# qq456cvb/SLAM-MaskRCNN

Hardware: AMD Instinct MI355X
Metric: Mvoxel-updates/s + frames/s, 512^3 semantic TSDF @ 640x480 (higher is better)
Workload: dtype f32; 1 GPU; C3: 512^3 semantic TSDF integrate (sdf f32, weight i32, colour u8x3, 32-bin u32 instance histogram), synthetic 640x480 depth+RGB+mask stream (seed 1, noise on), frames resident in HBM; frames_cycled=16

## Files before the change

### __graft_entry__.py

```python
from __future__ import annotations

import os
import subprocess
import sys

ROOT = os.path.dirname(os.path.abspath(__file__))
PKG = os.path.join(ROOT, "slam-maskrcnn_amd")
CSRC = os.path.join(PKG, "csrc")
LIB = os.path.join(PKG, "semtsdf", "libsemtsdf.so")

HIPCC_FLAGS = ["--offload-arch=gfx950", "-O3", "-ffp-contract=off", "-fPIC", "-shared", "-std=c++17", "-Wall",
               "-Wno-unused-result", "-Wno-bitwise-instead-of-logical"]


def _path():
    for p in (PKG, ROOT):
        if p not in sys.path:
            sys.path.insert(0, p)


def _lib_sources():
    srcs = [os.path.join(CSRC, f) for f in ("semtsdf_kernels.hip", "semtsdf_api.cpp")]
    hdrs = [os.path.join(CSRC, f) for f in ("semtsdf_internal.h", "semtsdf_libm.h", "semtsdf_steps.h")]
    return srcs, srcs + hdrs + [os.path.join(ROOT, "include", "semtsdf.h")]


def build_key(hipcc: str | None = None, extra_flags=()) -> str:
    import hashlib

    hipcc = hipcc or os.environ.get("HIPCC", "/opt/rocm/bin/hipcc")
    h = hashlib.sha256()
    for d in _lib_sources()[1]:
        with open(d, "rb") as f:
            h.update(os.path.basename(d).encode() + b"\0" + f.read() + b"\0")
    h.update(" ".join([*HIPCC_FLAGS, *extra_flags]).encode())
    try:
        ver = subprocess.run([hipcc, "--version"], capture_output=True, text=True, timeout=60).stdout
        h.update(next((ln for ln in ver.splitlines() if "clang version" in ln), ver).encode())
    except Exception:
        pass
    return h.hexdigest()


def build_lib(force: bool = False, extra_flags=(), out: str | None = None) -> str:
    srcs, deps = _lib_sources()
    out = out or LIB
    if not force and os.path.exists(out) and all(os.path.getmtime(out) >= os.path.getmtime(d) for d in deps):
        return out
    hipcc = os.environ.get("HIPCC", "/opt/rocm/bin/hipcc")
    key = build_key(hipcc, extra_flags)
    cmd = [hipcc, *HIPCC_FLAGS, *extra_flags, f'-DSEMTSDF_BUILD_KEY="{key}"', *srcs, "-o", out]
    subprocess.check_call(cmd)
    return out


DET_LIB = os.path.join(PKG, "semtsdf", "libsemtsdf_det.so")


def build_det_lib(force: bool = False) -> str:
    src = os.path.join(CSRC, "semtsdf_det.hip")
    deps = [src, os.path.join(ROOT, "include", "semtsdf_det.h")]
    if not force and os.path.exists(DET_LIB) and all(os.path.getmtime(DET_LIB) >= os.path.getmtime(d) for d in deps):
        return DET_LIB
    hipcc = os.environ.get("HIPCC", "/opt/rocm/bin/hipcc")
    subprocess.check_call([hipcc, *HIPCC_FLAGS, src, "-o", DET_LIB])
    return DET_LIB


def build() -> None:
    build_lib(force=True)
    build_det_lib(force=True)
    _path()
    sys.path.insert(0, os.path.join(ROOT, "oracle"))
    import oracle as O

    O.build(force=True)
    import semtsdf

    semtsdf.load()


def smoke() -> None:
    import numpy as np

    _path()
    sys.path.insert(0, os.path.join(ROOT, "oracle"))
    import oracle as O
    import semtsdf
    from semtsdf import _lib as L
    from semtsdf.synth import SyntheticStream

    semtsdf.load()
    st = SyntheticStream(seed=0)
    f0, f1, f2 = st.frame(0), st.frame(1), st.frame(2)
    D = 64
    p = semtsdf.default_params(D, (520.9, 521.0, 325.1, 249.7), 640, 480)
    semtsdf.place_from_frame(p, f0.depth, float(np.mean(f0.depth[f0.depth > 0])) / 5000.0, L.PLACE_SFM)
    vol = semtsdf.Volume(p, 0)
    g = O.OGeom.from_params(p)
    ost = O.OState(list(p.dim), p.mu, semantic=True)
    num_objs = 0
    for k, fr in enumerate((f1, f2)):
        E = (fr.w2c @ f0.c2w).astype(np.float32)
        m_gpu = fr.mask.copy()
        vol.parse_frame(fr.depth, fr.rgb, m_gpu, E)
        m_ref = fr.mask.copy()
# ... 30 lines not shown
```

### slam-maskrcnn_amd/csrc/semtsdf_api.cpp

```cpp
#include <hip/hip_runtime.h>

#include <algorithm>
#include <cmath>
#include <cstdarg>
#include <cstdio>
#include <cstdlib>
#include <cstring>
#include <mutex>
#include <string>
#include <vector>

#include "../../include/semtsdf.h"
#include "semtsdf_internal.h"

using namespace semtsdf;

namespace {

thread_local std::string g_err;

int fail(int code, const char* fmt, ...) {
    char buf[1024];
    va_list ap;
    va_start(ap, fmt);
    vsnprintf(buf, sizeof(buf), fmt, ap);
    va_end(ap);
    g_err = buf;
    return code;
}

#define HIPC(expr)                                                                                  \
    do {                                                                                            \
        hipError_t e_ = (expr);                                                                     \
        if (e_ != hipSuccess)                                                                       \
            return fail(e_ == hipErrorOutOfMemory ? SEMTSDF_ERR_OOM : SEMTSDF_ERR_HIP, "%s: %s (%s:%d)", \
                        #expr, hipGetErrorString(e_), __FILE__, __LINE__);                          \
    } while (0)

const uint8_t kPalette[kMaxObjects * 3] = {
    230, 25,  75,  60,  180, 75,  255, 225, 25,  0,   130, 200, 245, 130, 48,  145, 30,  180,
    70,  240, 240, 240, 50,  230, 210, 245, 60,  250, 190, 190, 0,   128, 128, 230, 190, 255,
    170, 110, 40,  255, 250, 200, 128, 0,   0,   170, 255, 195, 230, 25,  75,  60,  180, 75,
    255, 225, 25,  0,   130, 200, 245, 130, 48,  145, 30,  180, 70,  240, 240, 240, 50,  230,
    210, 245, 60,  250, 190, 190, 0,   128, 128, 230, 190, 255, 170, 110, 40,  255, 250, 200,
    128, 0,   0,   170, 255, 195};

constexpr int kCounters = 8;
#ifndef SEMTSDF_FRAME_SETS
#define SEMTSDF_FRAME_SETS 2
#endif
constexpr int kFrameSets = SEMTSDF_FRAME_SETS;

struct EventPair {
    hipEvent_t a, b;
};

}

struct semtsdf_vol {
    semtsdf_params p{};
    VolGeom g{};
    VolBufs b{};
    int device = 0;
    hipStream_t stream = nullptr;
    size_t device_bytes = 0;
    uint16_t* depth_d = nullptr;
    uint8_t* rgb_d = nullptr;
    uint8_t* mask_d = nullptr;
    int32_t* cls_d = nullptr;
    struct FrameSet {
        DepthPyramid pyr{};
        unsigned* unit_list = nullptr;
        unsigned* list_count = nullptr;
        unsigned* units = nullptr;
        unsigned* first_tab = nullptr;
        hipEvent_t prep_done = nullptr;
        hipEvent_t set_free = nullptr;
        bool free_recorded = false;
        hipStream_t reader = nullptr;
    } fs[kFrameSets];
    int next_set = 0;
    hipStream_t prep_stream = nullptr;
    hipEvent_t in_ev = nullptr;
    bool async_used = false;
    AssocTables* tables_d = nullptr;
    AssocDecision* decision_d = nullptr;
    AssocExact* exact_d = nullptr;
    AssocPixels px{};
    bool assoc_ray_done = false;
    int* num_objs_d = nullptr;
    float* probs_d = nullptr;
    uint8_t* box_d = nullptr;
    uint8_t* palette_d = nullptr;
    uint8_t* render_d = nullptr;
    float* render_t_d = nullptr;
    uint8_t* maps_d = nullptr;
    uint8_t* track_d = nullptr;
    unsigned long long* counters_d = nullptr;
    IntegrateRare* rare_d = nullptr;
    float* rcp_table_d = nullptr;
    AssocDecision* decision_h = nullptr;
    void* ray_state_d = nullptr;
    MarchCamera ray_cam{};
    int ray_kind = -1;
    int ray_nrec = 1;
    int ray_next = 0;
    uint32_t n_obs = 0;
    bool maps_dirty = false;
    bool maps_stale = true;
    hipEvent_t maps_ev = nullptr;
    bool maps_ev_set = false;
    hipStream_t map_stream = nullptr;
    bool map_set = false;
    bool multi_stream = false;
    bool color_wide = false;
    int64_t wmax_bound = 0;
    const uint8_t* pending_lut = nullptr;
    unsigned long long* wtrace_d = nullptr;
    unsigned* tile_cost_d = nullptr;
    unsigned* tile_perm_d = nullptr;
    int tile_cap = 0, tile_n = 0;
    bool tables_clean = false;
    unsigned long long votes_dropped_seen = 0;
    int instr = 0;
    std::vector<EventPair> ev_integrate, ev_assoc, ev_render, ev_prep;
    double t_integrate = 0, t_assoc = 0, t_render = 0, t_prep = 0;
    uint64_t n_integrate = 0, n_assoc = 0, n_render = 0, n_prep = 0;
};

namespace {

unsigned order_event_flags() { return hipEventDisableTiming | hipEventDisableSystemFence; }

size_t npx(const semtsdf_vol* v) { return (size_t)v->p.width * (size_t)v->p.height; }

hipStream_t pick(const semtsdf_vol* v, void* s) { return s ? (hipStream_t)s : v->stream; }

int dev_alloc(semtsdf_vol* v, void** p, size_t bytes) {
    if (bytes == 0) { *p = nullptr; return SEMTSDF_OK; }
    hipError_t e = hipMalloc(p, bytes);
    if (e != hipSuccess)
        return fail(e == hipErrorOutOfMemory ? SEMTSDF_ERR_OOM : SEMTSDF_ERR_HIP, "hipMalloc(%zu): %s", bytes,
                    hipGetErrorString(e));
    v->device_bytes += bytes;
    return SEMTSDF_OK;
}

void free_all(semtsdf_vol* v) {
    void* ptrs[] = {v->b.sdf, v->b.wt, v->b.bplain, v->b.boct, v->b.botmp, v->b.bdirty, v->b.dlist, v->b.sflag, v->b.color, v->b.hist, v->b.hmask, v->b.cls, v->b.cls_cnt, v->depth_d, v->rgb_d,
                    v->mask_d, v->cls_d, v->tables_d, v->decision_d,
                    v->num_objs_d, v->probs_d, v->box_d, v->palette_d, v->render_d, v->render_t_d, v->maps_d, v->track_d,
                    v->counters_d, v->ray_state_d, v->rcp_table_d, v->wtrace_d, v->exact_d, v->px.bits, v->px.p, v->tile_cost_d, v->tile_perm_d, v->rare_d};
    for (void* q : ptrs)
        if (q) (void)hipFree(q);
    for (auto& f : v->fs)
        for (void* q : {(void*)f.pyr.px, (void*)f.pyr.l0, (void*)f.pyr.l1, (void*)f.unit_list, (void*)f.list_count,
                        (void*)f.units})
            if (q) (void)hipFree(q);
    if (v->decision_h) (void)hipHostFree(v->decision_h);
    for (auto* vec : {&v->ev_integrate, &v->ev_assoc, &v->ev_render, &v->ev_prep})
        for (auto& e : *vec) { (void)hipEventDestroy(e.a); (void)hipEventDestroy(e.b); }
    if (v->maps_ev) (void)hipEventDestroy(v->maps_ev);
    for (auto& f : v->fs) {
        if (f.prep_done) (void)hipEventDestroy(f.prep_done);
        if (f.set_free) (void)hipEventDestroy(f.set_free);
    }
    if (v->prep_stream) (void)hipStreamDestroy(v->prep_stream);
    if (v->in_ev) (void)hipEventDestroy(v->in_ev);
    if (v->stream) (void)hipStreamDestroy(v->stream);
}

int local_planes(const semtsdf_params* p, int* chunk, int* halo);
int after_maps(semtsdf_vol* v, hipStream_t s);

int check_params(const semtsdf_params* p) {
    if (!p) return fail(SEMTSDF_ERR_INVALID, "params is NULL");
    for (int i = 0; i < 3; ++i) {
        if (p->dim[i] < 2 || p->dim[i] > 65535)
            return fail(SEMTSDF_ERR_INVALID, "dim[%d]=%d out of range [2, 65535]", i, p->dim[i]);
        if (!(p->voxel[i] > 0.0f) || !std::isfinite(p->voxel[i]))
            return fail(SEMTSDF_ERR_INVALID, "voxel[%d]=%g must be > 0 (place the volume first)", i, p->voxel[i]);
    }
    {
        const uint64_t ny = ((uint64_t)p->dim[1] + 7) / 8 * 8, nz = ((uint64_t)p->dim[2] + 2 * kZAlign) / kZAlign * kZAlign;
        if ((uint64_t)p->dim[0] * ny * nz >= (1ull << 32) || ny * nz >= (1ull << 32) || nz * 32 >= (1ull << 24))
            return fail(SEMTSDF_ERR_INVALID, "volume %d x %d x %d too large (2^32 stored voxels or more)", p->dim[0],
                        p->dim[1], p->dim[2]);
    }
    if (!(p->mu > 0.0f)) return fail(SEMTSDF_ERR_INVALID, "mu=%g must be > 0", p->mu);
    if (p->width <= 0 || p->height <= 0 || p->width > 65535 || p->height > 65535 || (int64_t)p->width * p->height > (1 << 28))
        return fail(SEMTSDF_ERR_INVALID, "bad frame size %dx%d", p->width, p->height);
    if (!(p->depth_scale > 0.0f)) return fail(SEMTSDF_ERR_INVALID, "depth_scale must be > 0");
    if (!(p->prior_mrcnn_err_rate >= 0x1p-10f && p->prior_mrcnn_err_rate < 1.0f))
        return fail(SEMTSDF_ERR_INVALID, "prior_mrcnn_err_rate=%g outside [2^-10, 1)", (double)p->prior_mrcnn_err_rate);
    if ((p->flags & SEMTSDF_F_VOTE) && (p->flags & SEMTSDF_F_SEMANTIC))
        return fail(SEMTSDF_ERR_INVALID, "SEMANTIC and VOTE are exclusive");
    for (int i = 0; i < 3; ++i)
        if (!(p->voxel[i] >= 0x1p-20f && p->voxel[i] <= 0x1p20f))
            return fail(SEMTSDF_ERR_INVALID, "voxel size %g outside [2^-20, 2^20]", (double)p->voxel[i]);
// ... 10 lines not shown
                        p->dim[1], p->dim[2], lz);
    }
    return SEMTSDF_OK;
}

int local_planes(const semtsdf_params* p, int* chunk, int* halo) {
    if (p->z_nshards == 1) { *chunk = p->dim[2]; *halo = 0; return p->dim[2]; }
    *chunk = p->z_chunk;
    *halo = 1;
    const int nchunks = (p->dim[2] + p->z_chunk - 1) / p->z_chunk;
    int mine = 0;
    const int n = p->z_nshards;
    for (int r = 0; r * n < nchunks; ++r)
        if (r * n + ((r & 1) ? n - 1 - p->z_shard : p->z_shard) < nchunks) ++mine;
    return mine * (p->z_chunk + 1);
}

void fill_E(float dst[12], const float E[16]) {
    for (int i = 0; i < 12; ++i) dst[i] = E[i];
}

void timing_begin(semtsdf_vol* v, std::vector<EventPair>& vec, hipStream_t s, EventPair* ep) {
    ep->a = ep->b = nullptr;
    if (!(v->instr & 1)) return;
    if (hipEventCreate(&ep->a) != hipSuccess || hipEventCreate(&ep->b) != hipSuccess) return;
    (void)hipEventRecord(ep->a, s);
    (void)vec;
}

void timing_end(semtsdf_vol* v, std::vector<EventPair>& vec, hipStream_t s, EventPair* ep) {
    if (!(v->instr & 1) || !ep->a) return;
    (void)hipEventRecord(ep->b, s);
    vec.push_back(*ep);
}

void screen_map(IntegrateArgs& a) {
    for (int i = 0; i < 3; ++i) {
        for (int j = 0; j < 3; ++j) {
            const double acc = (double)a.K[i * 3 + 0] * (double)a.E[0 * 4 + j] +
                               (double)a.K[i * 3 + 1] * (double)a.E[1 * 4 + j] +
                               (double)a.K[i * 3 + 2] * (double)a.E[2 * 4 + j];
            a.M[i * 3 + j] = (float)acc;
        }
        const double acc = (double)a.K[i * 3 + 0] * (double)a.E[3] + (double)a.K[i * 3 + 1] * (double)a.E[7] +
                           (double)a.K[i * 3 + 2] * (double)a.E[11];
        a.m[i] = (float)acc;
    }
    double KE[4][4];
    for (int i = 0; i < 4; ++i)
        for (int j = 0; j < 4; ++j) {
            if (i == 3) {
                KE[i][j] = (double)a.E[2 * 4 + j];
                continue;
            }
            KE[i][j] = (double)a.K[i * 3 + 0] * (double)a.E[0 * 4 + j] + (double)a.K[i * 3 + 1] * (double)a.E[1 * 4 + j] +
                       (double)a.K[i * 3 + 2] * (double)a.E[2 * 4 + j];
        }
    for (int i = 0; i < 4; ++i) {
        double c0 = KE[i][3];
        for (int j = 0; j < 3; ++j) {
            a.cullC[i * 4 + j] = (float)(KE[i][j] * (double)a.g.voxel[j]);
            c0 += KE[i][j] * (double)a.g.start[j];
        }
        a.cullC[i * 4 + 3] = (float)c0;
    }
    int b = 1;
    while (b < (a.width > a.height ? a.width : a.height) + 2) b <<= 1;
    a.ftol = 0.5f - ldexpf((float)b, -21);
}

int widen_color(semtsdf_vol* v, hipStream_t s) {
    if (v->color_wide) return SEMTSDF_OK;
    void* wide = nullptr;
    if (int rc = dev_alloc(v, &wide, v->g.nvox * 16)) return rc;
    HIPC(launch_color_widen(static_cast<const uint8_t*>(v->b.color), static_cast<int32_t*>(wide), v->g.nvox, s));
    HIPC(hipStreamSynchronize(s));
    HIPC(hipFree(v->b.color));
    v->device_bytes -= v->g.nvox * 4;
    v->b.color = wide;
    v->color_wide = true;
    return SEMTSDF_OK;
}


int ensure_prep_stream(semtsdf_vol* v) {
    if (v->prep_stream) return SEMTSDF_OK;
    int lo = 0, hi = 0;
    if (hipDeviceGetStreamPriorityRange(&lo, &hi) != hipSuccess) hi = 0;
    HIPC(hipStreamCreateWithPriority(&v->prep_stream, hipStreamNonBlocking, hi));
    for (auto& f : v->fs) {
        HIPC(hipEventCreateWithFlags(&f.prep_done, order_event_flags()));
        HIPC(hipEventCreateWithFlags(&f.set_free, order_event_flags()));
    }
    return SEMTSDF_OK;
}

int integrate_impl(semtsdf_vol* v, const uint16_t* depth_d, const uint8_t* rgb_d, const uint8_t* mask_d,
                   const int32_t* cls_d, const float E[16], hipStream_t s, bool async = false,
                   hipEvent_t inputs_ready = nullptr, bool inputs_on_s = false) {
    if (!E) return fail(SEMTSDF_ERR_INVALID, "E is NULL");
    if (!depth_d || !rgb_d) return fail(SEMTSDF_ERR_INVALID, "depth/rgb is NULL");
    if ((v->p.flags & SEMTSDF_F_SEMANTIC) && !mask_d) return fail(SEMTSDF_ERR_INVALID, "semantic volume needs a mask");
    if ((v->p.flags & SEMTSDF_F_VOTE) && !cls_d) return fail(SEMTSDF_ERR_INVALID, "vote volume needs cls");
    if ((v->p.flags & SEMTSDF_F_COLOR_I32) && !v->color_wide && v->wmax_bound + 1 >= (1ll << 23)) {
        if (int rc = widen_color(v, s)) return rc;
    }
    IntegrateArgs a{};
    a.g = v->g;
    a.b = v->b;
    fill_E(a.E, E);
    const float* K = v->p.K;
    a.K[0] = K[0]; a.K[1] = K[1]; a.K[2] = K[2];
    a.K[3] = K[4]; a.K[4] = K[5]; a.K[5] = K[6];
    a.K[6] = K[8]; a.K[7] = K[9]; a.K[8] = K[10];
    a.width = v->p.width;
    a.height = v->p.height;
    a.depth_scale = v->p.depth_scale;
    a.gate = v->p.gate;
    a.flags = v->p.flags | ((v->instr & 2) ? 0x80000000u : 0u);
    a.color_wide = v->color_wide ? 1 : 0;
    a.cull = (v->p.flags & SEMTSDF_F_NO_CULL) ? 0 : 1;
    {
        static const char* dbg = getenv("SEMTSDF_DEBUG_INTEGRATE");
        a.debug = dbg ? atoi(dbg) : 0;
    }
    a.depth = depth_d;
    a.rgb = rgb_d;
    a.mask = mask_d;
    a.cls = cls_d;
    const int fset = v->next_set;
    semtsdf_vol::FrameSet& F = v->fs[fset];
    a.pyr = F.pyr;
    a.counters = v->counters_d;
    a.rare = v->rare_d;
    a.unit_list = F.unit_list;
    a.list_count = F.list_count;
    a.units = F.units;
    a.first_tab = F.first_tab;
    a.first_nwaves = integrate_pre_waves();
    a.rcp_table = v->rcp_table_d;
    screen_map(a);
    a.pinhole = (a.K[1] == 0.0f && a.K[3] == 0.0f && a.K[6] == 0.0f && a.K[7] == 0.0f && a.K[8] == 1.0f) ? 1 : 0;
    a.rmu = 1.0f / v->g.mu;
    a.skip_thr = v->g.voxel[0] / 2.0f * (1.0f + 0x1p-16f);
    a.fastdiv = (v->g.mu >= 0x1p-20f && v->g.mu <= 0x1p20f && a.debug != 8) ? 1 : 0;
    a.free_ok = ((v->p.flags & SEMTSDF_F_GATE_COLOR) && !(v->p.flags & SEMTSDF_F_VOTE) && !(a.gate > 1.0f) &&
                 a.fastdiv && a.debug != 9)
                    ? 1
                    : 0;
    if (a.debug == 2) return SEMTSDF_OK;
    const uint8_t* lut = mask_d ? v->pending_lut : nullptr;
    const bool relabel_after = async && lut;
    if (async)
        if (int rc = ensure_prep_stream(v)) return rc;
    hipStream_t ps = s;
    const bool own_order = inputs_ready && inputs_on_s && s == v->stream && (!F.reader || F.reader == v->stream);
    if (async) {
        ps = v->prep_stream;
        v->async_used = true;
        if (inputs_ready) HIPC(hipStreamWaitEvent(ps, inputs_ready, 0));
        if (!own_order) {
            if (!F.free_recorded) {
                HIPC(hipEventRecord(F.set_free, F.reader == v->stream ? v->stream : s));
                F.free_recorded = true;
            }
            HIPC(hipStreamWaitEvent(ps, F.set_free, 0));
        }
    }
    v->next_set = (v->next_set + 1) % kFrameSets;
    EventPair epp;
    timing_begin(v, v->ev_prep, ps, &epp);
    HIPC(launch_depth_pyramid(depth_d, rgb_d, const_cast<uint8_t*>(mask_d), v->p.width, v->p.height,
                              v->p.depth_scale, F.pyr, F.list_count, ps, relabel_after ? nullptr : lut));
    if (lut && !relabel_after) v->pending_lut = nullptr;
    HIPC(launch_cull(a, ps));
    HIPC(launch_compact_lists(a, ps));
    timing_end(v, v->ev_prep, ps, &epp);
    v->n_prep++;
    if (async) {
        HIPC(hipEventRecord(F.prep_done, ps));
        HIPC(hipStreamWaitEvent(s, F.prep_done, 0));
    }
    if (relabel_after) {
        a.lut = &v->decision_d->lut[0];
        a.relabel_mask = const_cast<uint8_t*>(mask_d);
    }
    if (int rc = after_maps(v, s)) return rc;
    v->wmax_bound += 1;
// ... 364 lines not shown
    if (mode == SEMTSDF_PLACE_PYTHON) {
        const double md = mean_depth / 5000.0;
        double tl[3], br[3];
        const double tv[3] = {(double)rx, (double)ry, 1.0}, bv[3] = {(double)(rx + rw), (double)(ry + rh), 1.0};
        for (int i = 0; i < 3; ++i) {
            tl[i] = ((double)Ki[i * 4 + 0] * tv[0] + (double)Ki[i * 4 + 1] * tv[1]) + (double)Ki[i * 4 + 2] * tv[2];
            br[i] = ((double)Ki[i * 4 + 0] * bv[0] + (double)Ki[i * 4 + 1] * bv[1]) + (double)Ki[i * 4 + 2] * bv[2];
            tl[i] *= md;
            br[i] *= md;
        }
        const double dx = tl[0] - br[0], dy = tl[1] - br[1];
        const double half = std::sqrt(dx * dx + dy * dy) / 2.0;
        double vox[3];
        for (int i = 0; i < 3; ++i) {
            const double c = (tl[i] + br[i]) / 2.0;
            const double s = c - half, e = c + half;
            p->vol_start[i] = (float)s;
            p->vol_end[i] = (float)e;
            vox[i] = (e - s) / (double)(p->dim[i] - 1);
            p->voxel[i] = (float)vox[i];
        }
        p->mu = (float)(5.0 * vox[0]);
    } else {
        const float md = (float)mean_depth;
        float tl[4], br[4];
        const float tv[4] = {(float)rx, (float)ry, 1.0f, 1.0f};
        const float bv[4] = {(float)(rx + rw), (float)(ry + rh), 1.0f, 1.0f};
        for (int i = 0; i < 4; ++i) {
            double at = 0, ab = 0;
            for (int k = 0; k < 4; ++k) {
                at += (double)Ki[i * 4 + k] * (double)tv[k];
                ab += (double)Ki[i * 4 + k] * (double)bv[k];
            }
            tl[i] = (float)((double)(float)at * (double)md);
            br[i] = (float)((double)(float)ab * (double)md);
        }
        const float dx = tl[0] - br[0], dy = tl[1] - br[1];
        const float half = (float)(std::sqrt(std::pow((double)dx, 2) + std::pow((double)dy, 2)) / 2.0);
        for (int i = 0; i < 3; ++i) {
            const float c = (tl[i] + br[i]) * 0.5f;
            p->vol_start[i] = c - half;
            p->vol_end[i] = c + half;
            p->voxel[i] = (p->vol_end[i] - p->vol_start[i]) / (float)(p->dim[i] - 1);
        }
        p->mu = 5.0f * p->voxel[0];
    }
    return SEMTSDF_OK;
}

int semtsdf_create(const semtsdf_params* p, int device, semtsdf_vol** out) {
    if (!out) return fail(SEMTSDF_ERR_INVALID, "out is NULL");
    *out = nullptr;
    int rc = check_params(p);
    if (rc) return rc;
    HIPC(hipSetDevice(device));
    semtsdf_vol* v = new semtsdf_vol();
    v->p = *p;
    v->device = device;
    int chunk, halo;
    const int lz = local_planes(p, &chunk, &halo);
    VolGeom& g = v->g;
    g.dimx = p->dim[0]; g.dimy = p->dim[1]; g.dimz = p->dim[2];
    g.lz = lz;
    g.zs = (lz + kZAlign - 1) & ~(kZAlign - 1);
    g.shard = p->z_shard; g.nshards = p->z_nshards; g.chunk = chunk; g.halo = halo;
    for (int i = 0; i < 3; ++i) { g.start[i] = p->vol_start[i]; g.end[i] = p->vol_end[i]; g.voxel[i] = p->voxel[i]; }
    g.mu = p->mu;
    g.nuy = (uint32_t)(g.dimy + 7) / 8;
    g.nuz = (uint32_t)g.zs / 32;
    g.nvox = (uint64_t)g.dimx * g.nuy * g.nuz * 256u;
    g.ty = g.nuz * 256u;
    g.tx = g.nuy * g.ty;
    g.nbx = (g.dimx + 7) / 8; g.nby = (g.dimy + 7) / 8; g.nbz = (g.lz + 7) / 8;
    for (int i = 0; i < 3; ++i) g.rvox[i] = 1.0f / g.voxel[i];
    const size_t n = g.nvox;
    const size_t px = (size_t)p->width * p->height;
    auto bail = [&](int code) { free_all(v); delete v; return code; };
    int prio_least = 0, prio_greatest = 0;
    if (hipDeviceGetStreamPriorityRange(&prio_least, &prio_greatest) != hipSuccess) prio_greatest = 0;
    if (hipStreamCreateWithPriority(&v->stream, hipStreamNonBlocking, prio_greatest) != hipSuccess)
        return bail(fail(SEMTSDF_ERR_HIP, "hipStreamCreate failed"));
    const bool ci32 = p->flags & SEMTSDF_F_COLOR_I32;
    if ((rc = dev_alloc(v, (void**)&v->b.sdf, n * 4))) return bail(rc);
    if ((rc = dev_alloc(v, (void**)&v->b.wt, n * 4))) return bail(rc);
    if ((rc = dev_alloc(v, (void**)&v->b.sflag, n / 32 + 1))) return bail(rc);
    const size_t nbricks = (size_t)g.nbx * g.nby * g.nbz;
    if ((rc = dev_alloc(v, (void**)&v->b.bplain, nbricks * 4))) return bail(rc);
    if ((rc = dev_alloc(v, (void**)&v->b.boct, nbricks * 8))) return bail(rc);
    if ((rc = dev_alloc(v, (void**)&v->b.botmp, nbricks * 8))) return bail(rc);
    const size_t nquads = (size_t)g.nbx * g.nby * (size_t)((g.nbz + 3) / 4);
    if ((rc = dev_alloc(v, (void**)&v->b.bdirty, nquads * 4))) return bail(rc);
    if ((rc = dev_alloc(v, (void**)&v->b.dlist, (nquads + 1) * 4))) return bail(rc);
    if (nquads && (hipMemset(v->b.bdirty, 0, nquads * 4) != hipSuccess || hipMemset(v->b.dlist, 0, 4) != hipSuccess))
        return bail(fail(SEMTSDF_ERR_HIP, "memset failed"));
    (void)ci32;
    if ((rc = dev_alloc(v, &v->b.color, g.nvox * 4))) return bail(rc);
    if (p->flags & SEMTSDF_F_SEMANTIC)
    {
        if ((rc = dev_alloc(v, (void**)&v->b.hist, g.nvox * kMaxObjects * 4))) return bail(rc);
        if ((rc = dev_alloc(v, (void**)&v->b.hmask, n * 4))) return bail(rc);
    }
    if (p->flags & SEMTSDF_F_VOTE) {
        if ((rc = dev_alloc(v, (void**)&v->b.cls, n * 4))) return bail(rc);
        if ((rc = dev_alloc(v, (void**)&v->b.cls_cnt, n * 4))) return bail(rc);
        if ((rc = dev_alloc(v, (void**)&v->cls_d, px * 4))) return bail(rc);
    }
    if ((rc = dev_alloc(v, (void**)&v->depth_d, px * 2))) return bail(rc);
    if ((rc = dev_alloc(v, (void**)&v->rgb_d, px * 3))) return bail(rc);
    if ((rc = dev_alloc(v, (void**)&v->mask_d, px))) return bail(rc);
    for (auto& f : v->fs) {
        DepthPyramid& pyr = f.pyr;
        pyr.w0 = (p->width + 7) / 8; pyr.h0 = (p->height + 7) / 8;
        pyr.w1 = (p->width + 31) / 32; pyr.h1 = (p->height + 31) / 32;
        pyr.rs = 4u * (unsigned)((p->width + 1 + 3) / 4 * 4);
        const size_t nrec = (size_t)pyr.rs * (size_t)((p->height + 1 + 3) / 4);
        if ((rc = dev_alloc(v, (void**)&pyr.px, nrec * 8))) return bail(rc);
        if (hipMemset(pyr.px, 0, nrec * 8) != hipSuccess) return bail(fail(SEMTSDF_ERR_HIP, "memset failed"));
        if ((rc = dev_alloc(v, (void**)&pyr.l0, (size_t)pyr.w1 * 4 * pyr.h1 * 4 * sizeof(uint2)))) return bail(rc);
        if ((rc = dev_alloc(v, (void**)&pyr.l1, (size_t)pyr.w1 * pyr.h1 * sizeof(uint2)))) return bail(rc);
        if ((rc = dev_alloc(v, (void**)&f.unit_list, unit_list_capacity(g) * sizeof(unsigned)))) return bail(rc);
        if ((rc = dev_alloc(v, (void**)&f.list_count, kListCountWords * sizeof(unsigned)))) return bail(rc);
        const uint64_t nunits = std::max<uint64_t>(unit_count(g) + 2 * kLists + 2, 2u * (uint64_t)kPreWaves + 6u);
        if ((rc = dev_alloc(v, (void**)&f.units, (nunits + 2u * (uint64_t)kPreWaves) * sizeof(unsigned)))) return bail(rc);
        f.first_tab = f.units + nunits;
    }
    if ((rc = dev_alloc(v, (void**)&v->rcp_table_d, kRcpTable * sizeof(float)))) return bail(rc);
    {
        float t[kRcpTable];
        for (int i = 0; i < kRcpTable; ++i) t[i] = 1.0f / (float)(i + 1);
        if (hipMemcpy(v->rcp_table_d, t, sizeof(t), hipMemcpyHostToDevice) != hipSuccess)
            return bail(fail(SEMTSDF_ERR_HIP, "rcp table upload failed"));
    }
    if ((rc = dev_alloc(v, (void**)&v->tables_d, sizeof(AssocTables)))) return bail(rc);
    if ((rc = dev_alloc(v, (void**)&v->decision_d, sizeof(AssocDecision)))) return bail(rc);
    if ((rc = dev_alloc(v, (void**)&v->exact_d, sizeof(AssocExact)))) return bail(rc);
    if (hipMemset(v->exact_d, 0, sizeof(AssocExact)) != hipSuccess) return bail(fail(SEMTSDF_ERR_HIP, "memset failed"));
    if ((p->flags & SEMTSDF_F_SEMANTIC) && p->z_nshards == 1) {
        if ((rc = dev_alloc(v, (void**)&v->px.bits, npx(v) * sizeof(uint2)))) return bail(rc);
        if ((rc = dev_alloc(v, (void**)&v->px.p, npx(v) * kMaxObjects * sizeof(float)))) return bail(rc);
    }
    if ((rc = dev_alloc(v, (void**)&v->num_objs_d, 16))) return bail(rc);
    if ((rc = dev_alloc(v, (void**)&v->counters_d, kCounters * sizeof(unsigned long long)))) return bail(rc);
    if ((rc = dev_alloc(v, (void**)&v->rare_d, sizeof(IntegrateRare)))) return bail(rc);
    {
        const IntegrateRare r{v->b.bdirty, v->b.dlist, g.nby, g.nbz, v->counters_d};
        if (hipMemcpy(v->rare_d, &r, sizeof(r), hipMemcpyHostToDevice) != hipSuccess)
            return bail(fail(SEMTSDF_ERR_HIP, "upload of the integrate's rare-path fields failed"));
    }
    if ((rc = dev_alloc(v, (void**)&v->palette_d, sizeof(kPalette)))) return bail(rc);
    if (hipHostMalloc((void**)&v->decision_h, sizeof(AssocDecision), 0) != hipSuccess)
        return bail(fail(SEMTSDF_ERR_HIP, "hipHostMalloc failed"));
    if (hipMemcpy(v->palette_d, kPalette, sizeof(kPalette), hipMemcpyHostToDevice) != hipSuccess)
        return bail(fail(SEMTSDF_ERR_HIP, "palette upload failed"));
    if ((rc = semtsdf_reset(v, nullptr))) return bail(rc);
    if (hipStreamSynchronize(v->stream) != hipSuccess) return bail(fail(SEMTSDF_ERR_HIP, "sync failed"));
    *out = v;
    return SEMTSDF_OK;
}

int semtsdf_destroy(semtsdf_vol* v) {
    if (!v) return SEMTSDF_OK;
    (void)hipSetDevice(v->device);
    (void)hipStreamSynchronize(v->stream);
    free_all(v);
    delete v;
    return SEMTSDF_OK;
}

int semtsdf_get_params(const semtsdf_vol* v, semtsdf_params* out) {
    if (!v || !out) return fail(SEMTSDF_ERR_INVALID, "NULL argument");
    *out = v->p;
    return SEMTSDF_OK;
}

int semtsdf_get_state(const semtsdf_vol* v, semtsdf_state* out) {
    if (!v || !out) return fail(SEMTSDF_ERR_INVALID, "NULL argument");
    int n = 0;
    unsigned long long dropped = 0;
    HIPC(hipMemcpyAsync(&n, v->num_objs_d, sizeof(int), hipMemcpyDeviceToHost, v->stream));
    HIPC(hipMemcpyAsync(&dropped, v->counters_d + 2, sizeof(dropped), hipMemcpyDeviceToHost, v->stream));
    HIPC(hipStreamSynchronize(v->stream));
    out->n_obs = v->n_obs;
    out->num_objs = n;
    out->local_dim[0] = v->g.dimx;
    out->local_dim[1] = v->g.dimy;
    out->local_dim[2] = v->g.lz;
    out->local_voxels = (uint64_t)v->g.dimx * v->g.dimy * v->g.lz;
    out->device_bytes = v->device_bytes;
    out->label_votes_dropped = dropped;
    return SEMTSDF_OK;
}

int semtsdf_set_state(semtsdf_vol* v, uint32_t n_obs, int32_t num_objs) {
    if (!v) return fail(SEMTSDF_ERR_INVALID, "NULL handle");
    v->n_obs = n_obs;
    HIPC(hipMemcpyAsync(v->num_objs_d, &num_objs, sizeof(int), hipMemcpyHostToDevice, v->stream));
    HIPC(hipStreamSynchronize(v->stream));
    return SEMTSDF_OK;
}

void* semtsdf_get_stream(const semtsdf_vol* v) { return v ? (void*)v->stream : nullptr; }

int semtsdf_reset(semtsdf_vol* v, void* stream) {
    if (!v) return fail(SEMTSDF_ERR_INVALID, "NULL handle");
    HIPC(hipSetDevice(v->device));
    hipStream_t s = pick(v, stream);
    const size_t n = v->g.nvox;
    if (int rc = after_maps(v, s)) return rc;
    HIPC(launch_fill_volume(v->g, v->b, v->p.flags, s));
    HIPC(hipMemsetAsync(v->b.wt, 0, n * 4, s));
    HIPC(hipMemsetAsync(v->b.sflag, 0, n / 32 + 1, s));
    HIPC(hipMemsetAsync(v->b.color, 0, v->g.nvox * 4 * (v->color_wide ? 4 : 1), s));
    if (v->b.hist) HIPC(hipMemsetAsync(v->b.hist, 0, v->g.nvox * kMaxObjects * 4, s));
    if (v->b.hmask) HIPC(hipMemsetAsync(v->b.hmask, 0, n * 4, s));
    if (v->b.cls) HIPC(hipMemsetAsync(v->b.cls, 0, n * 4, s));
    if (v->b.cls_cnt) HIPC(hipMemsetAsync(v->b.cls_cnt, 0, n * 4, s));
    HIPC(hipMemsetAsync(v->num_objs_d, 0, 16, s));
    HIPC(hipMemsetAsync(v->counters_d, 0, kCounters * sizeof(unsigned long long), s));
    v->votes_dropped_seen = 0;
    v->n_obs = 0;
    v->wmax_bound = 0;
    v->maps_stale = true;
    return SEMTSDF_OK;
}

static int observe_before(semtsdf_vol* v, const uint8_t* mask_d, hipStream_t s) {
    if (!(v->p.flags & SEMTSDF_F_SEMANTIC) || v->n_obs > 0) return SEMTSDF_OK;
    if (!mask_d) return fail(SEMTSDF_ERR_INVALID, "semantic volume needs a mask");
    if (int rc = tables_ready(v, s)) return rc;
    HIPC(launch_mask_stats(mask_d, (int)npx(v), v->tables_d, s));
    HIPC(launch_first_frame_objs(v->tables_d, v->num_objs_d, s));
    return SEMTSDF_OK;
}
static void observe_after(semtsdf_vol* v) {
    if (v->p.flags & SEMTSDF_F_SEMANTIC) v->n_obs++;
}

int semtsdf_integrate(semtsdf_vol* v, const uint16_t* depth, const uint8_t* rgb, const uint8_t* mask,
                      const float E[16], void* stream) {
    if (!v || !depth || !rgb) return fail(SEMTSDF_ERR_INVALID, "NULL argument");
    HIPC(hipSetDevice(v->device));
    hipStream_t s = pick(v, stream);
    const size_t n = npx(v);
    const bool sem = v->p.flags & SEMTSDF_F_SEMANTIC;
    bool past_bins = false;
    if (sem) {
        if (!mask) return fail(SEMTSDF_ERR_INVALID, "semantic volume needs a mask");
        if (v->p.flags & SEMTSDF_F_ID_SATURATE) {
            if (int rc = validate_mask_host(v, mask)) return rc;
        } else {
            past_bins = validate_mask_host(v, mask) != SEMTSDF_OK;
        }
    }
    HIPC(hipMemcpyAsync(v->depth_d, depth, n * 2, hipMemcpyHostToDevice, s));
    HIPC(hipMemcpyAsync(v->rgb_d, rgb, n * 3, hipMemcpyHostToDevice, s));
    if (sem) HIPC(hipMemcpyAsync(v->mask_d, mask, n, hipMemcpyHostToDevice, s));
    if (int rc = observe_before(v, sem ? v->mask_d : nullptr, s)) return rc;
    int rc = integrate_impl(v, v->depth_d, v->rgb_d, sem ? v->mask_d : nullptr, nullptr, E, s);
    if (rc) return rc;
    observe_after(v);
    HIPC(hipStreamSynchronize(s));
    if (!sem) return SEMTSDF_OK;
    const int rc_votes = check_bad_label(v, s);
    if (past_bins)
        return fail(SEMTSDF_ERR_LABEL, "mask labels >= %d have no histogram bin: their votes were dropped, the "
                    "frame was applied (SEMTSDF_F_ID_SATURATE keeps ids below %d)", kMaxObjects, kMaxObjects);
    return rc_votes;
}

int semtsdf_integrate_dev(semtsdf_vol* v, const uint16_t* depth_d, const uint8_t* rgb_d, const uint8_t* mask_d,
                          const float E[16], void* stream) {
    if (!v) return fail(SEMTSDF_ERR_INVALID, "NULL handle");
    HIPC(hipSetDevice(v->device));
    hipStream_t s = pick(v, stream);
    if (int rc = observe_before(v, mask_d, s)) return rc;
    if (int rc = integrate_impl(v, depth_d, rgb_d, mask_d, nullptr, E, s)) return rc;
    observe_after(v);
    return SEMTSDF_OK;
}

int semtsdf_integrate_dev_async(semtsdf_vol* v, const uint16_t* depth_d, const uint8_t* rgb_d, const uint8_t* mask_d,
                                const float E[16], void* inputs_ready, void* stream) {
    if (!v) return fail(SEMTSDF_ERR_INVALID, "NULL handle");
    HIPC(hipSetDevice(v->device));
    hipStream_t s = pick(v, stream);
    if (int rc = observe_before(v, mask_d, s)) return rc;
    if (int rc = integrate_impl(v, depth_d, rgb_d, mask_d, nullptr, E, s, true, (hipEvent_t)inputs_ready)) return rc;
    observe_after(v);
    return SEMTSDF_OK;
}

int semtsdf_integrate_vote_dev(semtsdf_vol* v, const uint16_t* depth_d, const uint8_t* rgb_d, const int32_t* cls_d,
                               const float E[16], void* stream) {
// ... 758 lines not shown
    if (flags) HIPC(hipMemcpyAsync(flags, flags_d, n, hipMemcpyDeviceToHost, s));
    HIPC(hipStreamSynchronize(s));
    return SEMTSDF_OK;
}

static int icp_check(semtsdf_vol* v, const semtsdf_icp_in* in, const float* E_ref, const float* E_cur, float dist_max,
                     float cos_min, int32_t stride, const int64_t* words) {
    if (!v || !in || !E_ref || !E_cur || !words) return fail(SEMTSDF_ERR_INVALID, "NULL argument");
    if (!in->vertex || !in->normal || !in->flags || !in->m_point || !in->m_normal || !in->m_flags)
        return fail(SEMTSDF_ERR_INVALID, "NULL input map");
    if (npx(v) > ((size_t)1 << 19))
        return fail(SEMTSDF_ERR_INVALID, "image %d x %d has more than 2^19 pixels (the bound of the integer sums)",
                    v->p.width, v->p.height);
    if (stride < 1) return fail(SEMTSDF_ERR_INVALID, "stride=%d must be >= 1", (int)stride);
    if (!(dist_max > 0.0f && dist_max <= 1.0f))
        return fail(SEMTSDF_ERR_INVALID, "dist_max=%g outside (0, 1]", (double)dist_max);
    if (!(cos_min >= -1.0f && cos_min <= 1.0f))
        return fail(SEMTSDF_ERR_INVALID, "cos_min=%g outside [-1, 1]", (double)cos_min);
    if (v->p.z_nshards != 1)
        return fail(SEMTSDF_ERR_UNSUPPORTED, "the ICP system on a Z-sharded handle is not supported");
    return SEMTSDF_OK;
}

static int icp_impl(semtsdf_vol* v, const semtsdf_icp_in& in_d, const float E_ref[16], const float E_cur[16],
                    float dist_max, float cos_min, int32_t stride, int64_t* words_d, hipStream_t s) {
    IcpArgs a{};
    a.vertex = in_d.vertex; a.normal = in_d.normal; a.flags = in_d.flags;
    a.m_point = in_d.m_point; a.m_normal = in_d.m_normal; a.m_flags = in_d.m_flags;
    for (int i = 0; i < 3; ++i) {
        double acc = 0;
        for (int k = 0; k < 3; ++k) acc += (double)E_cur[k * 4 + i] * (double)E_cur[k * 4 + 3];
        a.o[i] = (float)(-acc);
        for (int j = 0; j < 3; ++j) {
            a.Rt[i * 3 + j] = E_cur[j * 4 + i];
            a.K[i * 3 + j] = v->p.K[i * 4 + j];
        }
    }
    fill_E(a.Eref, E_ref);
    a.dmax2 = dist_max * dist_max;
    a.cos_min = cos_min;
    a.stride = stride;
    a.width = v->p.width;
    a.height = v->p.height;
    a.words = reinterpret_cast<long long*>(words_d);
    HIPC(hipMemsetAsync(words_d, 0, kIcpWords * 8, s));
    HIPC(launch_icp_system(a, s));
    return SEMTSDF_OK;
}

int semtsdf_icp_system_dev(semtsdf_vol* v, const semtsdf_icp_in* in_dev, const float E_ref[16],
                           const float E_cur[16], float dist_max, float cos_min, int32_t stride, int64_t* words_dev,
                           void* stream) {
    if (int rc = icp_check(v, in_dev, E_ref, E_cur, dist_max, cos_min, stride, words_dev)) return rc;
    HIPC(hipSetDevice(v->device));
    return icp_impl(v, *in_dev, E_ref, E_cur, dist_max, cos_min, stride, words_dev, pick(v, stream));
}

int semtsdf_icp_system(semtsdf_vol* v, const semtsdf_icp_in* in_host, const float E_ref[16], const float E_cur[16],
                       float dist_max, float cos_min, int32_t stride, int64_t* words_host, void* stream) {
    if (int rc = icp_check(v, in_host, E_ref, E_cur, dist_max, cos_min, stride, words_host)) return rc;
    HIPC(hipSetDevice(v->device));
    hipStream_t s = pick(v, stream);
    const size_t n = npx(v);
    if (int rc = track_scratch(v)) return rc;
    float* f = reinterpret_cast<float*>(v->track_d);
    uint8_t* b = v->track_d + n * 48 + kIcpWords * 8;
    int64_t* words_d = reinterpret_cast<int64_t*>(v->track_d + n * 48);
    HIPC(hipMemcpyAsync(f, in_host->vertex, n * 12, hipMemcpyHostToDevice, s));
    HIPC(hipMemcpyAsync(f + n * 3, in_host->normal, n * 12, hipMemcpyHostToDevice, s));
    HIPC(hipMemcpyAsync(f + n * 6, in_host->m_point, n * 12, hipMemcpyHostToDevice, s));
    HIPC(hipMemcpyAsync(f + n * 9, in_host->m_normal, n * 12, hipMemcpyHostToDevice, s));
    HIPC(hipMemcpyAsync(b, in_host->flags, n, hipMemcpyHostToDevice, s));
    HIPC(hipMemcpyAsync(b + n, in_host->m_flags, n, hipMemcpyHostToDevice, s));
    semtsdf_icp_in d{f, f + n * 3, b, f + n * 6, f + n * 9, b + n};
    if (int rc = icp_impl(v, d, E_ref, E_cur, dist_max, cos_min, stride, words_d, s)) return rc;
    HIPC(hipMemcpyAsync(words_host, words_d, kIcpWords * 8, hipMemcpyDeviceToHost, s));
    HIPC(hipStreamSynchronize(s));
    return SEMTSDF_OK;
}

static uint64_t nref(const semtsdf_vol* v) { return (uint64_t)v->g.dimx * v->g.dimy * v->g.lz; }

static int vox_xfer(semtsdf_vol* v, void* host, void* dev, bool to_host, const char* what, hipStream_t s, uint64_t vb,
                    uint64_t ve) {
    if (ve <= vb) return SEMTSDF_OK;
    const uint64_t chunk = std::min<uint64_t>(ve - vb, 1ull << 26);
    void* stage = nullptr;
    HIPC(hipMalloc(&stage, chunk * 4));
    for (uint64_t v0 = vb; v0 < ve; v0 += chunk) {
        const uint64_t nv = std::min<uint64_t>(chunk, ve - v0);
        char* h = static_cast<char*>(host) + (v0 - vb) * 4;
        hipError_t e;
        if (to_host) {
            e = launch_vox_chunk(dev, stage, true, v->g, v0, nv, s);
            if (e == hipSuccess) e = hipMemcpyAsync(h, stage, nv * 4, hipMemcpyDeviceToHost, s);
        } else {
            e = hipMemcpyAsync(stage, h, nv * 4, hipMemcpyHostToDevice, s);
            if (e == hipSuccess) e = launch_vox_chunk(stage, dev, false, v->g, v0, nv, s);
        }
        if (e == hipSuccess) e = hipStreamSynchronize(s);
        if (e != hipSuccess) {
            (void)hipFree(stage);
            return fail(SEMTSDF_ERR_HIP, "%s transfer: %s", what, hipGetErrorString(e));
        }
    }
    HIPC(hipFree(stage));
    return SEMTSDF_OK;
}

static int color_xfer(semtsdf_vol* v, void* host, bool to_host, hipStream_t s, uint64_t vb, uint64_t ve) {
    const bool i32 = v->p.flags & SEMTSDF_F_COLOR_I32;
    const size_t es = i32 ? 4 : 1;
    if (ve <= vb) return SEMTSDF_OK;
    const uint64_t chunk = std::min<uint64_t>(ve - vb, 1ull << 24);
    void* stage = nullptr;
    HIPC(hipMalloc(&stage, chunk * 3 * es));
    for (uint64_t v0 = vb; v0 < ve; v0 += chunk) {
        const uint64_t nv = std::min<uint64_t>(chunk, ve - v0);
        char* h = static_cast<char*>(host) + (v0 - vb) * 3 * es;
        hipError_t e;
        if (to_host) {
            e = launch_color_chunk(v->b.color, stage, true, i32, v->color_wide, v->g, v0, nv, s);
            if (e == hipSuccess) e = hipMemcpyAsync(h, stage, nv * 3 * es, hipMemcpyDeviceToHost, s);
        } else {
            e = hipMemcpyAsync(stage, h, nv * 3 * es, hipMemcpyHostToDevice, s);
            if (e == hipSuccess) e = launch_color_chunk(stage, v->b.color, false, i32, v->color_wide, v->g, v0, nv, s);
        }
        if (e == hipSuccess) e = hipStreamSynchronize(s);
        if (e != hipSuccess) {
            (void)hipFree(stage);
            return fail(SEMTSDF_ERR_HIP, "colour transfer: %s", hipGetErrorString(e));
        }
    }
    HIPC(hipFree(stage));
    return SEMTSDF_OK;
}

int semtsdf_download_slab(semtsdf_vol* v, int x0, int x1, float* sdf, int32_t* wt, void* color, uint32_t* hist,
                          int32_t* cls, int32_t* cls_cnt) {
    if (!v) return fail(SEMTSDF_ERR_INVALID, "NULL handle");
    if (x0 < 0 || x1 > v->g.dimx || x0 > x1) return fail(SEMTSDF_ERR_INVALID, "bad x range [%d, %d)", x0, x1);
    HIPC(hipSetDevice(v->device));
    hipStream_t s = v->stream;
    const uint64_t plane = (uint64_t)v->g.dimy * v->g.lz;
    const uint64_t vb = (uint64_t)x0 * plane, ve = (uint64_t)x1 * plane;
    int rc;
    if (sdf && (rc = vox_xfer(v, sdf, v->b.sdf, true, "sdf", s, vb, ve))) return rc;
    if (wt && (rc = vox_xfer(v, wt, v->b.wt, true, "weight", s, vb, ve))) return rc;
    if (color) {
        rc = color_xfer(v, color, true, s, vb, ve);
        if (rc) return rc;
    }
    if (cls) {
        if (!(v->p.flags & SEMTSDF_F_VOTE)) return fail(SEMTSDF_ERR_STATE, "not a VOTE volume");
        if ((rc = vox_xfer(v, cls, v->b.cls, true, "cls", s, vb, ve))) return rc;
    }
    if (cls_cnt) {
        if (!(v->p.flags & SEMTSDF_F_VOTE)) return fail(SEMTSDF_ERR_STATE, "not a VOTE volume");
        if ((rc = vox_xfer(v, cls_cnt, v->b.cls_cnt, true, "cls_cnt", s, vb, ve))) return rc;
    }
    if (hist) {
        if (!(v->p.flags & SEMTSDF_F_SEMANTIC)) return fail(SEMTSDF_ERR_STATE, "not a SEMANTIC volume");
        const uint64_t chunk = std::max<uint64_t>(1, std::min<uint64_t>(ve - vb, 1ull << 22));
        uint32_t* stage = nullptr;
        HIPC(hipMalloc(&stage, chunk * kMaxObjects * 4));
        for (uint64_t v0 = vb; v0 < ve; v0 += chunk) {
            const uint64_t nv = std::min<uint64_t>(chunk, ve - v0);
            hipError_t e = launch_hist_chunk_to_vm(v->b.hist, stage, v->g, v0, nv, s);
            if (e == hipSuccess)
                e = hipMemcpyAsync(hist + (v0 - vb) * kMaxObjects, stage, nv * kMaxObjects * 4, hipMemcpyDeviceToHost, s);
            if (e == hipSuccess) e = hipStreamSynchronize(s);
            if (e != hipSuccess) {
                (void)hipFree(stage);
                return fail(SEMTSDF_ERR_HIP, "histogram download: %s", hipGetErrorString(e));
            }
        }
        HIPC(hipFree(stage));
    }
    HIPC(hipStreamSynchronize(s));
    return SEMTSDF_OK;
}

int semtsdf_download(semtsdf_vol* v, float* sdf, int32_t* wt, void* color, uint32_t* hist, int32_t* cls,
                     int32_t* cls_cnt) {
    if (!v) return fail(SEMTSDF_ERR_INVALID, "NULL handle");
    return semtsdf_download_slab(v, 0, v->g.dimx, sdf, wt, color, hist, cls, cls_cnt);
}

int semtsdf_upload(semtsdf_vol* v, const float* sdf, const int32_t* wt, const void* color, const uint32_t* hist,
                   const int32_t* cls, const int32_t* cls_cnt) {
    if (!v) return fail(SEMTSDF_ERR_INVALID, "NULL handle");
    HIPC(hipSetDevice(v->device));
    hipStream_t s = v->stream;
    int rc;
    if ((rc = after_maps(v, s))) return rc;
    v->maps_stale = true;
    if (sdf || wt) HIPC(hipMemsetAsync(v->b.sflag, 0, v->g.nvox / 32 + 1, s));
    if (sdf && (rc = vox_xfer(v, const_cast<float*>(sdf), v->b.sdf, false, "sdf", s, 0, nref(v)))) return rc;
    if (wt && (rc = vox_xfer(v, const_cast<int32_t*>(wt), v->b.wt, false, "weight", s, 0, nref(v)))) return rc;
    if (wt) {
        int64_t m = 0;
        for (uint64_t i = 0, n = nref(v); i < n; ++i) m = std::max<int64_t>(m, wt[i]);
        v->wmax_bound = m;
    }
    if (color) {
        if ((v->p.flags & SEMTSDF_F_COLOR_I32) && !v->color_wide) {
            const int32_t* c = static_cast<const int32_t*>(color);
            const uint64_t nc = nref(v) * 3;
            bool fits = true;
            for (uint64_t i = 0; i < nc && fits; ++i) fits = (uint32_t)c[i] <= 255u;
            if (!fits && (rc = widen_color(v, s))) return rc;
        }
        rc = color_xfer(v, const_cast<void*>(color), false, s, 0, nref(v));
        if (rc) return rc;
    }
    if (cls) {
        if (!(v->p.flags & SEMTSDF_F_VOTE)) return fail(SEMTSDF_ERR_STATE, "not a VOTE volume");
        if ((rc = vox_xfer(v, const_cast<int32_t*>(cls), v->b.cls, false, "cls", s, 0, nref(v)))) return rc;
    }
    if (cls_cnt) {
        if (!(v->p.flags & SEMTSDF_F_VOTE)) return fail(SEMTSDF_ERR_STATE, "not a VOTE volume");
        if ((rc = vox_xfer(v, const_cast<int32_t*>(cls_cnt), v->b.cls_cnt, false, "cls_cnt", s, 0, nref(v)))) return rc;
    }
    if (hist) {
        if (!(v->p.flags & SEMTSDF_F_SEMANTIC)) return fail(SEMTSDF_ERR_STATE, "not a SEMANTIC volume");
        HIPC(hipMemsetAsync(v->b.hmask, 0xFF, v->g.nvox * 4, s));
        const uint64_t n = (uint64_t)v->g.dimx * v->g.dimy * v->g.lz;
        const uint64_t chunk = std::max<uint64_t>(1, std::min<uint64_t>(n, 1ull << 22));
        uint32_t* stage = nullptr;
        HIPC(hipMalloc(&stage, chunk * kMaxObjects * 4));
        for (uint64_t v0 = 0; v0 < n; v0 += chunk) {
            const uint64_t nv = std::min<uint64_t>(chunk, n - v0);
            hipError_t e =
                hipMemcpyAsync(stage, hist + v0 * kMaxObjects, nv * kMaxObjects * 4, hipMemcpyHostToDevice, s);
            if (e == hipSuccess) e = launch_hist_chunk_to_bm(stage, v->b.hist, v->g, v0, nv, s);
            if (e == hipSuccess) e = hipStreamSynchronize(s);
            if (e != hipSuccess) {
                (void)hipFree(stage);
                return fail(SEMTSDF_ERR_HIP, "histogram upload: %s", hipGetErrorString(e));
            }
        }
        HIPC(hipFree(stage));
        HIPC(launch_hist_mask(v->g, v->b, s));
    }
    v->maps_stale = true;
    HIPC(hipStreamSynchronize(s));
    return SEMTSDF_OK;
}

int semtsdf_map_words(semtsdf_vol* v, uint64_t* out, uint64_t capacity, uint64_t* count) {
    if (!v || !count) return fail(SEMTSDF_ERR_INVALID, "NULL argument");
    HIPC(hipSetDevice(v->device));
    hipStream_t s = v->stream;
    *count = (uint64_t)v->g.nbx * v->g.nby * v->g.nbz;
    if (int rc = ensure_maps(v, s)) return rc;
    const uint64_t n = std::min<uint64_t>(capacity, *count);
    if (out && n) HIPC(hipMemcpyAsync(out, v->b.boct, n * sizeof(uint64_t), hipMemcpyDeviceToHost, s));
    HIPC(hipStreamSynchronize(s));
    return SEMTSDF_OK;
}

int semtsdf_export_surface(semtsdf_vol* v, float sdf_max, int32_t min_weight, semtsdf_surface_point* out,
                           uint64_t capacity, uint64_t* count) {
    static_assert(sizeof(semtsdf_surface_point) == sizeof(SurfacePoint), "surface point layout");
    if (!v || !count) return fail(SEMTSDF_ERR_INVALID, "NULL argument");
    if (!(sdf_max > 0.0f)) return fail(SEMTSDF_ERR_INVALID, "sdf_max must be > 0");
    HIPC(hipSetDevice(v->device));
    hipStream_t s = v->stream;
    if (int rc = after_maps(v, s)) return rc;
    unsigned long long* cnt_d = nullptr;
    HIPC(hipMalloc((void**)&cnt_d, sizeof(unsigned long long)));
    SurfacePoint* pts_d = nullptr;
    auto cleanup = [&]() {
        if (cnt_d) (void)hipFree(cnt_d);
        if (pts_d) (void)hipFree(pts_d);
    };
    auto run = [&](SurfacePoint* o, uint64_t cap, unsigned long long* n) -> hipError_t {
        hipError_t e = hipMemsetAsync(cnt_d, 0, sizeof(unsigned long long), s);
        if (e == hipSuccess) e = launch_export_surface(v->g, v->b, sdf_max, min_weight, v->color_wide ? 1 : 0,
                                                       (v->p.flags & SEMTSDF_F_SEMANTIC) ? 1 : 0, o, cap, cnt_d, s);
        if (e == hipSuccess) e = hipMemcpyAsync(n, cnt_d, sizeof(*n), hipMemcpyDeviceToHost, s);
        if (e == hipSuccess) e = hipStreamSynchronize(s);
        return e;
    };
    unsigned long long n = 0;
    hipError_t e = run(nullptr, 0, &n);
// ... 286 lines not shown
```

### slam-maskrcnn_amd/csrc/semtsdf_internal.h

```cpp
#pragma once
#include <hip/hip_runtime_api.h>
#include <stdint.h>

namespace semtsdf {

constexpr int kMaxObjects = 32;
constexpr int kMaxDetections = 256;
constexpr int kRcpTable = 1024;
constexpr int kZAlign = 32;
#ifndef SEMTSDF_BRICK_DIST_CAP
#define SEMTSDF_BRICK_DIST_CAP 16
#endif
constexpr int kBrickDistCap = SEMTSDF_BRICK_DIST_CAP;
constexpr int kListSegs = 64;
constexpr unsigned kPreWaves = 65534;
constexpr unsigned kFirstTabSlots = kListSegs * 256;
constexpr int kListCountStride = 64;
constexpr int kLists = 3;
constexpr int kListTotalsWord = kLists * kListSegs * kListCountStride;
constexpr int kListCountWords = kListTotalsWord + 8;

struct VolGeom {
    int dimx, dimy, dimz;
    int lz;
    int zs;
    int shard, nshards, chunk, halo;
    float start[3];
    float end[3];
    float voxel[3];
    float mu;
    uint64_t nvox;
    uint32_t nuy, nuz;
    uint32_t tx, ty;
    int nbx, nby, nbz;
    float rvox[3];
};

__device__ inline uint32_t tile_xterm(const VolGeom& g, int x) { return (uint32_t)x * g.tx; }
__device__ inline uint32_t tile_yterm(const VolGeom& g, int y) {
    return __umul24((uint32_t)(y >> 3), g.ty) + (uint32_t)(y & 7) * 4u;
}
__device__ inline uint32_t tile_zterm(int zl) { return (uint32_t)(zl >> 5) * 256u + (uint32_t)((zl >> 2) & 7) * 32u + (uint32_t)(zl & 3); }
__device__ inline uint32_t tile_index(const VolGeom& g, int x, int y, int zl) {
    return tile_xterm(g, x) + tile_yterm(g, y) + tile_zterm(zl);
}

struct VolBufs {
    float* sdf;
    int32_t* wt;
    void* color;
    uint32_t* hist;
    uint32_t* hmask;
    int32_t* cls;
    int32_t* cls_cnt;
    float* bplain;
    uint64_t* boct;
    uint64_t* botmp;
    uint32_t* bdirty;
    uint32_t* dlist;
    uint8_t* sflag;
};

struct DepthPyramid {
    uint2* px;
    uint2* l0;
    uint2* l1;
    int w0, h0, w1, h1;
    unsigned rs;
};

__device__ inline unsigned rec_index(const DepthPyramid& p, unsigned u, unsigned v) {
    return __umul24(v >> 2, p.rs) + ((u << 2) | (v & 3u));
}

struct IntegrateRare {
    uint32_t* bdirty;
    uint32_t* dlist;
    int nby, nbz;
    unsigned long long* counters;
};

struct IntegrateArgs {
    VolGeom g;
    VolBufs b;
    float E[12];
    float K[9];
    float M[9];
    float m[3];
    float cullC[16];
    float ftol;
    float skip_thr;
    const float* rcp_table;
    int width, height;
    float depth_scale;
    float gate;
    uint32_t flags;
    int cull;
    int debug;
    const uint16_t* depth;
    const uint8_t* rgb;
    const uint8_t* mask;
    const int32_t* cls;
    DepthPyramid pyr;
    unsigned long long* counters;
    int pinhole;
    float rmu;
    int fastdiv;
    unsigned* unit_list;
    unsigned* list_count;
    unsigned* units;
    int free_ok;
    int color_wide;
    unsigned long long* wtrace;
    unsigned wtrace_slots;
    const uint8_t* lut;
    uint8_t* relabel_mask;
    const IntegrateRare* rare;
    unsigned* first_tab;
    unsigned first_nwaves;
};
constexpr int kWaveTraceWords = 8;

constexpr double kFixScale = 268435456.0;
struct AssocTables {
    long long t1[kMaxObjects][kMaxObjects];
    long long t3[kMaxObjects][kMaxObjects];
    long long t2[kMaxObjects];
    unsigned int c1[kMaxObjects];
    unsigned int c2[kMaxObjects];
    unsigned int c3[kMaxObjects][kMaxObjects];
    unsigned int first_px[256];
    unsigned int max_label;
    unsigned int pos_max;
};
static_assert(sizeof(AssocTables) % 8 == 0, "AssocTables is cleared as 8-B words");

struct AssocDecision {
    int max_obj_now;
    int num_objs_before;
    int num_objs_after;
    int bad_label;
    int assigned_prev[kMaxObjects];
    float assigned_prob[kMaxObjects];
    unsigned char lut[256];
// ... 86 lines not shown
    uint8_t* flags;
};

struct FrameMapsArgs {
    const uint16_t* depth;
    float Kinv[9];
    float depth_scale;
    int width, height;
    float* vertex;
    float* normal;
    uint8_t* flags;
};

constexpr int kIcpWords = 32;

struct IcpArgs {
    const float* vertex;
    const float* normal;
    const uint8_t* flags;
    const float* m_point;
    const float* m_normal;
    const uint8_t* m_flags;
    float Rt[9], o[3];
    float Eref[12];
    float K[9];
    float dmax2, cos_min;
    int stride;
    int width, height;
    long long* words;
};

struct ShardRayState {
    int* k;
    float* fk;
    int* j;
    float* fj;
    float* fp;
    float* t;
};

constexpr int kAssocPartialLen = 3 * kMaxObjects * kMaxObjects + 3 * kMaxObjects;

struct ShardRayArgs {
    VolGeom g;
    VolBufs b;
    MarchCamera cam;
    int width, height;
    int kind;
    int step;
    const int2* gathered;
    int nrec;
    int2* send;
    ShardRayState st;
    int color_i32;
    const uint8_t* palette;
    uint8_t* out_bgr;
    float* out_t;
    const uint8_t* mask;
    float n_obs, eps, box_thresh;
    long long* partial;
};

hipError_t launch_shard_ray_step(const ShardRayArgs& a, hipStream_t s);
hipError_t launch_shard_render_final(const ShardRayArgs& a, hipStream_t s);
hipError_t launch_shard_render_finish(const ShardRayArgs& a, hipStream_t s);
hipError_t launch_shard_assoc_partial(const ShardRayArgs& a, hipStream_t s);
hipError_t launch_shard_assoc_pixels(const ShardRayArgs& a, int32_t* out, hipStream_t s);
hipError_t launch_tables_from_partial(const long long* reduced, AssocTables* t, hipStream_t s);
hipError_t launch_copy_f4(const void* src, void* dst, size_t n16, hipStream_t s);
hipError_t launch_min_i64(long long* dst, const long long* src, size_t n, hipStream_t s);
hipError_t launch_masks_to_labels(const uint8_t* masks, int npx, int n, int min_area, void* scratch, uint8_t* out,
                                  hipStream_t s);
size_t mask_scratch_bytes();
size_t mask_scratch_kept_offset();
hipError_t launch_detections_to_labels(const int32_t* boxes, const void* mini, int dtype, int mh, int mw, int n,
                                       int width, int height, int min_area, void* scratch, uint8_t* out,
                                       uint32_t* areas, hipStream_t s);
hipError_t launch_brick_min(const VolGeom& g, const VolBufs& b, bool all, hipStream_t s);
hipError_t launch_fill_volume(const VolGeom& g, const VolBufs& b, uint32_t flags, hipStream_t s);
hipError_t launch_depth_pyramid(const uint16_t* depth, const uint8_t* rgb, uint8_t* mask, int w, int h,
                                float scale, const DepthPyramid& p, unsigned* list_count, hipStream_t s,
                                const uint8_t* lut = nullptr);
hipError_t launch_vox_chunk(const void* src, void* dst, bool to_ref, const VolGeom& g, uint64_t v0, uint64_t nv,
                            hipStream_t s);
hipError_t launch_color_widen(const uint8_t* narrow, int32_t* wide, uint64_t nvox, hipStream_t s);
hipError_t launch_color_chunk(const void* src, void* dst, bool to_ref, bool ref_i32, bool dev_i32, const VolGeom& g,
                              uint64_t v0, uint64_t nv, hipStream_t s);
hipError_t launch_integrate(const IntegrateArgs& a, hipStream_t s, hipEvent_t e0 = nullptr,
                            hipEvent_t e1 = nullptr);
uint64_t unit_count(const VolGeom& g);
uint64_t unit_list_capacity(const VolGeom& g);
int unit_grid_fits(int dimx, int dimy, int local_z);
hipError_t launch_cull(const IntegrateArgs& a, hipStream_t s);
hipError_t launch_compact_lists(const IntegrateArgs& a, hipStream_t s);
unsigned integrate_pre_waves();
hipError_t launch_tables_init(AssocTables* t, hipStream_t s);
hipError_t launch_mask_stats(const uint8_t* mask, int npx, AssocTables* t, hipStream_t s);
hipError_t launch_assoc_march(const AssocArgs& a, hipStream_t s);
hipError_t launch_assoc_decide(const DecideArgs& a, hipStream_t s);
hipError_t launch_assoc_from_probs(const float* probs, const uint8_t* box, const uint8_t* mask, int npx, float n_obs,
                                   float eps, AssocTables* t, AssocPixels px, hipStream_t s);
hipError_t launch_libm_eval(int fn, const float* x, float* y, size_t n, hipStream_t s);
hipError_t launch_first_frame_objs(const AssocTables* t, int* num_objs_dev, hipStream_t s);
hipError_t launch_relabel(uint8_t* mask, int npx, const AssocDecision* d, hipStream_t s);
hipError_t launch_render(const RenderArgs& a, hipStream_t s);
hipError_t launch_model_maps(const MapsArgs& a, hipStream_t s);
hipError_t launch_frame_maps(const FrameMapsArgs& a, hipStream_t s);
hipError_t launch_icp_system(const IcpArgs& a, hipStream_t s);
hipError_t launch_march_fused(const AssocArgs& aa, const RenderArgs& ra, hipStream_t s);
hipError_t launch_copy_host(const void* src, void* dst, size_t n16, hipStream_t s);
hipError_t launch_hist_chunk_to_vm(const uint32_t* bm, uint32_t* vm, const VolGeom& g, uint64_t v0, uint64_t nv,
                                   hipStream_t s);
hipError_t launch_hist_chunk_to_bm(const uint32_t* vm, uint32_t* bm, const VolGeom& g, uint64_t v0, uint64_t nv,
                                   hipStream_t s);
hipError_t launch_hist_mask(const VolGeom& g, const VolBufs& b, hipStream_t s);
struct SurfacePoint {
    uint32_t x, y, z;
    float sdf;
    uint32_t rgbl;
};
hipError_t launch_export_surface(const VolGeom& g, const VolBufs& b, float sdf_max, int min_w, int color_wide,
                                 int semantic, SurfacePoint* out, uint64_t cap, unsigned long long* count, hipStream_t s);

struct MeshVertexRec {
    uint4 a;
    uint4 b;
};
constexpr int kMeshXB = 4;
constexpr unsigned kMeshGroup = 4096;
__host__ __device__ inline uint64_t mesh_blocks(const VolGeom& g) { return g.nvox / 256u; }
inline uint64_t mesh_groups(const VolGeom& g) { return (mesh_blocks(g) + kMeshGroup - 1) / kMeshGroup; }
__host__ __device__ inline uint32_t mesh_classify_blocks(const VolGeom& g) {
    return (uint32_t)((g.dimx + kMeshXB - 1) / kMeshXB) * g.nuy * g.nuz;
}
inline uint64_t mesh_list_words(const VolGeom& g) { return 2u + mesh_classify_blocks(g) + mesh_blocks(g); }
template <typename T>
__host__ __device__ inline T* mesh_list_blocks(const VolGeom&, T* alist) { return alist + 2; }
template <typename T>
__host__ __device__ inline T* mesh_list_tiles(const VolGeom& g, T* alist) { return alist + 2 + mesh_classify_blocks(g); }
hipError_t launch_mesh_count(const VolGeom& g, const VolBufs& b, int min_w, uint2* cnt, unsigned long long* gsum,
                             uint32_t* alist, ulonglong2* base, unsigned long long* tot, hipStream_t s);
hipError_t launch_mesh_emit(const VolGeom& g, const VolBufs& b, int min_w, int color_wide, int semantic,
                            const uint2* cnt, const uint32_t* alist, unsigned nblocks, unsigned ntiles,
                            const ulonglong2* base, uint32_t* vtab, MeshVertexRec* verts, uint32_t* tris, hipStream_t s);

struct InstanceRec {
    unsigned long long voxels, votes, support, sum[3], rgb_sum[3];
    uint32_t min[3], max[3];
};
hipError_t launch_instance_stats(const VolGeom& g, const VolBufs& b, float sdf_max, int min_w, int color_wide,
                                 InstanceRec* rec, unsigned long long* overlap, hipStream_t s);
struct RemapLut {
    unsigned long long w[4];
};
hipError_t launch_remap_instances(const VolGeom& g, const VolBufs& b, RemapLut lut, uint32_t moved, hipStream_t s);

}
```

### slam-maskrcnn_amd/csrc/semtsdf_kernels.hip

```cpp
#include <hip/hip_runtime.h>
#include <hip/hip_ext.h>
#include <stdint.h>
#include <limits.h>
#include <stddef.h>
#include <stdlib.h>
#include "semtsdf_internal.h"
#include "semtsdf_libm.h"
#include "semtsdf_steps.h"

namespace semtsdf {

__device__ __forceinline__ int f2i_rd(float x) {
    const float f = floorf(x);
    if (!(f == f)) return 0;
    if (f >= 2147483648.0f) return INT_MAX;
    if (f <= -2147483648.0f) return INT_MIN;
    return (int)f;
}

__device__ __forceinline__ float dot3(float a0, float a1, float a2, float b0, float b1, float b2) {
    return fmaf(a2, b2, fmaf(a1, b1, a0 * b0));
}

typedef float f32x2 __attribute__((ext_vector_type(2)));
// ... 927 lines not shown
    unsigned tmask = 0;
    float dm[4];
    float dmin = 1.0f;
#pragma unroll
    for (int k = 0; k < 4; ++k) {
        const float d = __uint_as_float(P.rec[k].x);
        dm[k] = d;
        const float diff = d - P.qz[k];
        const bool t = (d != 0.0f) & (diff > -g.mu);
        const float dc = fminf(diff, g.mu);
        C.fv[k] = div_by_rcp(dc, g.mu, a.rmu);
        dmin = __builtin_elementwise_minimum(dmin, fabsf(dc));
        tmask |= (t ? 1u : 0u) << k;
        C.pix[k] = P.rec[k].y;
        if (VOTE) C.img[k] = P.lin[k];
    }
    tmask &= P.vmask;
    if (SEM && a.lut) {
#pragma unroll
        for (int k = 0; k < 4; ++k) C.pix[k] = relabel_rec(C.pix[k], lutv);
    }
    C.sflag = P.sflag;
    C.ub = P.ub;
    if (!(dmin >= 0x1p-60f) || !a.fastdiv) {
#pragma unroll
        for (int k = 0; k < 4; ++k) {
            const float dc = fminf(dm[k] - P.qz[k], g.mu);
            if (!a.fastdiv || !(fabsf(dc) >= 0x1p-60f)) C.fv[k] = dc == 0.0f ? dc : dc / g.mu;
        }
    }
    unsigned gbits = 0xFu;
    if (GATE) {
        gbits = 0u;
#pragma unroll
        for (int k = 0; k < 4; ++k) gbits |= (C.fv[k] < a.gate ? 1u : 0u) << k;
    }
    unsigned gmask = tmask & gbits;
    if (COUNT && count) {
        n_touch += __popc(tmask);
        n_gate += __popc(gmask);
        n_lines += count_lines(tmask);
    }
    if (kProbes && (a.debug == 3 || a.debug == 21)) tmask = gmask = 0;
    if (kProbes && a.debug == 4) gmask = 0;
    C.tmask = tmask;
    C.gmask = gmask;
    C.hlab = 0xFFu;
    C.hmode = 0u;
    if (SEM && gmask && !(kProbes && a.debug == 6)) {
        unsigned lab = 0xFFu, same = 1u;
#pragma unroll
        for (int k = 3; k >= 0; --k) lab = ((gmask >> k) & 1u) ? (C.pix[k] >> 24) : lab;
#pragma unroll
        for (int k = 0; k < 4; ++k) same &= (((gmask >> k) & 1u) == 0u) | ((C.pix[k] >> 24) == lab);
        C.hlab = lab;
        C.hmode = (same && lab < (unsigned)kMaxObjects) ? 1u : 2u;
    }
}

constexpr uint64_t line_lanes() {
    uint64_t m = 0;
    for (int y = 0; y < UY; ++y) m |= 1ull << (LZQ * y);
    return m;
}
constexpr uint64_t kLineLanes = line_lanes();

__device__ __forceinline__ bool tile_line_all(bool p) {
    static_assert(UY == 8 && UX == 1, "lane = zq + LZQ y + kUnitLanes slot");
    const uint64_t b = __ballot(!p);
    const int lane = (int)__lane_id();
    return ((b >> (lane % LZQ + lane_slot(lane) * kUnitLanes)) & kLineLanes) == 0ull;
}

template <class T>
__device__ __forceinline__ T ld_state(const void* p) {
    static_assert(sizeof(T) == 16, "16-byte vectors");
    return *reinterpret_cast<const T*>(p);
}
template <class T>
__device__ __forceinline__ void st_state(void* p, const T& v) {
    static_assert(sizeof(T) == 16, "16-byte vectors");
    *reinterpret_cast<T*>(p) = v;
}

template <bool SEM, bool CI32, bool VOTE, bool FREE>
__device__ __forceinline__ void stage_load(const IntegrateArgs& a, const UnitPos& up, unsigned coff, const Cls& C,
                                           Ld& L) {
    const VolGeom& g = a.g;
    (void)up;
    const uint32_t ub = C.ub;
    const uint32_t v = ub + coff;
    const uint4* dummy = reinterpret_cast<const uint4*>(a.b.sdf);
    const bool t = C.tmask != 0u, gt = C.gmask != 0u;
    const unsigned lg = gt ? coff : 0u;
    bool fone = true;
#pragma unroll
    for (int k = 0; k < 4; ++k) fone &= (((C.tmask >> k) & 1u) == 0u) | (C.fv[k] == 1.0f);
    const bool skip = (C.sflag != 0u) & fone;
    L.skip = skip;
    L.s4 = ld_state<float4>(a.b.sdf + ((skip | !t) ? 0u : v));
    L.w4 = ld_state<int4>(a.b.wt + (t ? v : 0u));
    if (FREE) return;
    if (CI32) {
#pragma unroll
        for (int k = 0; k < 4; ++k) L.c32[k] = reinterpret_cast<const int4*>(a.b.color)[(uint64_t)ub + lg + (gt ? k : 0)];
    } else {
        L.c8 = ld_state<uint4>(reinterpret_cast<const uint32_t*>(a.b.color) + (gt ? v : 0u));
    }
    if (SEM)
        L.h4 = ld_state<uint4>(a.b.hist + (C.hmode == 1u ? (uint64_t)C.hlab * g.nvox + v : 0ull));
    if (VOTE) {
        L.vc4 = *(t ? reinterpret_cast<const int4*>(a.b.cls + v) : reinterpret_cast<const int4*>(dummy));
        L.vn4 = *(t ? reinterpret_cast<const int4*>(a.b.cls_cnt + v) : reinterpret_cast<const int4*>(dummy));
#pragma unroll
        for (int k = 0; k < 4; ++k) L.vin[k] = a.cls[C.img[k] < a.width * a.height ? C.img[k] : 0];
    }
}

template <bool SEM, bool GATE, bool CI32, bool VOTE, bool FREE>
__device__ __forceinline__ void stage_compute(const IntegrateArgs& a, const float* __restrict__ s_rcp, const Cls& C,
                                              const Ld& L, Out& O) {
    const unsigned tmask = C.tmask, gmask = C.gmask;
    const float so[4] = {L.skip ? 1.0f : L.s4.x, L.skip ? 1.0f : L.s4.y, L.skip ? 1.0f : L.s4.z,
                         L.skip ? 1.0f : L.s4.w};
    O.skip = L.skip;
    O.oflag = C.sflag;
    O.ub = C.ub;
    const int wo[4] = {L.w4.x, L.w4.y, L.w4.z, L.w4.w};
    float sn[4];
    int wn[4];
    unsigned wmax = 0u;
    float nmin = 1.0f;
#pragma unroll
    for (int k = 0; k < 4; ++k) {
        const int tk = (int)(tmask << (31 - k)) >> 31;
        const float num = fmaf(so[k], (float)wo[k], C.fv[k]);
        const float rw = s_rcp[min((unsigned)wo[k], (unsigned)kRcpTable - 1u)];
        const float upd = div_by_rcp(num, (float)wo[k] + 1.0f, rw);
        wmax = max(wmax, (unsigned)wo[k]);
        nmin = __builtin_elementwise_minimum(nmin, fabsf(num));
        sn[k] = __uint_as_float((__float_as_uint(upd) & (unsigned)tk) | (__float_as_uint(so[k]) & ~(unsigned)tk));
        wn[k] = wo[k] - tk;
    }
    if (!((wmax < (unsigned)kRcpTable) & (nmin >= 0x1p-60f)) || !a.fastdiv) {
#pragma unroll
        for (int k = 0; k < 4; ++k) {
            const float num = fmaf(so[k], (float)wo[k], C.fv[k]);
            const bool slow = !(((unsigned)wo[k] < (unsigned)kRcpTable) & (fabsf(num) >= 0x1p-60f)) || !a.fastdiv;
            if (!((tmask >> k) & 1u) || !slow) continue;
            sn[k] = num / (float)(wo[k] + 1);
        }
    }
    O.s4 = make_float4(sn[0], sn[1], sn[2], sn[3]);
    O.w4 = make_int4(wn[0], wn[1], wn[2], wn[3]);
    unsigned xs = 0u;
#pragma unroll
    for (int k = 0; k < 4; ++k) xs |= __float_as_uint(so[k] - a.skip_thr) ^ __float_as_uint(sn[k] - a.skip_thr);
    O.cross = (int)xs < 0;
    if (FREE) return;
    if (CI32) {
#pragma unroll
        for (int k = 0; k < 4; ++k) {
            const int4 o = L.c32[k];
            const bool gk = (gmask >> k) & 1u;
            const int wi = wo[k], dw = wo[k] + 1;
            const int r0 = C.pix[k] & 0xFF, r1 = (C.pix[k] >> 8) & 0xFF, r2 = (C.pix[k] >> 16) & 0xFF;
            int4 n;
            n.x = gk ? avg_div(o.x * wi + r0, dw) : o.x;
            n.y = gk ? avg_div(o.y * wi + r1, dw) : o.y;
            n.z = gk ? avg_div(o.z * wi + r2, dw) : o.z;
            n.w = o.w;
            O.c32[k] = n;
        }
    } else {
        O.c8 = L.c8;
    }
    if (gmask) {
        if (CI32) {
        } else {
            const unsigned co[4] = {L.c8.x, L.c8.y, L.c8.z, L.c8.w};
            unsigned cw[4];
            unsigned cslow = 0;
#pragma unroll
            for (int k = 0; k < 4; ++k) {
                const bool gk = (gmask >> k) & 1u;
                const unsigned wi = (unsigned)wo[k], o = co[k], px = C.pix[k];
                const float rw = s_rcp[min(wi, (unsigned)kRcpTable - 1u)];
                const unsigned n0 = avg_u8(o & 0xFFu, px & 0xFFu, wi, rw);
                const unsigned n1 = avg_u8((o >> 8) & 0xFFu, (px >> 8) & 0xFFu, wi, rw);
                const unsigned n2 = avg_u8((o >> 16) & 0xFFu, (px >> 16) & 0xFFu, wi, rw);
                cw[k] = gk ? (n0 | (n1 << 8) | (n2 << 16)) : o;
                cslow |= ((gk & (wi >= (unsigned)kRcpTable)) ? 1u : 0u) << k;
            }
            if (cslow) {
#pragma unroll
                for (int k = 0; k < 4; ++k) {
                    if (!(cslow & (1u << k))) continue;
                    const unsigned wi = (unsigned)wo[k], o = co[k], px = C.pix[k];
                    const int dw = (int)(wi + 1u);
                    const unsigned n0 = (unsigned)((int)((o & 0xFFu) * wi + (px & 0xFFu)) / dw);
                    const unsigned n1 = (unsigned)((int)(((o >> 8) & 0xFFu) * wi + ((px >> 8) & 0xFFu)) / dw);
                    const unsigned n2 = (unsigned)((int)(((o >> 16) & 0xFFu) * wi + ((px >> 16) & 0xFFu)) / dw);
                    cw[k] = (n0 & 0xFFu) | ((n1 & 0xFFu) << 8) | ((n2 & 0xFFu) << 16);
                }
            }
            O.c8 = make_uint4(cw[0], cw[1], cw[2], cw[3]);
        }
        if (SEM) {
            O.h4 = make_uint4(L.h4.x + (gmask & 1u), L.h4.y + ((gmask >> 1) & 1u), L.h4.z + ((gmask >> 2) & 1u),
                              L.h4.w + ((gmask >> 3) & 1u));
        }
    }
    if (VOTE) {
        int vc[4] = {L.vc4.x, L.vc4.y, L.vc4.z, L.vc4.w}, vn[4] = {L.vn4.x, L.vn4.y, L.vn4.z, L.vn4.w};
#pragma unroll
        for (int k = 0; k < 4; ++k) {
            if (!((tmask >> k) & 1u)) continue;
            if (vn[k] == 0) {
                vc[k] = L.vin[k];
                vn[k] = 1;
            } else if (vc[k] == L.vin[k]) {
                vn[k] += 1;
            } else {
                vn[k] -= 1;
            }
        }
        O.vc4 = make_int4(vc[0], vc[1], vc[2], vc[3]);
        O.vn4 = make_int4(vn[0], vn[1], vn[2], vn[3]);
    }
}

__device__ __forceinline__ void voxel_or(uint32_t* p, uint32_t v) {
    (void)__hip_atomic_fetch_or(p, v, __ATOMIC_RELAXED, __HIP_MEMORY_SCOPE_WORKGROUP);
}
__device__ __forceinline__ void voxel_add(uint32_t* p, uint32_t v) {
    (void)__hip_atomic_fetch_add(p, v, __ATOMIC_RELAXED, __HIP_MEMORY_SCOPE_WORKGROUP);
}

template <bool SEM, bool CI32, bool VOTE, bool FREE>
__device__ __forceinline__ void stage_store(const IntegrateArgs& a, const UnitPos& up, unsigned coff,
                                            const StoreMeta& M, const Out& O) {
    const VolGeom& g = a.g;
    const unsigned tmask = M.meta & 15u, gmask = (M.meta >> 4) & 15u, hmode = (M.meta >> 8) & 3u,
                   hlab = M.meta >> 16;
    {
        const uint64_t cb = __ballot(O.cross);
        const __attribute__((address_space(4))) IntegrateRare* R =
            (const __attribute__((address_space(4))) IntegrateRare*)a.rare;
        if (cb && R->bdirty) {
            const int lane = (int)__lane_id(), j = lane % kUnitLanes;
            const int bz = (up.uz * UZ >> 3) + j;
            const uint64_t pj = ((kLineLanes << (2 * (j & 3))) | (kLineLanes << (2 * (j & 3) + 1)))
                                << (lane_slot(lane) * kUnitLanes);
            if (j < UZ / 8 && (cb & pj) && bz < R->nbz) {
                const unsigned nbq = (unsigned)(R->nbz + 3) >> 2;
                const unsigned q = __umul24(__umul24((unsigned)(up.x * UX >> 3), (unsigned)R->nby) +
                                                (unsigned)(up.uy * UY >> 3), nbq) + ((unsigned)bz >> 2);
                __attribute__((address_space(1))) uint32_t* bd = (__attribute__((address_space(1))) uint32_t*)R->bdirty;
                __attribute__((address_space(1))) uint32_t* dl = (__attribute__((address_space(1))) uint32_t*)R->dlist;
                if (__hip_atomic_fetch_or(bd + q, 1u << (bz & 3), __ATOMIC_RELAXED, __HIP_MEMORY_SCOPE_AGENT) == 0u)
                    dl[1 + __hip_atomic_fetch_add(dl, 1u, __ATOMIC_RELAXED, __HIP_MEMORY_SCOPE_AGENT)] = q;
            }
        }
    }
    const bool line = ((__ballot(tmask != 0u) >> ((int)__lane_id() % LZQ + lane_slot((int)__lane_id()) * kUnitLanes)) &
                       kLineLanes) != 0ull;
    if (!line) return;
    const uint64_t v = O.ub + coff;
    if (!(kProbes && a.debug == 10) && tmask != 0u) {
        if (!O.skip) st_state(a.b.sdf + v, O.s4);
        st_state(a.b.wt + v, O.w4);
    }
    {
        const unsigned s_and = __float_as_uint(O.s4.x) & __float_as_uint(O.s4.y) & __float_as_uint(O.s4.z) &
                               __float_as_uint(O.s4.w);
        const unsigned s_or = __float_as_uint(O.s4.x) | __float_as_uint(O.s4.y) | __float_as_uint(O.s4.z) |
                              __float_as_uint(O.s4.w);
        const int wmx = max(max(O.w4.x, O.w4.y), max(O.w4.z, O.w4.w));
        const bool vals = (s_and == 0x3f800000u) & (s_or == 0x3f800000u) & (wmx < (1 << 23));
        const bool one = tmask != 0u ? vals : (O.oflag != 0u);
        const unsigned nb = tile_line_all(one) ? 1u : 0u;
        if (lane_y((int)__lane_id()) == 0 && nb != O.oflag) a.b.sflag[v >> 5] = (uint8_t)nb;
    }
    if (!FREE && gmask != 0u) {
        if (CI32) {
#pragma unroll
            for (int k = 0; k < 4; ++k) reinterpret_cast<int4*>(a.b.color)[v + k] = O.c32[k];
        } else {
            st_state(reinterpret_cast<uint32_t*>(a.b.color) + v, O.c8);
        }
        if (SEM && gmask) {
            if (hmode == 1u) {
                st_state(a.b.hist + (uint64_t)hlab * g.nvox + v, O.h4);
                const unsigned hk[4] = {O.h4.x, O.h4.y, O.h4.z, O.h4.w};
                unsigned nb = 0;
#pragma unroll
                for (int k = 0; k < 4; ++k) nb |= (((((gmask >> k) & 1u) != 0u) & (hk[k] == 1u)) ? 1u : 0u) << k;
                if (nb) {
#pragma unroll
                    for (int k = 0; k < 4; ++k)
                        if ((nb >> k) & 1u) voxel_or(a.b.hmask + v + k, 1u << hlab);
                }
            }
            if (hmode == 2u) {
                unsigned bad = 0;
#pragma unroll
                for (int k = 0; k < 4; ++k) {
                    const unsigned lab = (M.labs >> (8 * k)) & 0xFFu;
                    const bool gk = (gmask >> k) & 1u;
                    if (gk && lab < (unsigned)kMaxObjects) {
                        voxel_add(a.b.hist + (uint64_t)lab * g.nvox + v + k, 1u);
                        voxel_or(a.b.hmask + v + k, 1u << lab);
                    }
                    bad += (gk && lab >= (unsigned)kMaxObjects) ? 1u : 0u;
                }
                if (bad) {
                    const __attribute__((address_space(4))) IntegrateRare* R4 =
                        (const __attribute__((address_space(4))) IntegrateRare*)a.rare;
                    __hip_atomic_fetch_add((__attribute__((address_space(1))) unsigned long long*)R4->counters + 2,
                                           (unsigned long long)bad, __ATOMIC_RELAXED, __HIP_MEMORY_SCOPE_AGENT);
                }
            }
        }
    }
    if (!FREE && VOTE && tmask) {
        *reinterpret_cast<int4*>(a.b.cls + v) = O.vc4;
        *reinterpret_cast<int4*>(a.b.cls_cnt + v) = O.vn4;
    }
}

struct ListView {
    const unsigned* list;
    unsigned total, ngroups;
    unsigned cnt;
    unsigned i;
};

__device__ __forceinline__ ListView list_view(const unsigned* units, const unsigned* list_count, int l, unsigned wave,
                                              unsigned nwaves, unsigned rot, unsigned xi = 0u, unsigned nsp = 1u) {
    const __attribute__((address_space(4))) unsigned* tw =
        (const __attribute__((address_space(4))) unsigned*)(list_count + kListTotalsWord);
    ListView v;
    v.list = units + tw[2 * l];
    v.total = tw[2 * l + 1];
    const unsigned ng = (v.total + kSlots - 1) / kSlots;
    const unsigned lo = nsp == 1u ? 0u : ng * xi / nsp;
    v.ngroups = nsp == 1u ? ng : ng * (xi + 1u) / nsp;
    v.cnt = v.ngroups - lo;
    v.i = lo + (wave + nwaves - rot % nwaves) % nwaves;
    return v;
}

static_assert(kSlots == 2, "two entries per group (one 8-byte load, one pad per list)");
__device__ __forceinline__ void group_entries(const ListView& v, unsigned grp, unsigned seg_cap, unsigned* e) {
    (void)seg_cap;
    const __attribute__((address_space(4))) unsigned* l4 = (const __attribute__((address_space(4))) unsigned*)v.list;
    e[0] = l4[2u * grp];
    e[1] = l4[2u * grp + 1u];
}

__device__ __forceinline__ UnitPos lane_pos(const UnitGrid& ug, const unsigned* e) {
    const int slot = lane_slot(threadIdx.x & 63);
    UnitPos p = unit_pos(ug, e[0]);
#pragma unroll
    for (int k = 1; k < kSlots; ++k) {
        const bool have = e[k] != ~0u;
        const UnitPos q = unit_pos(ug, have ? e[k] : e[0]);
        if (slot == k) {
            p = q;
            p.ok = have;
        }
    }
    return p;
}

struct Counts {
    unsigned touch, gate, lines;
};

struct Pipe {
    UnitPos cur;
    Proj P;
    Cls C;
    Ld L;
    Out O;
    bool primed = false;
    unsigned lutv = 0;
    unsigned groups = 0;
};

template <int KIND>
struct KindOf {
    static constexpr bool FREE = KIND != 0, FULL = KIND == 2;
};

template <bool SEM, bool GATE, bool CI32, bool VOTE, bool COUNT, bool SHARD, bool PIN, int KIND>
__device__ __forceinline__ void list_prime(const IntegrateArgs& a, const UnitGrid& ug, unsigned seg_cap,
                                           const ListView& v, Pipe& S, Counts& n, const unsigned* pre = nullptr) {
    constexpr bool FREE = KindOf<KIND>::FREE, FULL = KindOf<KIND>::FULL;
    const int lane = threadIdx.x & 63;
    const unsigned coff = (unsigned)lane_zq(lane) * 32u + (unsigned)lane_y(lane) * 4u;
    unsigned e[kSlots];
    if (pre) {
        e[0] = pre[0];
        e[1] = pre[1];
    } else {
        group_entries(v, v.i, seg_cap, e);
    }
    S.cur = lane_pos(ug, e);
    stage_project<SHARD, PIN, FREE, FULL, VOTE>(a, S.cur, lane, S.P);
    stage_classify<SEM, GATE, VOTE, COUNT, FREE>(a, S.P, S.C, true, n.touch, n.gate, n.lines, S.lutv);
    stage_load<SEM, CI32, VOTE, FREE>(a, S.cur, coff, S.C, S.L);
    S.primed = true;
}

#ifndef SEMTSDF_PRIO_EVERY
#define SEMTSDF_PRIO_EVERY 4
#endif
static_assert((SEMTSDF_PRIO_EVERY & (SEMTSDF_PRIO_EVERY - 1)) == 0, "a power of two");
__device__ __forceinline__ void rotate_prio(unsigned p) {
    switch (p & 3u) {
        case 0: __builtin_amdgcn_s_setprio(0); break;
        case 1: __builtin_amdgcn_s_setprio(1); break;
        case 2: __builtin_amdgcn_s_setprio(2); break;
        default: __builtin_amdgcn_s_setprio(3); break;
    }
}
__device__ __forceinline__ unsigned dispatch_round() {
    return __builtin_amdgcn_readfirstlane((blockIdx.x * 4u) / gridDim.x);
}

template <bool SEM, bool GATE, bool CI32, bool VOTE, bool COUNT, bool SHARD, bool PIN, int KIND, int NKIND>
__device__ __forceinline__ void integrate_list(const IntegrateArgs& a, const UnitGrid& ug, unsigned seg_cap,
                                               const float* __restrict__ s_rcp, ListView& v, const ListView* nx,
                                               unsigned nwaves, Pipe& S, Counts& n) {
    constexpr bool FREE = KindOf<KIND>::FREE, FULL = KindOf<KIND>::FULL;
    constexpr bool NFREE = KindOf<(NKIND < 0 ? 0 : NKIND)>::FREE, NFULL = KindOf<(NKIND < 0 ? 0 : NKIND)>::FULL;
    const int lane = threadIdx.x & 63;
    const unsigned coff = (unsigned)lane_zq(lane) * 32u + (unsigned)lane_y(lane) * 4u;
    if (v.i >= v.ngroups) return;
    if (!S.primed) list_prime<SEM, GATE, CI32, VOTE, COUNT, SHARD, PIN, KIND>(a, ug, seg_cap, v, S, n);
    unsigned en[kSlots];
    if (v.i + nwaves < v.ngroups) group_entries(v, v.i + nwaves, seg_cap, en);
    const bool chain = NKIND >= 0 && nx->i < nx->ngroups;
    unsigned eb[kSlots];
    if (chain) group_entries(*nx, nx->i, seg_cap, eb);
    while (v.i + nwaves < v.ngroups) {
        const UnitPos nxt = lane_pos(ug, en);
        if (v.i + 2u * nwaves < v.ngroups) group_entries(v, v.i + 2u * nwaves, seg_cap, en);
        stage_project<SHARD, PIN, FREE, FULL, VOTE>(a, nxt, lane, S.P);
        stage_compute<SEM, GATE, CI32, VOTE, FREE>(a, s_rcp, S.C, S.L, S.O);
        const StoreMeta Mc = store_meta(S.C);
        stage_classify<SEM, GATE, VOTE, COUNT, FREE>(a, S.P, S.C, true, n.touch, n.gate, n.lines, S.lutv);
        stage_store<SEM, CI32, VOTE, FREE>(a, S.cur, coff, Mc, S.O);
        stage_load<SEM, CI32, VOTE, FREE>(a, nxt, coff, S.C, S.L);
        S.cur = nxt;
        v.i += nwaves;
        ++S.groups;
        if (SEMTSDF_PRIO_EVERY == 1 || (S.groups & (SEMTSDF_PRIO_EVERY - 1u)) == 0u)
            rotate_prio(S.groups / SEMTSDF_PRIO_EVERY);
    }
    if (chain) {
        const UnitPos nxt = lane_pos(ug, eb);
        stage_project<SHARD, PIN, NFREE, NFULL, VOTE>(a, nxt, lane, S.P);
        stage_compute<SEM, GATE, CI32, VOTE, FREE>(a, s_rcp, S.C, S.L, S.O);
        const StoreMeta Mc = store_meta(S.C);
        stage_classify<SEM, GATE, VOTE, COUNT, NFREE>(a, S.P, S.C, true, n.touch, n.gate, n.lines, S.lutv);
        stage_store<SEM, CI32, VOTE, FREE>(a, S.cur, coff, Mc, S.O);
        stage_load<SEM, CI32, VOTE, NFREE>(a, nxt, coff, S.C, S.L);
        S.cur = nxt;
        S.primed = true;
    } else {
        stage_compute<SEM, GATE, CI32, VOTE, FREE>(a, s_rcp, S.C, S.L, S.O);
        stage_store<SEM, CI32, VOTE, FREE>(a, S.cur, coff, store_meta(S.C), S.O);
        S.primed = false;
    }
    v.i += nwaves;
}

#ifndef SEMTSDF_INTEGRATE_WPE
#define SEMTSDF_INTEGRATE_WPE 4
#endif
template <bool SEM, bool GATE, bool CI32, bool VOTE, bool COUNT, bool SHARD, bool PIN>
__global__ __launch_bounds__(256) __attribute__((amdgpu_waves_per_eu(VOTE ? 3 : SEMTSDF_INTEGRATE_WPE))) void k_integrate(
    IntegrateArgs a, UnitGrid ug, unsigned seg_cap) {
    __shared__ float s_rcp[kRcpTable];
    unsigned long long tr[5] = {0, 0, 0, 0, 0};
    unsigned long long trn = 0;
    const unsigned nwaves = gridDim.x * (blockDim.x >> 6);
    const unsigned wave = __builtin_amdgcn_readfirstlane(blockIdx.x * (blockDim.x >> 6) + (threadIdx.x >> 6));
    auto groups_of = [&](unsigned n, unsigned rot_) -> unsigned long long {
        const unsigned ng = (n + kSlots - 1) / kSlots, i0 = (wave + nwaves - rot_ % nwaves) % nwaves;
        return i0 < ng ? (ng - 1u - i0) / nwaves + 1u : 0u;
    };
    if (SEMTSDF_WAVE_TRACE) tr[0] = wall_clock64();
    for (int i = (int)threadIdx.x; i < kRcpTable; i += (int)blockDim.x) s_rcp[i] = a.rcp_table[i];
    const int lane = threadIdx.x & 63;
    Counts n{};
    unsigned nlive = 0;
    Pipe S;
    S.groups = dispatch_round() * SEMTSDF_PRIO_EVERY;
    if (SEM && a.lut) S.lutv = reinterpret_cast<const uint32_t*>(a.lut)[lane];
    const unsigned* cnt = a.list_count;
    const unsigned* lst = a.units;
    unsigned n0;
    unsigned rot0 = 0;
    const bool split = (gridDim.x & 7u) == 0u;
    const unsigned nsp = split ? 8u : 1u, xi = split ? blockIdx.x & 7u : 0u;
    const unsigned wx = split ? __builtin_amdgcn_readfirstlane((blockIdx.x >> 3) * (blockDim.x >> 6) + (threadIdx.x >> 6))
                              : wave;
    const unsigned nwx = nwaves / nsp;
    if (GATE && !VOTE) {
        const __attribute__((address_space(4))) unsigned* u4 = (const __attribute__((address_space(4))) unsigned*)lst;
        const bool tab = split && a.first_nwaves == nwaves;
        const unsigned wq = min(wave, kPreWaves - 1u);
        const __attribute__((address_space(4))) unsigned* t4 =
            tab ? (const __attribute__((address_space(4))) unsigned*)a.first_tab : u4;
        const unsigned pre1[2] = {t4[2u * wq], t4[2u * wq + 1u]};
        ListView vf = list_view(lst, cnt, 2, wx, nwx, 0u, xi, nsp);
        ListView v1 = list_view(lst, cnt, 1, wx, nwx, 0u, xi, nsp);
        rot0 = (vf.cnt + v1.cnt) % nwx;
        ListView v0 = list_view(lst, cnt, 0, wx, nwx, rot0, xi, nsp);
        if (vf.i < vf.ngroups)
            list_prime<SEM, GATE, CI32, VOTE, COUNT, SHARD, PIN, 2>(a, ug, seg_cap, vf, S, n);
        else if (v1.i < v1.ngroups)
            list_prime<SEM, GATE, CI32, VOTE, COUNT, SHARD, PIN, 1>(a, ug, seg_cap, v1, S, n,
                                                                   (!split || tab) && wq == wave ? pre1 : nullptr);
        else if (v0.i < v0.ngroups)
            list_prime<SEM, GATE, CI32, VOTE, COUNT, SHARD, PIN, 0>(a, ug, seg_cap, v0, S, n);
        __syncthreads();
        if (SEMTSDF_WAVE_TRACE) tr[1] = tr[2] = tr[3] = wall_clock64();
        integrate_list<SEM, GATE, CI32, VOTE, COUNT, SHARD, PIN, 2, 1>(a, ug, seg_cap, s_rcp, vf, &v1, nwx, S, n);
        if (SEMTSDF_WAVE_TRACE) tr[2] = wall_clock64();
        integrate_list<SEM, GATE, CI32, VOTE, COUNT, SHARD, PIN, 1, 0>(a, ug, seg_cap, s_rcp, v1, &v0, nwx, S, n);
        if (SEMTSDF_WAVE_TRACE) {
            tr[3] = wall_clock64();
            trn = groups_of(vf.total, 0u) | (groups_of(v1.total, 0u) << 20);
        }
        integrate_list<SEM, GATE, CI32, VOTE, COUNT, SHARD, PIN, 0, -1>(a, ug, seg_cap, s_rcp, v0, nullptr, nwx, S, n);
        n0 = v0.total;
        if (COUNT && blockIdx.x == 0 && threadIdx.x == 0) {
            atomicAdd(a.counters + 4, (unsigned long long)(v1.total + vf.total));
            atomicAdd(a.counters + 5, (unsigned long long)vf.total);
        }
        if (COUNT) nlive += v1.total + vf.total;
    } else {
        const __attribute__((address_space(4))) unsigned* u4 = (const __attribute__((address_space(4))) unsigned*)lst;
        const bool tab = split && a.first_nwaves == nwaves;
        const unsigned wq = min(wave, kPreWaves - 1u);
        const __attribute__((address_space(4))) unsigned* t4 =
            tab ? (const __attribute__((address_space(4))) unsigned*)a.first_tab - 4 : u4;
        const unsigned pre0[2] = {t4[4u + 2u * wq], t4[5u + 2u * wq]};
        ListView v0 = list_view(lst, cnt, 0, wx, nwx, 0u, xi, nsp);
        if (v0.i < v0.ngroups)
            list_prime<SEM, GATE, CI32, VOTE, COUNT, SHARD, PIN, 0>(a, ug, seg_cap, v0, S, n,
                                                                   (tab || (!split && v0.list == lst + 4)) && wq == wave ? pre0
                                                                                                                : nullptr);
        __syncthreads();
        if (SEMTSDF_WAVE_TRACE) tr[1] = tr[2] = tr[3] = wall_clock64();
        integrate_list<SEM, GATE, CI32, VOTE, COUNT, SHARD, PIN, 0, -1>(a, ug, seg_cap, s_rcp, v0, nullptr, nwx, S, n);
        n0 = v0.total;
    }
    if (SEM && a.lut && a.relabel_mask) {
        const unsigned npx = (unsigned)(a.width * a.height);
        const unsigned gid = blockIdx.x * blockDim.x + threadIdx.x, nth = gridDim.x * blockDim.x;
        uint32_t* m4 = reinterpret_cast<uint32_t*>(a.relabel_mask);
        const bool al = ((uintptr_t)a.relabel_mask & 3u) == 0u;
        const unsigned n4 = al ? npx >> 2 : 0u;
        for (unsigned base = 0; base < n4; base += nth) {
            const unsigned i = base + gid;
            const uint32_t v = i < n4 ? m4[i] : 0u;
            uint32_t o = 0;
#pragma unroll
            for (int k = 0; k < 4; ++k) o |= (relabel_rec(v << (24 - 8 * k), S.lutv) >> 24) << (8 * k);
            if (i < n4) m4[i] = o;
        }
        for (unsigned base = n4 * 4; base < npx; base += nth) {
            const unsigned i = base + gid;
            const uint32_t v = i < npx ? (uint32_t)a.relabel_mask[i] : 0u;
            const uint32_t o = relabel_rec(v << 24, S.lutv) >> 24;
            if (i < npx) a.relabel_mask[i] = (uint8_t)o;
        }
    }
    if (SEMTSDF_WAVE_TRACE && a.wtrace && wave < a.wtrace_slots) {
        tr[4] = wall_clock64();
        trn |= groups_of(n0, rot0) << 40;
        if (lane < 8) {
            const unsigned long long hw = (unsigned long long)__smid() | ((unsigned long long)blockIdx.x << 32);
            const unsigned hwid = __builtin_amdgcn_s_getreg((4) | (0 << 6) | (31 << 11));
            const unsigned long long v = lane < 5 ? tr[lane < 5 ? lane : 0] : lane == 5 ? hw : lane == 6 ? trn : (unsigned long long)hwid;
            a.wtrace[(size_t)wave * kWaveTraceWords + lane] = v;
        }
    }
    if (COUNT) {
        nlive += n0;
        unsigned long long t = n.touch, gg = n.gate, tl = n.lines;
        for (int off = 32; off > 0; off >>= 1) {
            t += __shfl_xor(t, off, 64);
            gg += __shfl_xor(gg, off, 64);
            tl += __shfl_xor(tl, off, 64);
        }
        if (lane == 0) {
            if (t) atomicAdd(a.counters + 0, t);
            if (gg) atomicAdd(a.counters + 1, gg);
            if (tl) atomicAdd(a.counters + 7, tl);
        }
        if (blockIdx.x == 0 && threadIdx.x == 0) atomicAdd(a.counters + 3, (unsigned long long)nlive);
    }
}

static unsigned resident_grid_cus() {
    int dev = 0, cus = 0;
    if (hipGetDevice(&dev) != hipSuccess) return 256;
    if (hipDeviceGetAttribute(&cus, hipDeviceAttributeMultiprocessorCount, dev) != hipSuccess) return 256;
    return (unsigned)cus;
}

template <typename K>
static unsigned resident_grid(K kernel, int block = 256) {
    int dev = 0, cus = 0, per = 0;
    if (hipGetDevice(&dev) != hipSuccess) return 1024;
    if (hipDeviceGetAttribute(&cus, hipDeviceAttributeMultiprocessorCount, dev) != hipSuccess) return 1024;
    if (hipOccupancyMaxActiveBlocksPerMultiprocessor(&per, kernel, block, 0) != hipSuccess || per < 1) per = 1;
    return (unsigned)(cus * per);
}

template <bool SEM, bool GATE, bool CI32, bool VOTE, bool COUNT, bool SHARD, bool PIN>
static hipError_t launch_integrate_k(const IntegrateArgs& a, hipStream_t s, hipEvent_t e0, hipEvent_t e1) {
    const UnitGrid ug = unit_grid(a.g);
    if (ug.n == 0) return hipSuccess;
    constexpr int block = 256;
    static const unsigned grid0 = resident_grid(k_integrate<SEM, GATE, CI32, VOTE, COUNT, SHARD, PIN>, block);
    const unsigned ncu = resident_grid_cus();
    unsigned grid = grid0;
    if (kProbes && a.debug >= 100) grid = grid0 * (unsigned)(a.debug - 100) / 8u;
    static const char* gpc = getenv("SEMTSDF_GRID_PER_CU");
    if (gpc && atoi(gpc) > 0) grid = ncu * (unsigned)atoi(gpc);
    if (e0) {
        hipExtLaunchKernelGGL((k_integrate<SEM, GATE, CI32, VOTE, COUNT, SHARD, PIN>), dim3(grid), dim3(block), 0, s, e0,
                              e1, 0, a, ug, list_seg_cap(ug));
    } else {
        hipLaunchKernelGGL((k_integrate<SEM, GATE, CI32, VOTE, COUNT, SHARD, PIN>), dim3(grid), dim3(block), 0, s, a, ug,
                           list_seg_cap(ug));
    }
    return hipGetLastError();
}

template <bool SEM, bool GATE, bool CI32, bool VOTE>
static hipError_t launch_integrate_t(const IntegrateArgs& a, bool count, hipStream_t s, hipEvent_t e0, hipEvent_t e1) {
    const bool shard = a.g.nshards > 1, pin = a.pinhole != 0;
    if (count) {
        if (shard) return launch_integrate_k<SEM, GATE, CI32, VOTE, true, true, false>(a, s, e0, e1);
        return launch_integrate_k<SEM, GATE, CI32, VOTE, true, false, false>(a, s, e0, e1);
    }
    if (shard) {
        if (pin) return launch_integrate_k<SEM, GATE, CI32, VOTE, false, true, true>(a, s, e0, e1);
        return launch_integrate_k<SEM, GATE, CI32, VOTE, false, true, false>(a, s, e0, e1);
    }
    if (pin) return launch_integrate_k<SEM, GATE, CI32, VOTE, false, false, true>(a, s, e0, e1);
    return launch_integrate_k<SEM, GATE, CI32, VOTE, false, false, false>(a, s, e0, e1);
}

unsigned integrate_pre_waves() {
    static const unsigned w = 4u * resident_grid(k_integrate<true, true, false, false, false, false, true>, 256);
    return w <= kFirstTabSlots ? w : 0u;
}

hipError_t launch_integrate(const IntegrateArgs& a, hipStream_t s, hipEvent_t e0, hipEvent_t e1) {
    const bool count = a.counters != nullptr && (a.flags & 0x80000000u);
    const bool sem = a.flags & 0x1u, gate = a.flags & 0x2u, ci32 = a.color_wide != 0, vote = a.flags & 0x8u;
    if (vote) {
        if (ci32) return launch_integrate_t<false, false, true, true>(a, count, s, e0, e1);
        return launch_integrate_t<false, false, false, true>(a, count, s, e0, e1);
    }
    if (sem) {
        if (gate) {
            if (ci32) return launch_integrate_t<true, true, true, false>(a, count, s, e0, e1);
            return launch_integrate_t<true, true, false, false>(a, count, s, e0, e1);
        }
        if (ci32) return launch_integrate_t<true, false, true, false>(a, count, s, e0, e1);
        return launch_integrate_t<true, false, false, false>(a, count, s, e0, e1);
    }
    if (gate) {
        if (ci32) return launch_integrate_t<false, true, true, false>(a, count, s, e0, e1);
        return launch_integrate_t<false, true, false, false>(a, count, s, e0, e1);
    }
    if (ci32) return launch_integrate_t<false, false, true, false>(a, count, s, e0, e1);
    return launch_integrate_t<false, false, false, false>(a, count, s, e0, e1);
}

struct Tri {
    uint32_t i000;
    uint32_t dx, dy;
    uint32_t dz;
    float fx, fy, fz;
};

struct TriCoord {
    int xc, yc, zc, zl;
    int dxv, dyv, dzv;
    float fx, fy, fz;
};

template <bool SH = true>
__device__ __forceinline__ TriCoord tri_coord(const VolGeom& g, float px, float py, float pz) {
    const float ix = vox_coord(px, g.start[0], g.voxel[0], g.rvox[0]);
    const float iy = vox_coord(py, g.start[1], g.voxel[1], g.rvox[1]);
    const float iz = vox_coord(pz, g.start[2], g.voxel[2], g.rvox[2]);
    const float flx = floorf(ix), fly = floorf(iy), flz = floorf(iz);
    const float hx = (float)(g.dimx - 1), hy = (float)(g.dimy - 1), hz = (float)(g.dimz - 1);
    TriCoord c;
    c.fx = ix - flx;
    c.fy = iy - fly;
    c.fz = iz - flz;
    c.xc = (int)fminf(fmaxf(flx, 0.0f), hx);
    c.yc = (int)fminf(fmaxf(fly, 0.0f), hy);
    c.zc = (int)fminf(fmaxf(flz, 0.0f), hz);
    c.dxv = ((flx >= 0.0f) & (flx < hx)) ? 1 : 0;
    c.dyv = ((fly >= 0.0f) & (fly < hy)) ? 1 : 0;
    c.dzv = ((flz >= 0.0f) & (flz < hz)) ? 1 : 0;
    c.zl = (!SH || g.nshards == 1) ? c.zc : global_to_local_z(g, c.zc);
    return c;
}

__device__ __forceinline__ Tri tri_from(const VolGeom& g, const TriCoord& c) {
    Tri t;
    const uint32_t y0 = tile_yterm(g, c.yc), z0 = tile_zterm(c.zl);
    t.i000 = tile_xterm(g, c.xc) + y0 + z0;
    t.dx = c.dxv ? g.tx : 0u;
    t.dy = tile_yterm(g, c.yc + c.dyv) - y0;
    t.dz = tile_zterm(c.zl + c.dzv) - z0;
    t.fx = c.fx; t.fy = c.fy; t.fz = c.fz;
    return t;
}

template <bool SH = true>
__device__ __forceinline__ Tri tri_setup(const VolGeom& g, float px, float py, float pz) {
    return tri_from(g, tri_coord<SH>(g, px, py, pz));
}

__device__ __forceinline__ int brick_of(const VolGeom& g, const TriCoord& c) {
    return (int)__umul24(__umul24((unsigned)(c.xc >> 3), (unsigned)g.nby) + (unsigned)(c.yc >> 3), (unsigned)g.nbz) +
           (c.zl >> 3);
}

template <typename T>
__device__ __forceinline__ float tri_eval(const T* __restrict__ p, const Tri& t) {
    const T* q = p + t.i000;
    const float d0 = (float)q[0], d1 = (float)q[t.dz];
    const float d2 = (float)q[t.dy], d3 = (float)q[t.dy + t.dz];
    const float d4 = (float)q[t.dx], d5 = (float)q[t.dx + t.dz];
    const float d6 = (float)q[t.dx + t.dy], d7 = (float)q[t.dx + t.dy + t.dz];
    const float low = mixf(mixf(d0, d4, t.fx), mixf(d2, d6, t.fx), t.fy);
    const float high = mixf(mixf(d1, d5, t.fx), mixf(d3, d7, t.fx), t.fy);
    return mixf(low, high, t.fz);
}

__device__ __forceinline__ unsigned tri_bins(const uint32_t* __restrict__ hm, const Tri& t) {
    const uint32_t* q = hm + t.i000;
    return q[0] | q[t.dz] | q[t.dy] | q[t.dy + t.dz] | q[t.dx] | q[t.dx + t.dz] | q[t.dx + t.dy] |
           q[t.dx + t.dy + t.dz];
}

__device__ __forceinline__ unsigned tri_hist(const VolGeom& g, const VolBufs& b, const Tri& tr, float* p) {
    const unsigned bins = tri_bins(b.hmask, tr);
#pragma unroll
    for (int k = 0; k < kMaxObjects; ++k) p[k] = ((bins >> k) & 1u) ? tri_eval(b.hist + (uint64_t)k * g.nvox, tr) : 0.0f;
    return bins;
}

template <bool SH = true>
// ... 1081 lines not shown
    ray_render(a.cam, x, y, &ox, &oy, &oz, &dx, &dy, &dz);
    uint8_t b = 0, gch = 0, r = 0;
    float th = -1.0f;
    MarchStats ms;
    const uint64_t t_start = STATS ? __builtin_amdgcn_s_memrealtime() : 0;
    if (march_ray(a.g, a.b, ox, oy, oz, dx, dy, dz, &t, STATS ? &ms : nullptr)) {
        th = t;
        const Tri tr = tri_setup<false>(a.g, fmaf(t, dx, ox), fmaf(t, dy, oy), fmaf(t, dz, oz));
        shade_hit(a.g, a.b, tr, a.mode, a.color_i32, a.palette, &b, &gch, &r);
    }
    a.out_bgr[(size_t)px * 3 + 0] = b;
    a.out_bgr[(size_t)px * 3 + 1] = gch;
    a.out_bgr[(size_t)px * 3 + 2] = r;
    if (a.out_t) a.out_t[px] = th;
    if (STATS) {
        unsigned* q = a.ray_stats + (size_t)px * 4;
        q[0] = ms.iters; q[1] = ms.lookups; q[2] = ms.evals; q[3] = ms.skipped;
        const uint64_t t_end = __builtin_amdgcn_s_memrealtime();
        const size_t npx = (size_t)a.width * a.height;
        const unsigned wave = (unsigned)(by * ((a.width + 15) / 16) + bx) * 4 + (threadIdx.x >> 6);
        if ((threadIdx.x & 63) == 0) {
            unsigned long long* w = reinterpret_cast<unsigned long long*>(a.ray_stats + npx * 4) + wave * 2;
            w[0] = t_start;
            w[1] = t_end;
        }
    }
}

template <bool STATS>
__global__ __launch_bounds__(256) __attribute__((amdgpu_waves_per_eu(SEMTSDF_MARCH_WPE))) void k_render(RenderArgs a) {
    render_tile<STATS>(a, (int)blockIdx.x, (int)blockIdx.y);
}

#ifndef SEMTSDF_FUSED_WPE
#define SEMTSDF_FUSED_WPE 4
#endif
__global__ __launch_bounds__(256) __attribute__((amdgpu_waves_per_eu(SEMTSDF_FUSED_WPE))) void k_march_fused(
    AssocArgs aa, RenderArgs ra, int na, int nr) {
    __shared__ AssocLds s;
    const int b = aa.tile_perm ? (int)__builtin_amdgcn_readfirstlane(aa.tile_perm[blockIdx.x]) : (int)blockIdx.x;
    const int m = min(na, nr);
    const uint64_t t0 = aa.tile_cost ? __builtin_amdgcn_s_memrealtime() : 0;
    bool assoc;
    int t;
    if (b < 2 * m) {
        assoc = (b & 1) == 0;
        t = b >> 1;
    } else {
        assoc = na > nr;
        t = b - m;
    }
    if (assoc) {
        const int tx = (aa.width + 15) / 16;
        assoc_tile(aa, s, t % tx, t / tx);
    } else {
        const int tx = (ra.width + 15) / 16;
        render_tile<false>(ra, t % tx, t / tx);
    }
    if (aa.tile_cost) {
        __syncthreads();
        if (threadIdx.x == 0) aa.tile_cost[b] = (unsigned)min(__builtin_amdgcn_s_memrealtime() - t0, (uint64_t)0xFFFFFFFFu);
    }
}

hipError_t launch_march_fused(const AssocArgs& aa, const RenderArgs& ra, hipStream_t s) {
    const int na = ((aa.width + 15) / 16) * ((aa.height + 15) / 16);
    const int nr = ((ra.width + 15) / 16) * ((ra.height + 15) / 16);
    hipLaunchKernelGGL(k_march_fused, dim3(na + nr), dim3(256), 0, s, aa, ra, na, nr);
    return hipGetLastError();
}

hipError_t launch_render(const RenderArgs& a, hipStream_t s) {
    const dim3 grid((a.width + 15) / 16, (a.height + 15) / 16);
    if (a.ray_stats)
        hipLaunchKernelGGL(k_render<true>, grid, dim3(256), 0, s, a);
    else
        hipLaunchKernelGGL(k_render<false>, grid, dim3(256), 0, s, a);
    return hipGetLastError();
}

__device__ __forceinline__ float maps_sample(const VolGeom& g, const VolBufs& b, float px, float py, float pz,
                                             int* wmin) {
    const Tri tr = tri_setup<false>(g, px, py, pz);
    const int32_t* q = b.wt + tr.i000;
    const int w0 = min(min(q[0], q[tr.dz]), min(q[tr.dy], q[tr.dy + tr.dz]));
    const int w1 = min(min(q[tr.dx], q[tr.dx + tr.dz]), min(q[tr.dx + tr.dy], q[tr.dx + tr.dy + tr.dz]));
    *wmin = min(*wmin, min(w0, w1));
    return tri_eval(b.sdf, tr);
}

template <bool LABEL, bool NORMAL>
__global__ __launch_bounds__(256) __attribute__((amdgpu_waves_per_eu(SEMTSDF_MARCH_WPE))) void k_model_maps(MapsArgs a) {
    const int x = (int)blockIdx.x * 16 + (int)(threadIdx.x & 15);
    const int y = (int)blockIdx.y * 16 + (int)(threadIdx.x >> 4);
    if (x >= a.width || y >= a.height) return;
    const size_t px = (size_t)y * a.width + x;
    float ox, oy, oz, dx, dy, dz, t;
    ray_render(a.cam, x, y, &ox, &oy, &oz, &dx, &dy, &dz);
    float th = -1.0f, P[3] = {0.0f, 0.0f, 0.0f}, n[3] = {0.0f, 0.0f, 0.0f}, votes = 0.0f;
    int obj = 0;
    unsigned fl = 0;
    if (march_ray(a.g, a.b, ox, oy, oz, dx, dy, dz, &t, nullptr)) {
        th = t;
        fl = 1u;
        P[0] = fmaf(t, dx, ox);
        P[1] = fmaf(t, dy, oy);
        P[2] = fmaf(t, dz, oz);
        if (LABEL) {
            const Tri tr = tri_setup<false>(a.g, P[0], P[1], P[2]);
            unsigned bins = tri_bins(a.b.hmask, tr);
            while (bins) {
                const int k = __ffs((int)bins) - 1;
                bins &= bins - 1u;
                const float c = tri_eval(a.b.hist + (uint64_t)k * a.g.nvox, tr);
                if (c > votes) { votes = c; obj = k; }
            }
        }
        if (NORMAL) {
            int wmin = INT_MAX;
            float g0 = 0.0f, g1 = 0.0f, g2 = 0.0f;
#pragma unroll 1
            for (int ax = 0; ax < 3; ++ax) {
                const bool ax0 = ax == 0, ax1 = ax == 1, ax2 = ax == 2;
                const float v = ax0 ? a.g.voxel[0] : ax1 ? a.g.voxel[1] : a.g.voxel[2];
                const float pa = ax0 ? P[0] : ax1 ? P[1] : P[2];
                const float hi = pa + v, lo = pa - v;
                const float sp = maps_sample(a.g, a.b, ax0 ? hi : P[0], ax1 ? hi : P[1], ax2 ? hi : P[2], &wmin);
                const float sm = maps_sample(a.g, a.b, ax0 ? lo : P[0], ax1 ? lo : P[1], ax2 ? lo : P[2], &wmin);
                const float d = (sp - sm) / (v + v);
                g0 = ax0 ? d : g0;
                g1 = ax1 ? d : g1;
                g2 = ax2 ? d : g2;
            }
            const float n2 = dot3(g0, g1, g2, g0, g1, g2);
            if (wmin >= a.min_weight && n2 > 0.0f && n2 < __builtin_inff()) {
                const float inv = 1.0f / sqrtf(n2);
                n[0] = g0 * inv;
                n[1] = g1 * inv;
                n[2] = g2 * inv;
                fl |= 2u;
            }
        }
    }
    if (a.t) a.t[px] = th;
    if (a.point) {
        a.point[px * 3 + 0] = P[0];
        a.point[px * 3 + 1] = P[1];
        a.point[px * 3 + 2] = P[2];
    }
    if (LABEL) {
        if (a.label) a.label[px] = (uint8_t)obj;
        if (a.votes) a.votes[px] = votes;
    }
    if (NORMAL) {
        if (a.normal) {
            a.normal[px * 3 + 0] = n[0];
            a.normal[px * 3 + 1] = n[1];
            a.normal[px * 3 + 2] = n[2];
        }
        if (a.flags) a.flags[px] = (uint8_t)fl;
    }
}

hipError_t launch_model_maps(const MapsArgs& a, hipStream_t s) {
    const dim3 grid((a.width + 15) / 16, (a.height + 15) / 16);
    const bool lab = a.label || a.votes, nor = a.normal || a.flags;
    if (lab && nor)
        hipLaunchKernelGGL((k_model_maps<true, true>), grid, dim3(256), 0, s, a);
    else if (lab)
// ... 516 lines not shown
}

hipError_t launch_shard_render_final(const ShardRayArgs& a, hipStream_t s) {
    hipLaunchKernelGGL(k_shard_render_final, tile_grid(a.width, a.height), dim3(256), 0, s, a);
    return hipGetLastError();
}

hipError_t launch_shard_render_finish(const ShardRayArgs& a, hipStream_t s) {
    const int npx = a.width * a.height;
    int blocks = (npx + 255) / 256;
    if (blocks > 1024) blocks = 1024;
    hipLaunchKernelGGL(k_shard_render_finish, dim3(blocks), dim3(256), 0, s, a);
    return hipGetLastError();
}

hipError_t launch_shard_assoc_partial(const ShardRayArgs& a, hipStream_t s) {
    hipLaunchKernelGGL(k_shard_assoc_partial, tile_grid(a.width, a.height), dim3(256), 0, s, a);
    return hipGetLastError();
}

hipError_t launch_tables_from_partial(const long long* reduced, AssocTables* t, hipStream_t s) {
    hipLaunchKernelGGL(k_tables_from_partial, dim3(1), dim3(256), 0, s, reduced, t);
    return hipGetLastError();
}

__device__ __forceinline__ uint64_t tile_of_ref(const VolGeom& g, uint64_t v) {
    const uint64_t row = v / (uint64_t)g.lz;
    const int z = (int)(v - row * (uint64_t)g.lz);
    const int x = (int)(row / (uint64_t)g.dimy), y = (int)(row - (uint64_t)x * g.dimy);
    return tile_index(g, x, y, z);
}

__global__ __launch_bounds__(256) void k_hist_mask(VolGeom g, const uint32_t* __restrict__ hist,
                                                   uint32_t* __restrict__ hmask) {
    for (uint64_t v = (uint64_t)blockIdx.x * blockDim.x + threadIdx.x; v < g.nvox; v += (uint64_t)gridDim.x * blockDim.x) {
        unsigned m = 0;
        for (int k = 0; k < kMaxObjects; ++k) m |= (hist[(uint64_t)k * g.nvox + v] != 0u ? 1u : 0u) << k;
        hmask[v] = m;
    }
}

hipError_t launch_hist_mask(const VolGeom& g, const VolBufs& b, hipStream_t s) {
    if (!b.hist || !b.hmask || g.nvox == 0) return hipSuccess;
    uint64_t blocks = (g.nvox + 255) / 256;
    if (blocks > 16384) blocks = 16384;
    hipLaunchKernelGGL(k_hist_mask, dim3((unsigned)blocks), dim3(256), 0, s, g, b.hist, b.hmask);
    return hipGetLastError();
}

__global__ __launch_bounds__(256) void k_hist_to_vm(VolGeom g, const uint32_t* __restrict__ bm, uint32_t* __restrict__ vm,
                                                    uint64_t v0, uint64_t nv) {
    for (uint64_t i = (uint64_t)blockIdx.x * blockDim.x + threadIdx.x; i < nv * kMaxObjects;
         i += (uint64_t)gridDim.x * blockDim.x) {
        const uint64_t v = v0 + i / kMaxObjects, k = i % kMaxObjects;
        vm[i] = bm[k * g.nvox + tile_of_ref(g, v)];
    }
}

__global__ __launch_bounds__(256) void k_hist_to_bm(VolGeom g, const uint32_t* __restrict__ vm, uint32_t* __restrict__ bm,
                                                    uint64_t v0, uint64_t nv) {
    for (uint64_t i = (uint64_t)blockIdx.x * blockDim.x + threadIdx.x; i < nv * kMaxObjects;
         i += (uint64_t)gridDim.x * blockDim.x) {
        const uint64_t k = i / nv, v = v0 + i % nv;
        bm[k * g.nvox + tile_of_ref(g, v)] = vm[(v - v0) * kMaxObjects + k];
    }
}

hipError_t launch_hist_chunk_to_vm(const uint32_t* bm, uint32_t* vm, const VolGeom& g, uint64_t v0, uint64_t nv,
                                   hipStream_t s) {
    uint64_t blocks = (nv * kMaxObjects + 255) / 256;
    if (blocks > 16384) blocks = 16384;
    hipLaunchKernelGGL(k_hist_to_vm, dim3((unsigned)blocks), dim3(256), 0, s, g, bm, vm, v0, nv);
    return hipGetLastError();
}

hipError_t launch_hist_chunk_to_bm(const uint32_t* vm, uint32_t* bm, const VolGeom& g, uint64_t v0, uint64_t nv,
                                   hipStream_t s) {
    uint64_t blocks = (nv * kMaxObjects + 255) / 256;
    if (blocks > 16384) blocks = 16384;
    hipLaunchKernelGGL(k_hist_to_bm, dim3((unsigned)blocks), dim3(256), 0, s, g, vm, bm, v0, nv);
    return hipGetLastError();
}

__global__ __launch_bounds__(256) void k_vox_to_ref(VolGeom g, const uint32_t* __restrict__ dev, uint32_t* __restrict__ ref,
                                                    uint64_t v0, uint64_t nv) {
    for (uint64_t i = (uint64_t)blockIdx.x * blockDim.x + threadIdx.x; i < nv; i += (uint64_t)gridDim.x * blockDim.x)
        ref[i] = dev[tile_of_ref(g, v0 + i)];
}

__global__ __launch_bounds__(256) void k_vox_from_ref(VolGeom g, const uint32_t* __restrict__ ref, uint32_t* __restrict__ dev,
                                                      uint64_t v0, uint64_t nv) {
    for (uint64_t i = (uint64_t)blockIdx.x * blockDim.x + threadIdx.x; i < nv; i += (uint64_t)gridDim.x * blockDim.x)
        dev[tile_of_ref(g, v0 + i)] = ref[i];
}

hipError_t launch_vox_chunk(const void* src, void* dst, bool to_ref, const VolGeom& g, uint64_t v0, uint64_t nv,
                            hipStream_t s) {
    uint64_t blocks = (nv + 255) / 256;
    if (blocks > 16384) blocks = 16384;
    if (blocks == 0) return hipSuccess;
    if (to_ref)
        hipLaunchKernelGGL(k_vox_to_ref, dim3((unsigned)blocks), dim3(256), 0, s, g, (const uint32_t*)src, (uint32_t*)dst, v0, nv);
    else
        hipLaunchKernelGGL(k_vox_from_ref, dim3((unsigned)blocks), dim3(256), 0, s, g, (const uint32_t*)src, (uint32_t*)dst, v0, nv);
    return hipGetLastError();
}

template <typename TD, typename TR>
__global__ __launch_bounds__(256) void k_color_to_ref(VolGeom g, const TD* __restrict__ dev, TR* __restrict__ ref,
                                                      uint64_t v0, uint64_t nv) {
    for (uint64_t i = (uint64_t)blockIdx.x * blockDim.x + threadIdx.x; i < nv * 3; i += (uint64_t)gridDim.x * blockDim.x) {
        const uint64_t v = v0 + i / 3, c = i % 3;
        ref[i] = (TR)dev[tile_of_ref(g, v) * 4 + c];
    }
}

template <typename TD, typename TR>
__global__ __launch_bounds__(256) void k_color_from_ref(VolGeom g, const TR* __restrict__ ref, TD* __restrict__ dev,
                                                        uint64_t v0, uint64_t nv) {
    for (uint64_t i = (uint64_t)blockIdx.x * blockDim.x + threadIdx.x; i < nv * 3; i += (uint64_t)gridDim.x * blockDim.x) {
        const uint64_t v = v0 + i / 3, c = i % 3;
        dev[tile_of_ref(g, v) * 4 + c] = (TD)ref[i];
    }
}

__global__ __launch_bounds__(256) void k_color_widen(const uint32_t* __restrict__ narrow, int4* __restrict__ wide,
                                                     uint64_t nvox) {
    for (uint64_t v = (uint64_t)blockIdx.x * blockDim.x + threadIdx.x; v < nvox; v += (uint64_t)gridDim.x * blockDim.x) {
        const uint32_t c = narrow[v];
        wide[v] = make_int4((int)(c & 0xFFu), (int)((c >> 8) & 0xFFu), (int)((c >> 16) & 0xFFu), 0);
    }
}

hipError_t launch_color_widen(const uint8_t* narrow, int32_t* wide, uint64_t nvox, hipStream_t s) {
    if (nvox == 0) return hipSuccess;
    uint64_t blocks = (nvox + 255) / 256;
    if (blocks > 65536) blocks = 65536;
    hipLaunchKernelGGL(k_color_widen, dim3((unsigned)blocks), dim3(256), 0, s, reinterpret_cast<const uint32_t*>(narrow),
                       reinterpret_cast<int4*>(wide), nvox);
    return hipGetLastError();
}

template <typename TD, typename TR>
static void color_chunk_t(const void* src, void* dst, bool to_ref, const VolGeom& g, uint64_t v0, uint64_t nv,
                          dim3 gr, hipStream_t s) {
    if (to_ref)
        hipLaunchKernelGGL((k_color_to_ref<TD, TR>), gr, dim3(256), 0, s, g, (const TD*)src, (TR*)dst, v0, nv);
    else
        hipLaunchKernelGGL((k_color_from_ref<TD, TR>), gr, dim3(256), 0, s, g, (const TR*)src, (TD*)dst, v0, nv);
}

hipError_t launch_color_chunk(const void* src, void* dst, bool to_ref, bool ref_i32, bool dev_i32, const VolGeom& g,
                              uint64_t v0, uint64_t nv, hipStream_t s) {
    uint64_t blocks = (nv * 3 + 255) / 256;
    if (blocks > 16384) blocks = 16384;
    const dim3 gr((unsigned)blocks);
    if (dev_i32)
        color_chunk_t<int32_t, int32_t>(src, dst, to_ref, g, v0, nv, gr, s);
    else if (ref_i32)
        color_chunk_t<uint8_t, int32_t>(src, dst, to_ref, g, v0, nv, gr, s);
    else
        color_chunk_t<uint8_t, uint8_t>(src, dst, to_ref, g, v0, nv, gr, s);
    return hipGetLastError();
}


struct MaskScratch {
    unsigned area[kMaxDetections];
    unsigned short rank[kMaxDetections];
    unsigned char label[kMaxDetections];
    unsigned n_kept;
};

__global__ __launch_bounds__(256) void k_mask_areas(const uint8_t* __restrict__ masks, int npx, int n,
                                                     MaskScratch* __restrict__ sc) {
    __shared__ unsigned s_area[kMaxDetections];
    for (int i = threadIdx.x; i < n; i += blockDim.x) s_area[i] = 0u;
    __syncthreads();
    const int lane = threadIdx.x & 63;
    for (int base = blockIdx.x * blockDim.x; base < npx; base += gridDim.x * blockDim.x) {
        const int p = base + (int)threadIdx.x;
        const uint8_t* row = masks + (size_t)p * n;
        for (int i = 0; i < n; ++i) {
            const bool on = p < npx && row[i] != 0;
            const unsigned c = (unsigned)__popcll(__ballot(on));
            if (lane == 0 && c) atomicAdd(&s_area[i], c);
        }
    }
    __syncthreads();
    for (int i = threadIdx.x; i < n; i += blockDim.x)
        if (s_area[i]) atomicAdd(&sc->area[i], s_area[i]);
}

__global__ __launch_bounds__(256) void k_mask_decide(MaskScratch* __restrict__ sc, int n, int min_area) {
    const int i = threadIdx.x;
    __shared__ unsigned s_area[kMaxDetections];
    __shared__ unsigned char s_keep[kMaxDetections];
    if (i < n) {
        s_area[i] = sc->area[i];
        s_keep[i] = (long long)sc->area[i] > (long long)min_area ? 1 : 0;
    }
    __syncthreads();
    if (i < n) {
        unsigned rank = 0, before = 0;
        for (int j = 0; j < n; ++j) {
            if (!s_keep[j]) continue;
            rank += (s_area[j] < s_area[i] || (s_area[j] == s_area[i] && j < i)) ? 1u : 0u;
            before += j < i ? 1u : 0u;
        }
        sc->rank[i] = s_keep[i] ? (unsigned short)rank : (unsigned short)0xFFFF;
        sc->label[i] = (unsigned char)(before + 1);
    }
    if (i == 0) {
        unsigned k = 0;
// ... 118 lines not shown
        const int p = base + (int)threadIdx.x;
        bool on = false;
        if (p < total) {
            const int ry = p / cw;
            on = paste_on(m, mh, mw, b, sy, sx, cy0 + ry, cx0 + (p - ry * cw));
        }
        count += (unsigned)__popcll(__ballot(on));
    }
    if ((threadIdx.x & 63) == 0 && count) atomicAdd(&s_count, count);
    __syncthreads();
    if (threadIdx.x == 0 && s_count) atomicAdd(&sc->area[i], s_count);
}

__global__ __launch_bounds__(256) void k_paste_labels(const PasteBox* __restrict__ boxes, const void* __restrict__ mini,
                                                      int dtype, int mh, int mw, int n, int width, int height,
                                                      const MaskScratch* __restrict__ sc, uint8_t* __restrict__ out,
                                                      unsigned* __restrict__ areas) {
    __shared__ PasteBox s_box[kMaxDetections];
    __shared__ float s_sy[kMaxDetections], s_sx[kMaxDetections];
    __shared__ unsigned short s_idx[kMaxDetections];
    __shared__ unsigned char s_label[kMaxDetections];
    for (int i = threadIdx.x; i < n; i += 256) {
        const unsigned r = sc->rank[i];
        if (r != 0xFFFFu) {
            const PasteBox b = boxes[i];
            s_box[r] = b;
            s_sy[r] = paste_scale(mh, (long long)b.y2 - b.y1);
            s_sx[r] = paste_scale(mw, (long long)b.x2 - b.x1);
            s_idx[r] = (unsigned short)i;
            s_label[r] = sc->label[i];
        }
        if (areas && blockIdx.x == 0) areas[i] = sc->area[i];
    }
    __syncthreads();
    const int kept = (int)sc->n_kept;
    const int p = blockIdx.x * 256 + (int)threadIdx.x;
    if (p >= width * height) return;
    const int y = p / width, x = p - y * width;
    const int msz = mh * mw;
    unsigned char lab = 0;
    for (int r = 0; r < kept; ++r) {
        const PasteBox b = s_box[r];
        if (y < b.y1 || y >= b.y2 || x < b.x1 || x >= b.x2) continue;
        const MiniGlobal m{(const char*)mini + (size_t)s_idx[r] * msz * (dtype == 2 ? 4 : 2), dtype};
        if (paste_on(m, mh, mw, b, s_sy[r], s_sx[r], y, x)) {
            lab = s_label[r];
            break;
        }
    }
    out[p] = lab;
}

hipError_t launch_detections_to_labels(const int32_t* boxes, const void* mini, int dtype, int mh, int mw, int n,
                                       int width, int height, int min_area, void* scratch, uint8_t* out,
                                       uint32_t* areas, hipStream_t s) {
    static_assert(sizeof(PasteBox) == 4 * sizeof(int32_t), "boxes are [n][4] int32");
    MaskScratch* sc = (MaskScratch*)scratch;
    const PasteBox* b = (const PasteBox*)boxes;
    hipLaunchKernelGGL(k_paste_clear, dim3(1), dim3(kMaxDetections), 0, s, sc);
    if (n > 0)
        hipLaunchKernelGGL(k_paste_areas, dim3(kPasteAreaBlocks, n), dim3(256), 0, s, b, mini, dtype, mh, mw, width,
                           height, sc);
    hipLaunchKernelGGL(k_mask_decide, dim3(1), dim3(kMaxDetections), 0, s, sc, n, min_area);
    const int blocks = (width * height + 255) / 256;
    hipLaunchKernelGGL(k_paste_labels, dim3(blocks), dim3(256), 0, s, b, mini, dtype, mh, mw, n, width, height,
                       (const MaskScratch*)sc, out, areas);
    return hipGetLastError();
}



__global__ __launch_bounds__(256) void k_export_surface(VolGeom g, VolBufs b, float sdf_max, int min_w, int color_wide,
                                                        int semantic, SurfacePoint* __restrict__ out, uint64_t cap,
                                                        unsigned long long* __restrict__ count) {
    const uint64_t n = (uint64_t)g.dimx * (uint64_t)g.dimy * (uint64_t)g.lz;
    for (uint64_t v = blockIdx.x * (uint64_t)blockDim.x + threadIdx.x; v < n; v += (uint64_t)gridDim.x * blockDim.x) {
        const uint64_t row = v / (uint64_t)g.lz;
        const int l = (int)(v - row * (uint64_t)g.lz);
        const int x = (int)(row / (uint64_t)g.dimy), y = (int)(row - (uint64_t)x * g.dimy);
        if (g.nshards > 1 && (l % (g.chunk + g.halo)) >= g.chunk) continue;
        const int gz = local_to_global_z(g, l);
        if (gz >= g.dimz) continue;
        const uint32_t t = tile_index(g, x, y, l);
        const int w = b.wt[t];
        const float s = b.sdf[t];
        if (w < min_w || !(fabsf(s) < sdf_max)) continue;
        unsigned r, gg, bb;
        if (color_wide) {
            const int4 c = reinterpret_cast<const int4*>(b.color)[t];
            r = (unsigned)min(max(c.x, 0), 255); gg = (unsigned)min(max(c.y, 0), 255); bb = (unsigned)min(max(c.z, 0), 255);
        } else {
            const unsigned c = reinterpret_cast<const uint32_t*>(b.color)[t];
            r = c & 0xFFu; gg = (c >> 8) & 0xFFu; bb = (c >> 16) & 0xFFu;
        }
        unsigned lab = 0, best = 0;
        if (semantic) {
            unsigned bins = b.hmask[t];
            while (bins) {
                const int k = __ffs((int)bins) - 1;
                bins &= bins - 1u;
                const unsigned c = b.hist[(uint64_t)k * g.nvox + t];
                if (c > best) { best = c; lab = (unsigned)k; }
            }
        }
        const unsigned long long i = atomicAdd(count, 1ull);
        if (out && i < cap) {
            SurfacePoint p;
            p.x = (uint32_t)x; p.y = (uint32_t)y; p.z = (uint32_t)gz;
            p.sdf = s;
            p.rgbl = r | (gg << 8) | (bb << 16) | (lab << 24);
            out[i] = p;
        }
    }
}

hipError_t launch_export_surface(const VolGeom& g, const VolBufs& b, float sdf_max, int min_w, int color_wide,
                                 int semantic, SurfacePoint* out, uint64_t cap, unsigned long long* count, hipStream_t s) {
    const uint64_t n = (uint64_t)g.dimx * g.dimy * g.lz;
    if (n == 0) return hipSuccess;
    const uint64_t blocks = (n + 255) / 256;
    hipLaunchKernelGGL(k_export_surface, dim3((unsigned)(blocks < 65536 ? blocks : 65536)), dim3(256), 0, s, g, b, sdf_max,
                       min_w, color_wide, semantic, out, cap, count);
    return hipGetLastError();
}

struct MeshTable {
    uint8_t v[6][4];
    uint8_t n[6][16];
    uint8_t e[6][16][6];
    int bad;
};

constexpr MeshTable make_mesh_table() {
    MeshTable T{};
    const int perms[6][3] = {{0, 1, 2}, {0, 2, 1}, {1, 0, 2}, {1, 2, 0}, {2, 0, 1}, {2, 1, 0}};
    for (int t = 0; t < 6; ++t) {
        int V[4][3] = {};
        for (int i = 0; i < 3; ++i) {
            for (int a = 0; a < 3; ++a) V[i + 1][a] = V[i][a];
            V[i + 1][perms[t][i]] += 1;
        }
        for (int i = 0; i < 4; ++i) T.v[t][i] = (uint8_t)(V[i][0] | V[i][1] << 1 | V[i][2] << 2);
        for (int s = 0; s < 16; ++s) {
            int neg[4] = {}, pos[4] = {}, nn = 0, np = 0;
            for (int i = 0; i < 4; ++i) {
                if (s >> i & 1) neg[nn++] = i;
                else pos[np++] = i;
            }
            int tri[2][3][2] = {};
            int nt = 0;
            if (nn == 1) {
                for (int k = 0; k < 3; ++k) { tri[0][k][0] = neg[0]; tri[0][k][1] = pos[k]; }
                nt = 1;
            } else if (nn == 3) {
                for (int k = 0; k < 3; ++k) { tri[0][k][0] = pos[0]; tri[0][k][1] = neg[k]; }
                nt = 1;
            } else if (nn == 2) {
                const int A = neg[0], B = neg[1], C = pos[0], D = pos[1];
                const int q[2][3][2] = {{{A, C}, {A, D}, {B, D}}, {{A, C}, {B, D}, {B, C}}};
                for (int j = 0; j < 2; ++j)
                    for (int k = 0; k < 3; ++k) { tri[j][k][0] = q[j][k][0]; tri[j][k][1] = q[j][k][1]; }
                nt = 2;
            }
            T.n[t][s] = (uint8_t)nt;
            int want[3] = {};
            for (int a = 0; a < 3; ++a) {
                for (int i = 0; i < np; ++i) want[a] += V[pos[i]][a] * nn;
// ... 23 lines not shown
__constant__ MeshTable kMesh = make_mesh_table();

constexpr int kMeshHY = 10;
constexpr int kMeshHZ = 40;

__device__ __forceinline__ unsigned mesh_block_scan(unsigned val, unsigned* s_w, unsigned* tot) {
    const int lane = threadIdx.x & 63, w = threadIdx.x >> 6;
    unsigned incl = val;
    for (int off = 1; off < 64; off <<= 1) {
        const unsigned n = __shfl_up(incl, off);
        if (lane >= off) incl += n;
    }
    if (lane == 63) s_w[w] = incl;
    __syncthreads();
    unsigned pre = 0, t = 0;
    for (int i = 0; i < 4; ++i) {
        const unsigned c = s_w[i];
        pre += i < w ? c : 0u;
        t += c;
    }
    __syncthreads();
    *tot = t;
    return pre + incl - val;
}

__device__ __forceinline__ unsigned mesh_tet_case(unsigned signs, int t) {
    unsigned s = 0;
    for (int i = 0; i < 4; ++i) s |= ((signs >> kMesh.v[t][i]) & 1u) << i;
    return s;
}

__device__ __forceinline__ unsigned mesh_voxel_rgbl(const VolGeom& g, const VolBufs& b, uint32_t t, int color_wide,
                                                    int semantic) {
    unsigned r, gg, bb;
    if (color_wide) {
        const int4 c = reinterpret_cast<const int4*>(b.color)[t];
        r = (unsigned)min(max(c.x, 0), 255); gg = (unsigned)min(max(c.y, 0), 255); bb = (unsigned)min(max(c.z, 0), 255);
    } else {
        const unsigned c = reinterpret_cast<const uint32_t*>(b.color)[t];
        r = c & 0xFFu; gg = (c >> 8) & 0xFFu; bb = (c >> 16) & 0xFFu;
    }
    unsigned lab = 0, best = 0;
    if (semantic) {
        unsigned bins = b.hmask[t];
        while (bins) {
            const int k = __ffs((int)bins) - 1;
            bins &= bins - 1u;
            const unsigned c = b.hist[(uint64_t)k * g.nvox + t];
            if (c > best) { best = c; lab = (unsigned)k; }
        }
    }
    return r | (gg << 8) | (bb << 16) | (lab << 24);
}

template <int EMIT>
__global__ __launch_bounds__(256) void k_mesh_classify(VolGeom g, VolBufs b, int min_w, int color_wide, int semantic,
                                                       uint2* __restrict__ cnt, unsigned long long* __restrict__ gsum,
                                                       uint32_t* __restrict__ alist, const ulonglong2* __restrict__ base,
                                                       uint32_t* __restrict__ vtab, MeshVertexRec* __restrict__ verts) {
    constexpr int NL = kMeshXB + 2;
    __shared__ uint8_t s_f[NL][kMeshHY][kMeshHZ];
    __shared__ float s_s[EMIT ? NL : 1][EMIT ? kMeshHY : 1][EMIT ? kMeshHZ : 1];
    __shared__ uint8_t s_cv[kMeshXB + 1][9][36];
    __shared__ unsigned s_w[4];
    const unsigned tid = threadIdx.x;
    const unsigned tiles_x = g.nuz * g.nuy;
    const unsigned bid = EMIT ? mesh_list_blocks(g, alist)[blockIdx.x] : blockIdx.x;
    const unsigned tyz = bid % tiles_x;
    const int zt = (int)(tyz % g.nuz), yt = (int)(tyz / g.nuz), x0 = (int)(bid / tiles_x) * kMeshXB;
    const int nx = min(kMeshXB, g.dimx - x0);
    const int y0 = yt * 8, z0 = zt * 32;
    int has_neg = 0, has_pos = 0;
    for (int i = (int)tid; i < NL * kMeshHY * kMeshHZ; i += 256) {
        const int dx = i / (kMeshHY * kMeshHZ), r = i - dx * (kMeshHY * kMeshHZ);
        const int zg = r / (kMeshHY * 4), r2 = r - zg * (kMeshHY * 4);
        const int hy = r2 >> 2, hz = zg * 4 + (r2 & 3);
        const int X = x0 + dx - 1, Y = y0 - 1 + hy, L = z0 - 4 + hz;
        unsigned f = 0;
        float s = 0.0f;
        if (hz >= 3 && hz <= 36 && X >= 0 && X < g.dimx && Y >= 0 && Y < g.dimy && L >= 0 && L < g.lz &&
            local_to_global_z(g, L) < g.dimz) {
            const uint32_t t = tile_index(g, X, Y, L);
            s = b.sdf[t];
            const unsigned ok = b.wt[t] >= min_w ? 1u : 0u, ng = s < 0.0f ? 1u : 0u;
            f = ok | (ng << 1);
            has_neg |= (int)(ok & ng);
            has_pos |= (int)(ok & (ng ^ 1u));
        }
        s_f[dx][hy][hz] = (uint8_t)f;
        if constexpr (EMIT != 0) s_s[dx][hy][hz] = s;
    }
    const int any_neg = __syncthreads_or(has_neg);
    const int any_pos = __syncthreads_or(has_pos);
    if (!any_neg || !any_pos) {
        if (!EMIT && (int)tid < nx) cnt[(unsigned)(x0 + (int)tid) * tiles_x + tyz] = make_uint2(0u, 0u);
        return;
    }
    const int per = g.chunk + g.halo;
    for (int i = (int)tid; i < (kMeshXB + 1) * 9 * 33; i += 256) {
        const int cx = i / (9 * 33), r = i - cx * (9 * 33);
        const int cy = r / 33, cz = r - cy * 33;
        const int L = z0 - 1 + cz;
        unsigned v = (L >= 0 && (g.nshards == 1 || (L % per) < g.chunk)) ? 1u : 0u;
        for (int p = 0; p < 8; ++p) v &= s_f[cx + (p & 1)][cy + ((p >> 1) & 1)][3 + cz + (p >> 2)];
        s_cv[cx][cy][cz] = (uint8_t)v;
    }
    __syncthreads();
    const int zi = (int)((tid >> 5) * 4 + (tid & 3)), yi = (int)((tid >> 2) & 7);
    const int hy = yi + 1, hz = zi + 4;
    bool listed = false;
    for (int j = 0; j < nx; ++j) {
        const int x = x0 + j;
        const unsigned blk = (unsigned)x * tiles_x + tyz;
        if (EMIT) {
            const uint2 c = cnt[blk];
            if ((c.x | c.y) == 0u) continue;
        }
        unsigned signs = 0;
        for (int p = 0; p < 8; ++p)
            signs |= ((unsigned)(s_f[j + 1 + (p & 1)][hy + ((p >> 1) & 1)][hz + (p >> 2)] >> 1) & 1u) << p;
        const unsigned valid = s_cv[j + 1][yi + 1][zi + 1];
        unsigned mask = 0;
        for (int c = 1; c < 8; ++c) {
            if ((((signs >> c) ^ signs) & 1u) == 0u) continue;
            const int ex = c & 1, ey = (c >> 1) & 1, ez = c >> 2;
            unsigned any = 0;
            for (int mx = ex; mx < 2; ++mx)
                for (int my = ey; my < 2; ++my)
                    for (int mz = ez; mz < 2; ++mz) any |= s_cv[j + mx][yi + my][zi + mz];
            mask |= any << c;
        }
        unsigned ntri = 0;
        if (valid)
            for (int t = 0; t < 6; ++t) ntri += kMesh.n[t][mesh_tet_case(signs, t)];
        const unsigned nv = (unsigned)__popc(mask);
        unsigned tot;
        const unsigned pre = mesh_block_scan(nv | (ntri << 16), s_w, &tot);
        if constexpr (!EMIT) {
            if (tid == 0) {
                cnt[blk] = make_uint2(tot & 0xFFFFu, tot >> 16);
                if (tot) {
                    atomicAdd(&gsum[2u * (blk / kMeshGroup)], (unsigned long long)(tot & 0xFFFFu));
                    atomicAdd(&gsum[2u * (blk / kMeshGroup) + 1u], (unsigned long long)(tot >> 16));
                }
                if (tot >> 16) mesh_list_tiles(g, alist)[atomicAdd(&alist[1], 1u)] = blk;
                if (tot && !listed) {
                    listed = true;
                    mesh_list_blocks(g, alist)[atomicAdd(&alist[0], 1u)] = bid;
                }
            }
        } else {
            const uint32_t t0 = blk * 256u + tid;
            vtab[t0] = valid | mask | ((pre & 0xFFFFu) << 8) | (signs << 19);
            const int y = y0 + yi, l = z0 + zi;
            const int gz = local_to_global_z(g, l);
            uint64_t vi = base[blk].x + (pre & 0xFFFFu);
            const float s0 = s_s[j + 1][hy][hz];
            for (int c = 1; c < 8; ++c) {
                if (!((mask >> c) & 1u)) continue;
                const int ex = c & 1, ey = (c >> 1) & 1, ez = c >> 2;
                const float s1 = s_s[j + 1 + ex][hy + ey][hz + ez];
                const float t = __fdiv_rn(s0, __fsub_rn(s0, s1));
                const float px = __fadd_rn(__fmul_rn(__fadd_rn((float)x, ex ? t : 0.0f), g.voxel[0]), g.start[0]);
                const float py = __fadd_rn(__fmul_rn(__fadd_rn((float)y, ey ? t : 0.0f), g.voxel[1]), g.start[1]);
                const float pz = __fadd_rn(__fmul_rn(__fadd_rn((float)gz, ez ? t : 0.0f), g.voxel[2]), g.start[2]);
                const bool own = fabsf(s0) <= fabsf(s1);
                const uint32_t ta = own ? t0 : tile_index(g, x + ex, y + ey, l + ez);
// ... 56 lines not shown
    unsigned tot;
    const unsigned pre = mesh_block_scan(ntri, s_w, &tot);
    if (!ntri) return;
    const int zt = (int)(blk % g.nuz), yt = (int)((blk / g.nuz) % g.nuy), x = (int)(blk / (g.nuz * g.nuy));
    const int y = yt * 8 + (int)((tid >> 2) & 7), l = zt * 32 + (int)((tid >> 5) * 4 + (tid & 3));
    for (int p = 0; p < 7; ++p) {
        const uint32_t t = tile_index(g, x + (p & 1), y + ((p >> 1) & 1), l + (p >> 2));
        const uint32_t wp = vtab[t];
        s_first[p][tid] = (uint32_t)(base[t >> 8].x + ((wp >> 8) & 0x7FFu));
        s_mask[p][tid] = (uint8_t)(wp & 0xFEu);
    }
    uint64_t ti = (base[blk].y + pre) * 3u;
    for (int t = 0; t < 6; ++t) {
        const unsigned s = mesh_tet_case(signs, t);
        const unsigned n = kMesh.n[t][s];
        for (unsigned j = 0; j < n * 3u; ++j) {
            const unsigned e = kMesh.e[t][s][j];
            const unsigned p = e & 7u, c = e >> 3;
            tris[ti++] = s_first[p][tid] + (unsigned)__popc(s_mask[p][tid] & ((1u << c) - 1u));
        }
    }
}

hipError_t launch_mesh_count(const VolGeom& g, const VolBufs& b, int min_w, uint2* cnt, unsigned long long* gsum,
                             uint32_t* alist, ulonglong2* base, unsigned long long* tot, hipStream_t s) {
    const unsigned nb = (unsigned)mesh_blocks(g), ng = (unsigned)mesh_groups(g);
    hipError_t e = hipMemsetAsync(gsum, 0, (size_t)ng * 2 * sizeof(unsigned long long), s);
    if (e == hipSuccess) e = hipMemsetAsync(alist, 0, 2 * sizeof(uint32_t), s);
    if (e != hipSuccess) return e;
    hipLaunchKernelGGL(k_mesh_classify<0>, dim3(mesh_classify_blocks(g)), dim3(256), 0, s, g, b, min_w, 0, 0, cnt, gsum,
                       alist, (const ulonglong2*)nullptr, (uint32_t*)nullptr, (MeshVertexRec*)nullptr);
    hipLaunchKernelGGL(k_mesh_scan, dim3(ng), dim3(256), 0, s, (const uint2*)cnt, (const unsigned long long*)gsum, base,
                       nb, tot);
    return hipGetLastError();
}

hipError_t launch_mesh_emit(const VolGeom& g, const VolBufs& b, int min_w, int color_wide, int semantic,
                            const uint2* cnt, const uint32_t* alist, unsigned nblocks, unsigned ntiles,
                            const ulonglong2* base, uint32_t* vtab, MeshVertexRec* verts, uint32_t* tris, hipStream_t s) {
    if (nblocks > mesh_classify_blocks(g) || ntiles > mesh_blocks(g)) return hipErrorInvalidValue;
    if (nblocks)
        hipLaunchKernelGGL(k_mesh_classify<1>, dim3(nblocks), dim3(256), 0, s, g, b, min_w, color_wide, semantic,
                           const_cast<uint2*>(cnt), (unsigned long long*)nullptr, const_cast<uint32_t*>(alist), base, vtab,
                           verts);
    if (ntiles) hipLaunchKernelGGL(k_mesh_triangles, dim3(ntiles), dim3(256), 0, s, g, alist, base, vtab, tris);
    return hipGetLastError();
}

constexpr int kInstSums = 9;
static_assert(offsetof(InstanceRec, min) == kInstSums * 8 && sizeof(InstanceRec) == 96, "InstanceRec layout");
constexpr unsigned kInstBlocks = 2048;

__global__ __launch_bounds__(256) void k_instance_clear(InstanceRec* __restrict__ rec,
                                                        unsigned long long* __restrict__ overlap) {
    const unsigned tid = threadIdx.x;
    if (tid < kMaxObjects) {
        InstanceRec r{};
        r.min[0] = r.min[1] = r.min[2] = 0xFFFFFFFFu;
        rec[tid] = r;
    }
    if (overlap)
        for (unsigned i = tid; i < kMaxObjects * kMaxObjects; i += 256u) overlap[i] = 0ull;
}

__global__ __launch_bounds__(256) void k_instance_stats(VolGeom g, VolBufs b, float sdf_max, int min_w, int color_wide,
                                                        InstanceRec* __restrict__ rec,
                                                        unsigned long long* __restrict__ overlap) {
    __shared__ unsigned long long s_sum[kMaxObjects][kInstSums];
    __shared__ unsigned s_min[kMaxObjects][3], s_max[kMaxObjects][3];
    __shared__ unsigned s_ov[kMaxObjects * kMaxObjects];
    const unsigned tid = threadIdx.x;
    for (unsigned i = tid; i < kMaxObjects * kInstSums; i += 256u) (&s_sum[0][0])[i] = 0ull;
    for (unsigned i = tid; i < kMaxObjects * 3; i += 256u) { (&s_min[0][0])[i] = 0xFFFFFFFFu; (&s_max[0][0])[i] = 0u; }
    for (unsigned i = tid; i < kMaxObjects * kMaxObjects; i += 256u) s_ov[i] = 0u;
    __syncthreads();
    const unsigned ntiles = (unsigned)(g.nvox >> 8), tiles_x = g.nuy * g.nuz;
    const unsigned lane = tid & 63u;
    const int yi = (int)(lane & 7u), zq = (int)(lane >> 3);
    const int per = g.chunk + g.halo;
    for (unsigned tile = __builtin_amdgcn_readfirstlane(blockIdx.x * 4u + (tid >> 6)); tile < ntiles;
         tile += gridDim.x * 4u) {
        const uint32_t t0 = tile * 256u + lane * 4u;
        const float4 s4 = reinterpret_cast<const float4*>(b.sdf)[t0 >> 2];
        const int4 w4 = reinterpret_cast<const int4*>(b.wt)[t0 >> 2];
        const float sv[4] = {s4.x, s4.y, s4.z, s4.w};
        const int wv[4] = {w4.x, w4.y, w4.z, w4.w};
        unsigned sel = 0;
#pragma unroll
        for (int j = 0; j < 4; ++j) sel |= (wv[j] >= min_w && fabsf(sv[j]) < sdf_max ? 1u : 0u) << j;
        if (!sel) continue;
        const unsigned x = tile / tiles_x, r = tile - x * tiles_x;
        const unsigned yt = r / g.nuz, zt = r - yt * g.nuz;
        const int y = (int)yt * 8 + yi;
        if (y >= g.dimy) continue;
#pragma unroll
        for (int j = 0; j < 4; ++j) {
            if (!((sel >> j) & 1u)) continue;
            const int l = (int)zt * 32 + zq * 4 + j;
            if (l >= g.lz) continue;
            if (g.nshards > 1 && (l % per) >= g.chunk) continue;
            const int gz = local_to_global_z(g, l);
            if (gz >= g.dimz) continue;
            const uint32_t t = t0 + (uint32_t)j;
            const unsigned bins = b.hmask[t];
            unsigned lab = 0, best = 0;
            for (unsigned m = bins; m; m &= m - 1u) {
                const int k = __ffs((int)m) - 1;
                const unsigned c = b.hist[(uint64_t)k * g.nvox + t];
                if (c > best) { best = c; lab = (unsigned)k; }
                atomicAdd(&s_sum[k][2], 1ull);
                if (overlap)
                    for (unsigned m2 = bins; m2; m2 &= m2 - 1u) atomicAdd(&s_ov[k * kMaxObjects + (__ffs((int)m2) - 1)], 1u);
            }
            unsigned cr, cg, cb;
            if (color_wide) {
                const int4 c = reinterpret_cast<const int4*>(b.color)[t];
                cr = (unsigned)min(max(c.x, 0), 255); cg = (unsigned)min(max(c.y, 0), 255); cb = (unsigned)min(max(c.z, 0), 255);
            } else {
                const unsigned c = reinterpret_cast<const uint32_t*>(b.color)[t];
                cr = c & 0xFFu; cg = (c >> 8) & 0xFFu; cb = (c >> 16) & 0xFFu;
            }
            unsigned long long* a = s_sum[lab];
            atomicAdd(&a[0], 1ull);
            atomicAdd(&a[1], (unsigned long long)best);
            atomicAdd(&a[3], (unsigned long long)x);
            atomicAdd(&a[4], (unsigned long long)y);
            atomicAdd(&a[5], (unsigned long long)gz);
            atomicAdd(&a[6], (unsigned long long)cr);
            atomicAdd(&a[7], (unsigned long long)cg);
            atomicAdd(&a[8], (unsigned long long)cb);
            atomicMin(&s_min[lab][0], x); atomicMin(&s_min[lab][1], (unsigned)y); atomicMin(&s_min[lab][2], (unsigned)gz);
            atomicMax(&s_max[lab][0], x); atomicMax(&s_max[lab][1], (unsigned)y); atomicMax(&s_max[lab][2], (unsigned)gz);
        }
    }
    __syncthreads();
    for (unsigned i = tid; i < kMaxObjects * kInstSums; i += 256u) {
        const unsigned long long v = (&s_sum[0][0])[i];
        if (v) atomicAdd(reinterpret_cast<unsigned long long*>(&rec[i / kInstSums]) + i % kInstSums, v);
    }
    if (tid < kMaxObjects * 3) {
        const unsigned k = tid / 3u, a = tid - k * 3u;
        if (s_min[k][a] != 0xFFFFFFFFu) {
            atomicMin(&rec[k].min[a], s_min[k][a]);
            atomicMax(&rec[k].max[a], s_max[k][a]);
        }
    }
    if (overlap)
        for (unsigned i = tid; i < kMaxObjects * kMaxObjects; i += 256u)
            if (s_ov[i]) atomicAdd(&overlap[i], (unsigned long long)s_ov[i]);
}

hipError_t launch_instance_stats(const VolGeom& g, const VolBufs& b, float sdf_max, int min_w, int color_wide,
                                 InstanceRec* rec, unsigned long long* overlap, hipStream_t s) {
    hipLaunchKernelGGL(k_instance_clear, dim3(1), dim3(256), 0, s, rec, overlap);
    const uint64_t blocks = ((g.nvox >> 8) + 3u) / 4u;
    if (blocks)
        hipLaunchKernelGGL(k_instance_stats, dim3((unsigned)(blocks < kInstBlocks ? blocks : kInstBlocks)), dim3(256), 0, s,
                           g, b, sdf_max, min_w, color_wide, rec, overlap);
    return hipGetLastError();
}

__device__ __forceinline__ unsigned remap_lut(const RemapLut& L, int k) {
    const unsigned long long w = k < 16 ? (k < 8 ? L.w[0] : L.w[1]) : (k < 24 ? L.w[2] : L.w[3]);
    return (unsigned)(w >> ((k & 7) * 8)) & 0xFFu;
}

__global__ __launch_bounds__(256) void k_remap_instances(VolGeom g, uint32_t* hist, uint32_t* __restrict__ hmask,
// ... 44 lines not shown
```

Baseline: 1.610 million Mvoxel-updates/s.

## Store TSDF weights as uint16 with on-demand widening to int32

The per-voxel weight array is now stored as 16-bit unsigned by default, and every kernel reading it (integrate, maps sampling, meshing, instance stats, transfers) is templated or branched on a wide flag. If the running weight bound could exceed 65535, or uploaded weights do not fit, the volume is widened to int32 once. This halves weight read and write traffic in the memory-bound integrate kernel. The cost is an extra template dimension, a runtime branch in the non-templated readers, and the code needed to widen and narrow the buffer.

```diff
diff --git a/__graft_entry__.py b/__graft_entry__.py
--- a/__graft_entry__.py
+++ b/__graft_entry__.py
@@ -21,7 +21,7 @@
 
 def _lib_sources():
     srcs = [os.path.join(CSRC, f) for f in ("semtsdf_kernels.hip", "semtsdf_api.cpp")]
-    hdrs = [os.path.join(CSRC, f) for f in ("semtsdf_internal.h", "semtsdf_libm.h", "semtsdf_steps.h")]
+    hdrs = [os.path.join(CSRC, f) for f in ("semtsdf_internal.h", "semtsdf_libm.h", "semtsdf_steps.h", "semtsdf_wscan.h")]
     return srcs, srcs + hdrs + [os.path.join(ROOT, "include", "semtsdf.h")]
 
 
diff --git a/slam-maskrcnn_amd/csrc/semtsdf_api.cpp b/slam-maskrcnn_amd/csrc/semtsdf_api.cpp
--- a/slam-maskrcnn_amd/csrc/semtsdf_api.cpp
+++ b/slam-maskrcnn_amd/csrc/semtsdf_api.cpp
@@ -12,6 +12,7 @@
 
 #include "../../include/semtsdf.h"
 #include "semtsdf_internal.h"
+#include "semtsdf_wscan.h"
 
 using namespace semtsdf;
 
@@ -115,6 +116,7 @@
     bool multi_stream = false;
     bool color_wide = false;
     int64_t wmax_bound = 0;
+    bool wt_wide = false;
     const uint8_t* pending_lut = nullptr;
     unsigned long long* wtrace_d = nullptr;
     unsigned* tile_cost_d = nullptr;
@@ -291,6 +293,19 @@
     return SEMTSDF_OK;
 }
 
+int widen_weights(semtsdf_vol* v, hipStream_t s) {
+    if (v->wt_wide) return SEMTSDF_OK;
+    void* wide = nullptr;
+    if (int rc = dev_alloc(v, &wide, v->g.nvox * 4)) return rc;
+    HIPC(launch_weight_widen(static_cast<const uint16_t*>(v->b.wt), static_cast<int32_t*>(wide), v->g.nvox, s));
+    HIPC(hipStreamSynchronize(s));
+    HIPC(hipFree(v->b.wt));
+    v->device_bytes -= v->g.nvox * 2;
+    v->b.wt = wide;
+    v->wt_wide = true;
+    v->b.wt_wide = 1;
+    return SEMTSDF_OK;
+}
 
 int ensure_prep_stream(semtsdf_vol* v) {
     if (v->prep_stream) return SEMTSDF_OK;
@@ -313,6 +328,9 @@
     if ((v->p.flags & SEMTSDF_F_VOTE) && !cls_d) return fail(SEMTSDF_ERR_INVALID, "vote volume needs cls");
     if ((v->p.flags & SEMTSDF_F_COLOR_I32) && !v->color_wide && v->wmax_bound + 1 >= (1ll << 23)) {
         if (int rc = widen_color(v, s)) return rc;
+    }
+    if (!v->wt_wide && v->wmax_bound + 1 > kNarrowWeightMax) {
+        if (int rc = widen_weights(v, s)) return rc;
     }
     IntegrateArgs a{};
     a.g = v->g;
@@ -843,7 +861,7 @@
         return bail(fail(SEMTSDF_ERR_HIP, "hipStreamCreate failed"));
     const bool ci32 = p->flags & SEMTSDF_F_COLOR_I32;
     if ((rc = dev_alloc(v, (void**)&v->b.sdf, n * 4))) return bail(rc);
-    if ((rc = dev_alloc(v, (void**)&v->b.wt, n * 4))) return bail(rc);
+    if ((rc = dev_alloc(v, &v->b.wt, n * 2))) return bail(rc);
     if ((rc = dev_alloc(v, (void**)&v->b.sflag, n / 32 + 1))) return bail(rc);
     const size_t nbricks = (size_t)g.nbx * g.nby * g.nbz;
     if ((rc = dev_alloc(v, (void**)&v->b.bplain, nbricks * 4))) return bail(rc);
@@ -969,7 +987,17 @@
     const size_t n = v->g.nvox;
     if (int rc = after_maps(v, s)) return rc;
     HIPC(launch_fill_volume(v->g, v->b, v->p.flags, s));
-    HIPC(hipMemsetAsync(v->b.wt, 0, n * 4, s));
+    if (v->wt_wide) {
+        void* narrow = nullptr;
+        if (int rc = dev_alloc(v, &narrow, n * 2)) return rc;
+        HIPC(hipStreamSynchronize(s));
+        HIPC(hipFree(v->b.wt));
+        v->device_bytes -= n * 4;
+        v->b.wt = narrow;
+        v->wt_wide = false;
+        v->b.wt_wide = 0;
+    }
+    HIPC(hipMemsetAsync(v->b.wt, 0, n * 2, s));
     HIPC(hipMemsetAsync(v->b.sflag, 0, n / 32 + 1, s));
     HIPC(hipMemsetAsync(v->b.color, 0, v->g.nvox * 4 * (v->color_wide ? 4 : 1), s));
     if (v->b.hist) HIPC(hipMemsetAsync(v->b.hist, 0, v->g.nvox * kMaxObjects * 4, s));
@@ -1894,7 +1922,7 @@
 static uint64_t nref(const semtsdf_vol* v) { return (uint64_t)v->g.dimx * v->g.dimy * v->g.lz; }
 
 static int vox_xfer(semtsdf_vol* v, void* host, void* dev, bool to_host, const char* what, hipStream_t s, uint64_t vb,
-                    uint64_t ve) {
+                    uint64_t ve, bool dev_u16 = false) {
     if (ve <= vb) return SEMTSDF_OK;
     const uint64_t chunk = std::min<uint64_t>(ve - vb, 1ull << 26);
     void* stage = nullptr;
@@ -1904,11 +1932,11 @@
         char* h = static_cast<char*>(host) + (v0 - vb) * 4;
         hipError_t e;
         if (to_host) {
-            e = launch_vox_chunk(dev, stage, true, v->g, v0, nv, s);
+            e = launch_vox_chunk(dev, stage, true, v->g, v0, nv, s, dev_u16);
             if (e == hipSuccess) e = hipMemcpyAsync(h, stage, nv * 4, hipMemcpyDeviceToHost, s);
         } else {
             e = hipMemcpyAsync(stage, h, nv * 4, hipMemcpyHostToDevice, s);
-            if (e == hipSuccess) e = launch_vox_chunk(stage, dev, false, v->g, v0, nv, s);
+            if (e == hipSuccess) e = launch_vox_chunk(stage, dev, false, v->g, v0, nv, s, dev_u16);
         }
         if (e == hipSuccess) e = hipStreamSynchronize(s);
         if (e != hipSuccess) {
@@ -1958,7 +1986,7 @@
     const uint64_t vb = (uint64_t)x0 * plane, ve = (uint64_t)x1 * plane;
     int rc;
     if (sdf && (rc = vox_xfer(v, sdf, v->b.sdf, true, "sdf", s, vb, ve))) return rc;
-    if (wt && (rc = vox_xfer(v, wt, v->b.wt, true, "weight", s, vb, ve))) return rc;
+    if (wt && (rc = vox_xfer(v, wt, v->b.wt, true, "weight", s, vb, ve, !v->wt_wide))) return rc;
     if (color) {
         rc = color_xfer(v, color, true, s, vb, ve);
         if (rc) return rc;
@@ -2009,11 +2037,12 @@
     v->maps_stale = true;
     if (sdf || wt) HIPC(hipMemsetAsync(v->b.sflag, 0, v->g.nvox / 32 + 1, s));
     if (sdf && (rc = vox_xfer(v, const_cast<float*>(sdf), v->b.sdf, false, "sdf", s, 0, nref(v)))) return rc;
-    if (wt && (rc = vox_xfer(v, const_cast<int32_t*>(wt), v->b.wt, false, "weight", s, 0, nref(v)))) return rc;
     if (wt) {
-        int64_t m = 0;
-        for (uint64_t i = 0, n = nref(v); i < n; ++i) m = std::max<int64_t>(m, wt[i]);
-        v->wmax_bound = m;
+        const WeightScan ws = scan_weights(wt, nref(v));
+        if (!ws.fits_u16 && (rc = widen_weights(v, s))) return rc;
+        rc = vox_xfer(v, const_cast<int32_t*>(wt), v->b.wt, false, "weight", s, 0, nref(v), !v->wt_wide);
+        if (rc) return rc;
+        v->wmax_bound = ws.wmax;
     }
     if (color) {
         if ((v->p.flags & SEMTSDF_F_COLOR_I32) && !v->color_wide) {
diff --git a/slam-maskrcnn_amd/csrc/semtsdf_internal.h b/slam-maskrcnn_amd/csrc/semtsdf_internal.h
--- a/slam-maskrcnn_amd/csrc/semtsdf_internal.h
+++ b/slam-maskrcnn_amd/csrc/semtsdf_internal.h
@@ -47,7 +47,7 @@
 
 struct VolBufs {
     float* sdf;
-    int32_t* wt;
+    void* wt;
     void* color;
     uint32_t* hist;
     uint32_t* hmask;
@@ -59,7 +59,12 @@
     uint32_t* bdirty;
     uint32_t* dlist;
     uint8_t* sflag;
-};
+    int wt_wide;
+};
+
+__device__ inline int wt_at(const VolBufs& b, uint32_t t) {
+    return b.wt_wide ? static_cast<const int32_t*>(b.wt)[t] : (int)static_cast<const uint16_t*>(b.wt)[t];
+}
 
 struct DepthPyramid {
     uint2* px;
@@ -312,7 +317,8 @@
                                 float scale, const DepthPyramid& p, unsigned* list_count, hipStream_t s,
                                 const uint8_t* lut = nullptr);
 hipError_t launch_vox_chunk(const void* src, void* dst, bool to_ref, const VolGeom& g, uint64_t v0, uint64_t nv,
-                            hipStream_t s);
+                            hipStream_t s, bool dev_u16 = false);
+hipError_t launch_weight_widen(const uint16_t* narrow, int32_t* wide, uint64_t nvox, hipStream_t s);
 hipError_t launch_color_widen(const uint8_t* narrow, int32_t* wide, uint64_t nvox, hipStream_t s);
 hipError_t launch_color_chunk(const void* src, void* dst, bool to_ref, bool ref_i32, bool dev_i32, const VolGeom& g,
                               uint64_t v0, uint64_t nv, hipStream_t s);
diff --git a/slam-maskrcnn_amd/csrc/semtsdf_kernels.hip b/slam-maskrcnn_amd/csrc/semtsdf_kernels.hip
--- a/slam-maskrcnn_amd/csrc/semtsdf_kernels.hip
+++ b/slam-maskrcnn_amd/csrc/semtsdf_kernels.hip
@@ -1033,8 +1033,23 @@
     static_assert(sizeof(T) == 16, "16-byte vectors");
     *reinterpret_cast<T*>(p) = v;
 }
-
-template <bool SEM, bool CI32, bool VOTE, bool FREE>
+template <bool WW>
+__device__ __forceinline__ int4 ld_weights(const void* wt, uint32_t v) {
+    if (WW) return ld_state<int4>(static_cast<const int32_t*>(wt) + v);
+    const uint2 p = *reinterpret_cast<const uint2*>(static_cast<const uint16_t*>(wt) + v);
+    return make_int4((int)(p.x & 0xFFFFu), (int)(p.x >> 16), (int)(p.y & 0xFFFFu), (int)(p.y >> 16));
+}
+template <bool WW>
+__device__ __forceinline__ void st_weights(void* wt, uint64_t v, const int4& w) {
+    if (WW) {
+        st_state(static_cast<int32_t*>(wt) + v, w);
+    } else {
+        *reinterpret_cast<uint2*>(static_cast<uint16_t*>(wt) + v) =
+            make_uint2((unsigned)w.x | ((unsigned)w.y << 16), (unsigned)w.z | ((unsigned)w.w << 16));
+    }
+}
+
+template <bool SEM, bool CI32, bool VOTE, bool FREE, bool WW>
 __device__ __forceinline__ void stage_load(const IntegrateArgs& a, const UnitPos& up, unsigned coff, const Cls& C,
                                            Ld& L) {
     const VolGeom& g = a.g;
@@ -1050,7 +1065,7 @@
     const bool skip = (C.sflag != 0u) & fone;
     L.skip = skip;
     L.s4 = ld_state<float4>(a.b.sdf + ((skip | !t) ? 0u : v));
-    L.w4 = ld_state<int4>(a.b.wt + (t ? v : 0u));
+    L.w4 = ld_weights<WW>(a.b.wt, t ? v : 0u);
     if (FREE) return;
     if (CI32) {
 #pragma unroll
@@ -1188,7 +1203,7 @@
     (void)__hip_atomic_fetch_add(p, v, __ATOMIC_RELAXED, __HIP_MEMORY_SCOPE_WORKGROUP);
 }
 
-template <bool SEM, bool CI32, bool VOTE, bool FREE>
+template <bool SEM, bool CI32, bool VOTE, bool FREE, bool WW>
 __device__ __forceinline__ void stage_store(const IntegrateArgs& a, const UnitPos& up, unsigned coff,
                                             const StoreMeta& M, const Out& O) {
     const VolGeom& g = a.g;
@@ -1220,7 +1235,7 @@
     const uint64_t v = O.ub + coff;
     if (!(kProbes && a.debug == 10) && tmask != 0u) {
         if (!O.skip) st_state(a.b.sdf + v, O.s4);
-        st_state(a.b.wt + v, O.w4);
+        st_weights<WW>(a.b.wt, v, O.w4);
     }
     {
         const unsigned s_and = __float_as_uint(O.s4.x) & __float_as_uint(O.s4.y) & __float_as_uint(O.s4.z) &
@@ -1345,7 +1360,7 @@
     static constexpr bool FREE = KIND != 0, FULL = KIND == 2;
 };
 
-template <bool SEM, bool GATE, bool CI32, bool VOTE, bool COUNT, bool SHARD, bool PIN, int KIND>
+template <bool SEM, bool GATE, bool CI32, bool VOTE, bool WW, bool COUNT, bool SHARD, bool PIN, int KIND>
 __device__ __forceinline__ void list_prime(const IntegrateArgs& a, const UnitGrid& ug, unsigned seg_cap,
                                            const ListView& v, Pipe& S, Counts& n, const unsigned* pre = nullptr) {
     constexpr bool FREE = KindOf<KIND>::FREE, FULL = KindOf<KIND>::FULL;
@@ -1361,7 +1376,7 @@
     S.cur = lane_pos(ug, e);
     stage_project<SHARD, PIN, FREE, FULL, VOTE>(a, S.cur, lane, S.P);
     stage_classify<SEM, GATE, VOTE, COUNT, FREE>(a, S.P, S.C, true, n.touch, n.gate, n.lines, S.lutv);
-    stage_load<SEM, CI32, VOTE, FREE>(a, S.cur, coff, S.C, S.L);
+    stage_load<SEM, CI32, VOTE, FREE, WW>(a, S.cur, coff, S.C, S.L);
     S.primed = true;
 }
 
@@ -1381,7 +1396,7 @@
     return __builtin_amdgcn_readfirstlane((blockIdx.x * 4u) / gridDim.x);
 }
 
-template <bool SEM, bool GATE, bool CI32, bool VOTE, bool COUNT, bool SHARD, bool PIN, int KIND, int NKIND>
+template <bool SEM, bool GATE, bool CI32, bool VOTE, bool WW, bool COUNT, bool SHARD, bool PIN, int KIND, int NKIND>
 __device__ __forceinline__ void integrate_list(const IntegrateArgs& a, const UnitGrid& ug, unsigned seg_cap,
                                                const float* __restrict__ s_rcp, ListView& v, const ListView* nx,
                                                unsigned nwaves, Pipe& S, Counts& n) {
@@ -1390,7 +1405,7 @@
     const int lane = threadIdx.x & 63;
     const unsigned coff = (unsigned)lane_zq(lane) * 32u + (unsigned)lane_y(lane) * 4u;
     if (v.i >= v.ngroups) return;
-    if (!S.primed) list_prime<SEM, GATE, CI32, VOTE, COUNT, SHARD, PIN, KIND>(a, ug, seg_cap, v, S, n);
+    if (!S.primed) list_prime<SEM, GATE, CI32, VOTE, WW, COUNT, SHARD, PIN, KIND>(a, ug, seg_cap, v, S, n);
     unsigned en[kSlots];
     if (v.i + nwaves < v.ngroups) group_entries(v, v.i + nwaves, seg_cap, en);
     const bool chain = NKIND >= 0 && nx->i < nx->ngroups;
@@ -1403,8 +1418,8 @@
         stage_compute<SEM, GATE, CI32, VOTE, FREE>(a, s_rcp, S.C, S.L, S.O);
         const StoreMeta Mc = store_meta(S.C);
         stage_classify<SEM, GATE, VOTE, COUNT, FREE>(a, S.P, S.C, true, n.touch, n.gate, n.lines, S.lutv);
-        stage_store<SEM, CI32, VOTE, FREE>(a, S.cur, coff, Mc, S.O);
-        stage_load<SEM, CI32, VOTE, FREE>(a, nxt, coff, S.C, S.L);
+        stage_store<SEM, CI32, VOTE, FREE, WW>(a, S.cur, coff, Mc, S.O);
+        stage_load<SEM, CI32, VOTE, FREE, WW>(a, nxt, coff, S.C, S.L);
         S.cur = nxt;
         v.i += nwaves;
         ++S.groups;
@@ -1417,13 +1432,13 @@
         stage_compute<SEM, GATE, CI32, VOTE, FREE>(a, s_rcp, S.C, S.L, S.O);
         const StoreMeta Mc = store_meta(S.C);
         stage_classify<SEM, GATE, VOTE, COUNT, NFREE>(a, S.P, S.C, true, n.touch, n.gate, n.lines, S.lutv);
-        stage_store<SEM, CI32, VOTE, FREE>(a, S.cur, coff, Mc, S.O);
-        stage_load<SEM, CI32, VOTE, NFREE>(a, nxt, coff, S.C, S.L);
+        stage_store<SEM, CI32, VOTE, FREE, WW>(a, S.cur, coff, Mc, S.O);
+        stage_load<SEM, CI32, VOTE, NFREE, WW>(a, nxt, coff, S.C, S.L);
         S.cur = nxt;
         S.primed = true;
     } else {
         stage_compute<SEM, GATE, CI32, VOTE, FREE>(a, s_rcp, S.C, S.L, S.O);
-        stage_store<SEM, CI32, VOTE, FREE>(a, S.cur, coff, store_meta(S.C), S.O);
+        stage_store<SEM, CI32, VOTE, FREE, WW>(a, S.cur, coff, store_meta(S.C), S.O);
         S.primed = false;
     }
     v.i += nwaves;
@@ -1432,10 +1447,9 @@
 #ifndef SEMTSDF_INTEGRATE_WPE
 #define SEMTSDF_INTEGRATE_WPE 4
 #endif
-template <bool SEM, bool GATE, bool CI32, bool VOTE, bool COUNT, bool SHARD, bool PIN>
-__global__ __launch_bounds__(256) __attribute__((amdgpu_waves_per_eu(VOTE ? 3 : SEMTSDF_INTEGRATE_WPE))) void k_integrate(
-    IntegrateArgs a, UnitGrid ug, unsigned seg_cap) {
-    __shared__ float s_rcp[kRcpTable];
+template <bool SEM, bool GATE, bool CI32, bool VOTE, bool WW, bool COUNT, bool SHARD, bool PIN>
+__device__ __forceinline__ void integrate_body(const IntegrateArgs& a, const UnitGrid& ug, unsigned seg_cap,
+                                               float* s_rcp) {
     unsigned long long tr[5] = {0, 0, 0, 0, 0};
     unsigned long long trn = 0;
     const unsigned nwaves = gridDim.x * (blockDim.x >> 6);
@@ -1473,22 +1487,22 @@
         rot0 = (vf.cnt + v1.cnt) % nwx;
         ListView v0 = list_view(lst, cnt, 0, wx, nwx, rot0, xi, nsp);
         if (vf.i < vf.ngroups)
-            list_prime<SEM, GATE, CI32, VOTE, COUNT, SHARD, PIN, 2>(a, ug, seg_cap, vf, S, n);
+            list_prime<SEM, GATE, CI32, VOTE, WW, COUNT, SHARD, PIN, 2>(a, ug, seg_cap, vf, S, n);
         else if (v1.i < v1.ngroups)
-            list_prime<SEM, GATE, CI32, VOTE, COUNT, SHARD, PIN, 1>(a, ug, seg_cap, v1, S, n,
+            list_prime<SEM, GATE, CI32, VOTE, WW, COUNT, SHARD, PIN, 1>(a, ug, seg_cap, v1, S, n,
                                                                    (!split || tab) && wq == wave ? pre1 : nullptr);
         else if (v0.i < v0.ngroups)
-            list_prime<SEM, GATE, CI32, VOTE, COUNT, SHARD, PIN, 0>(a, ug, seg_cap, v0, S, n);
+            list_prime<SEM, GATE, CI32, VOTE, WW, COUNT, SHARD, PIN, 0>(a, ug, seg_cap, v0, S, n);
         __syncthreads();
         if (SEMTSDF_WAVE_TRACE) tr[1] = tr[2] = tr[3] = wall_clock64();
-        integrate_list<SEM, GATE, CI32, VOTE, COUNT, SHARD, PIN, 2, 1>(a, ug, seg_cap, s_rcp, vf, &v1, nwx, S, n);
+        integrate_list<SEM, GATE, CI32, VOTE, WW, COUNT, SHARD, PIN, 2, 1>(a, ug, seg_cap, s_rcp, vf, &v1, nwx, S, n);
         if (SEMTSDF_WAVE_TRACE) tr[2] = wall_clock64();
-        integrate_list<SEM, GATE, CI32, VOTE, COUNT, SHARD, PIN, 1, 0>(a, ug, seg_cap, s_rcp, v1, &v0, nwx, S, n);
+        integrate_list<SEM, GATE, CI32, VOTE, WW, COUNT, SHARD, PIN, 1, 0>(a, ug, seg_cap, s_rcp, v1, &v0, nwx, S, n);
         if (SEMTSDF_WAVE_TRACE) {
             tr[3] = wall_clock64();
             trn = groups_of(vf.total, 0u) | (groups_of(v1.total, 0u) << 20);
         }
-        integrate_list<SEM, GATE, CI32, VOTE, COUNT, SHARD, PIN, 0, -1>(a, ug, seg_cap, s_rcp, v0, nullptr, nwx, S, n);
+        integrate_list<SEM, GATE, CI32, VOTE, WW, COUNT, SHARD, PIN, 0, -1>(a, ug, seg_cap, s_rcp, v0, nullptr, nwx, S, n);
         n0 = v0.total;
         if (COUNT && blockIdx.x == 0 && threadIdx.x == 0) {
             atomicAdd(a.counters + 4, (unsigned long long)(v1.total + vf.total));
@@ -1504,12 +1518,12 @@
         const unsigned pre0[2] = {t4[4u + 2u * wq], t4[5u + 2u * wq]};
         ListView v0 = list_view(lst, cnt, 0, wx, nwx, 0u, xi, nsp);
         if (v0.i < v0.ngroups)
-            list_prime<SEM, GATE, CI32, VOTE, COUNT, SHARD, PIN, 0>(a, ug, seg_cap, v0, S, n,
+            list_prime<SEM, GATE, CI32, VOTE, WW, COUNT, SHARD, PIN, 0>(a, ug, seg_cap, v0, S, n,
                                                                    (tab || (!split && v0.list == lst + 4)) && wq == wave ? pre0
                                                                                                                 : nullptr);
         __syncthreads();
         if (SEMTSDF_WAVE_TRACE) tr[1] = tr[2] = tr[3] = wall_clock64();
-        integrate_list<SEM, GATE, CI32, VOTE, COUNT, SHARD, PIN, 0, -1>(a, ug, seg_cap, s_rcp, v0, nullptr, nwx, S, n);
+        integrate_list<SEM, GATE, CI32, VOTE, WW, COUNT, SHARD, PIN, 0, -1>(a, ug, seg_cap, s_rcp, v0, nullptr, nwx, S, n);
         n0 = v0.total;
     }
     if (SEM && a.lut && a.relabel_mask) {
@@ -1560,6 +1574,20 @@
     }
 }
 
+template <bool SEM, bool GATE, bool CI32, bool VOTE, bool COUNT, bool SHARD, bool PIN>
+__global__ __launch_bounds__(256) __attribute__((amdgpu_waves_per_eu(VOTE ? 3 : SEMTSDF_INTEGRATE_WPE))) void k_integrate(
+    IntegrateArgs a, UnitGrid ug, unsigned seg_cap) {
+    __shared__ float s_rcp[kRcpTable];
+    integrate_body<SEM, GATE, CI32, VOTE, false, COUNT, SHARD, PIN>(a, ug, seg_cap, s_rcp);
+}
+
+template <bool SEM, bool GATE, bool CI32, bool VOTE, bool COUNT, bool SHARD, bool PIN>
+__global__ __launch_bounds__(256) __attribute__((amdgpu_waves_per_eu(VOTE ? 3 : SEMTSDF_INTEGRATE_WPE))) void k_integrate_w(
+    IntegrateArgs a, UnitGrid ug, unsigned seg_cap) {
+    __shared__ float s_rcp[kRcpTable];
+    integrate_body<SEM, GATE, CI32, VOTE, true, COUNT, SHARD, PIN>(a, ug, seg_cap, s_rcp);
+}
+
 static unsigned resident_grid_cus() {
     int dev = 0, cus = 0;
     if (hipGetDevice(&dev) != hipSuccess) return 256;
@@ -1576,40 +1604,42 @@
     return (unsigned)(cus * per);
 }
 
-template <bool SEM, bool GATE, bool CI32, bool VOTE, bool COUNT, bool SHARD, bool PIN>
+template <bool SEM, bool GATE, bool CI32, bool VOTE, bool WW, bool COUNT, bool SHARD, bool PIN>
 static hipError_t launch_integrate_k(const IntegrateArgs& a, hipStream_t s, hipEvent_t e0, hipEvent_t e1) {
     const UnitGrid ug = unit_grid(a.g);
     if (ug.n == 0) return hipSuccess;
     constexpr int block = 256;
-    static const unsigned grid0 = resident_grid(k_integrate<SEM, GATE, CI32, VOTE, COUNT, SHARD, PIN>, block);
+    const auto kern = WW ? k_integrate_w<SEM, GATE, CI32, VOTE, COUNT, SHARD, PIN>
+                         : k_integrate<SEM, GATE, CI32, VOTE, COUNT, SHARD, PIN>;
+    static const unsigned grid0 = resident_grid(kern, block);
     const unsigned ncu = resident_grid_cus();
     unsigned grid = grid0;
     if (kProbes && a.debug >= 100) grid = grid0 * (unsigned)(a.debug - 100) / 8u;
     static const char* gpc = getenv("SEMTSDF_GRID_PER_CU");
     if (gpc && atoi(gpc) > 0) grid = ncu * (unsigned)atoi(gpc);
     if (e0) {
-        hipExtLaunchKernelGGL((k_integrate<SEM, GATE, CI32, VOTE, COUNT, SHARD, PIN>), dim3(grid), dim3(block), 0, s, e0,
+        hipExtLaunchKernelGGL(kern, dim3(grid), dim3(block), 0, s, e0,
                               e1, 0, a, ug, list_seg_cap(ug));
     } else {
-        hipLaunchKernelGGL((k_integrate<SEM, GATE, CI32, VOTE, COUNT, SHARD, PIN>), dim3(grid), dim3(block), 0, s, a, ug,
+        hipLaunchKernelGGL(kern, dim3(grid), dim3(block), 0, s, a, ug,
                            list_seg_cap(ug));
     }
     return hipGetLastError();
 }
 
-template <bool SEM, bool GATE, bool CI32, bool VOTE>
+template <bool SEM, bool GATE, bool CI32, bool VOTE, bool WW>
 static hipError_t launch_integrate_t(const IntegrateArgs& a, bool count, hipStream_t s, hipEvent_t e0, hipEvent_t e1) {
     const bool shard = a.g.nshards > 1, pin = a.pinhole != 0;
     if (count) {
-        if (shard) return launch_integrate_k<SEM, GATE, CI32, VOTE, true, true, false>(a, s, e0, e1);
-        return launch_integrate_k<SEM, GATE, CI32, VOTE, true, false, false>(a, s, e0, e1);
+        if (shard) return launch_integrate_k<SEM, GATE, CI32, VOTE, WW, true, true, false>(a, s, e0, e1);
+        return launch_integrate_k<SEM, GATE, CI32, VOTE, WW, true, false, false>(a, s, e0, e1);
     }
     if (shard) {
-        if (pin) return launch_integrate_k<SEM, GATE, CI32, VOTE, false, true, true>(a, s, e0, e1);
-        return launch_integrate_k<SEM, GATE, CI32, VOTE, false, true, false>(a, s, e0, e1);
-    }
-    if (pin) return launch_integrate_k<SEM, GATE, CI32, VOTE, false, false, true>(a, s, e0, e1);
-    return launch_integrate_k<SEM, GATE, CI32, VOTE, false, false, false>(a, s, e0, e1);
+        if (pin) return launch_integrate_k<SEM, GATE, CI32, VOTE, WW, false, true, true>(a, s, e0, e1);
+        return launch_integrate_k<SEM, GATE, CI32, VOTE, WW, false, true, false>(a, s, e0, e1);
+    }
+    if (pin) return launch_integrate_k<SEM, GATE, CI32, VOTE, WW, false, false, true>(a, s, e0, e1);
+    return launch_integrate_k<SEM, GATE, CI32, VOTE, WW, false, false, false>(a, s, e0, e1);
 }
 
 unsigned integrate_pre_waves() {
@@ -1617,27 +1647,32 @@
     return w <= kFirstTabSlots ? w : 0u;
 }
 
-hipError_t launch_integrate(const IntegrateArgs& a, hipStream_t s, hipEvent_t e0, hipEvent_t e1) {
+template <bool WW>
+static hipError_t launch_integrate_w(const IntegrateArgs& a, hipStream_t s, hipEvent_t e0, hipEvent_t e1) {
     const bool count = a.counters != nullptr && (a.flags & 0x80000000u);
     const bool sem = a.flags & 0x1u, gate = a.flags & 0x2u, ci32 = a.color_wide != 0, vote = a.flags & 0x8u;
     if (vote) {
-        if (ci32) return launch_integrate_t<false, false, true, true>(a, count, s, e0, e1);
-        return launch_integrate_t<false, false, false, true>(a, count, s, e0, e1);
+        if (ci32) return launch_integrate_t<false, false, true, true, WW>(a, count, s, e0, e1);
+        return launch_integrate_t<false, false, false, true, WW>(a, count, s, e0, e1);
     }
     if (sem) {
         if (gate) {
-            if (ci32) return launch_integrate_t<true, true, true, false>(a, count, s, e0, e1);
-            return launch_integrate_t<true, true, false, false>(a, count, s, e0, e1);
-        }
-        if (ci32) return launch_integrate_t<true, false, true, false>(a, count, s, e0, e1);
-        return launch_integrate_t<true, false, false, false>(a, count, s, e0, e1);
+            if (ci32) return launch_integrate_t<true, true, true, false, WW>(a, count, s, e0, e1);
+            return launch_integrate_t<true, true, false, false, WW>(a, count, s, e0, e1);
+        }
+        if (ci32) return launch_integrate_t<true, false, true, false, WW>(a, count, s, e0, e1);
+        return launch_integrate_t<true, false, false, false, WW>(a, count, s, e0, e1);
     }
     if (gate) {
-        if (ci32) return launch_integrate_t<false, true, true, false>(a, count, s, e0, e1);
-        return launch_integrate_t<false, true, false, false>(a, count, s, e0, e1);
-    }
-    if (ci32) return launch_integrate_t<false, false, true, false>(a, count, s, e0, e1);
-    return launch_integrate_t<false, false, false, false>(a, count, s, e0, e1);
+        if (ci32) return launch_integrate_t<false, true, true, false, WW>(a, count, s, e0, e1);
+        return launch_integrate_t<false, true, false, false, WW>(a, count, s, e0, e1);
+    }
+    if (ci32) return launch_integrate_t<false, false, true, false, WW>(a, count, s, e0, e1);
+    return launch_integrate_t<false, false, false, false, WW>(a, count, s, e0, e1);
+}
+
+hipError_t launch_integrate(const IntegrateArgs& a, hipStream_t s, hipEvent_t e0, hipEvent_t e1) {
+    return a.b.wt_wide ? launch_integrate_w<true>(a, s, e0, e1) : launch_integrate_w<false>(a, s, e0, e1);
 }
 
 struct Tri {
@@ -2885,9 +2920,10 @@
 __device__ __forceinline__ float maps_sample(const VolGeom& g, const VolBufs& b, float px, float py, float pz,
                                              int* wmin) {
     const Tri tr = tri_setup<false>(g, px, py, pz);
-    const int32_t* q = b.wt + tr.i000;
-    const int w0 = min(min(q[0], q[tr.dz]), min(q[tr.dy], q[tr.dy + tr.dz]));
-    const int w1 = min(min(q[tr.dx], q[tr.dx + tr.dz]), min(q[tr.dx + tr.dy], q[tr.dx + tr.dy + tr.dz]));
+    const uint32_t q = tr.i000;
+    const int w0 = min(min(wt_at(b, q), wt_at(b, q + tr.dz)), min(wt_at(b, q + tr.dy), wt_at(b, q + tr.dy + tr.dz)));
+    const int w1 = min(min(wt_at(b, q + tr.dx), wt_at(b, q + tr.dx + tr.dz)),
+                       min(wt_at(b, q + tr.dx + tr.dy), wt_at(b, q + tr.dx + tr.dy + tr.dz)));
     *wmin = min(*wmin, min(w0, w1));
     return tri_eval(b.sdf, tr);
 }
@@ -3570,27 +3606,33 @@
     return hipGetLastError();
 }
 
-__global__ __launch_bounds__(256) void k_vox_to_ref(VolGeom g, const uint32_t* __restrict__ dev, uint32_t* __restrict__ ref,
+template <typename TD>
+__global__ __launch_bounds__(256) void k_vox_to_ref(VolGeom g, const TD* __restrict__ dev, uint32_t* __restrict__ ref,
                                                     uint64_t v0, uint64_t nv) {
     for (uint64_t i = (uint64_t)blockIdx.x * blockDim.x + threadIdx.x; i < nv; i += (uint64_t)gridDim.x * blockDim.x)
         ref[i] = dev[tile_of_ref(g, v0 + i)];
 }
 
-__global__ __launch_bounds__(256) void k_vox_from_ref(VolGeom g, const uint32_t* __restrict__ ref, uint32_t* __restrict__ dev,
+template <typename TD>
+__global__ __launch_bounds__(256) void k_vox_from_ref(VolGeom g, const uint32_t* __restrict__ ref, TD* __restrict__ dev,
                                                       uint64_t v0, uint64_t nv) {
     for (uint64_t i = (uint64_t)blockIdx.x * blockDim.x + threadIdx.x; i < nv; i += (uint64_t)gridDim.x * blockDim.x)
-        dev[tile_of_ref(g, v0 + i)] = ref[i];
+        dev[tile_of_ref(g, v0 + i)] = (TD)ref[i];
 }
 
 hipError_t launch_vox_chunk(const void* src, void* dst, bool to_ref, const VolGeom& g, uint64_t v0, uint64_t nv,
-                            hipStream_t s) {
+                            hipStream_t s, bool dev_u16) {
     uint64_t blocks = (nv + 255) / 256;
     if (blocks > 16384) blocks = 16384;
     if (blocks == 0) return hipSuccess;
-    if (to_ref)
-        hipLaunchKernelGGL(k_vox_to_ref, dim3((unsigned)blocks), dim3(256), 0, s, g, (const uint32_t*)src, (uint32_t*)dst, v0, nv);
+    if (to_ref && dev_u16)
+        hipLaunchKernelGGL(k_vox_to_ref<uint16_t>, dim3((unsigned)blocks), dim3(256), 0, s, g, (const uint16_t*)src, (uint32_t*)dst, v0, nv);
+    else if (to_ref)
+        hipLaunchKernelGGL(k_vox_to_ref<uint32_t>, dim3((unsigned)blocks), dim3(256), 0, s, g, (const uint32_t*)src, (uint32_t*)dst, v0, nv);
+    else if (dev_u16)
+        hipLaunchKernelGGL(k_vox_from_ref<uint16_t>, dim3((unsigned)blocks), dim3(256), 0, s, g, (const uint32_t*)src, (uint16_t*)dst, v0, nv);
     else
-        hipLaunchKernelGGL(k_vox_from_ref, dim3((unsigned)blocks), dim3(256), 0, s, g, (const uint32_t*)src, (uint32_t*)dst, v0, nv);
+        hipLaunchKernelGGL(k_vox_from_ref<uint32_t>, dim3((unsigned)blocks), dim3(256), 0, s, g, (const uint32_t*)src, (uint32_t*)dst, v0, nv);
     return hipGetLastError();
 }
 
@@ -3618,6 +3660,20 @@
         const uint32_t c = narrow[v];
         wide[v] = make_int4((int)(c & 0xFFu), (int)((c >> 8) & 0xFFu), (int)((c >> 16) & 0xFFu), 0);
     }
+}
+
+__global__ __launch_bounds__(256) void k_weight_widen(const uint16_t* __restrict__ narrow, int32_t* __restrict__ wide,
+                                                      uint64_t nvox) {
+    for (uint64_t v = (uint64_t)blockIdx.x * blockDim.x + threadIdx.x; v < nvox; v += (uint64_t)gridDim.x * blockDim.x)
+        wide[v] = (int32_t)narrow[v];
+}
+
+hipError_t launch_weight_widen(const uint16_t* narrow, int32_t* wide, uint64_t nvox, hipStream_t s) {
+    if (nvox == 0) return hipSuccess;
+    uint64_t blocks = (nvox + 255) / 256;
+    if (blocks > 65536) blocks = 65536;
+    hipLaunchKernelGGL(k_weight_widen, dim3((unsigned)blocks), dim3(256), 0, s, narrow, wide, nvox);
+    return hipGetLastError();
 }
 
 hipError_t launch_color_widen(const uint8_t* narrow, int32_t* wide, uint64_t nvox, hipStream_t s) {
@@ -3902,7 +3958,7 @@
         const int gz = local_to_global_z(g, l);
         if (gz >= g.dimz) continue;
         const uint32_t t = tile_index(g, x, y, l);
-        const int w = b.wt[t];
+        const int w = wt_at(b, t);
         const float s = b.sdf[t];
         if (w < min_w || !(fabsf(s) < sdf_max)) continue;
         unsigned r, gg, bb;
@@ -4092,7 +4148,7 @@
             local_to_global_z(g, L) < g.dimz) {
             const uint32_t t = tile_index(g, X, Y, L);
             s = b.sdf[t];
-            const unsigned ok = b.wt[t] >= min_w ? 1u : 0u, ng = s < 0.0f ? 1u : 0u;
+            const unsigned ok = wt_at(b, t) >= min_w ? 1u : 0u, ng = s < 0.0f ? 1u : 0u;
             f = ok | (ng << 1);
             has_neg |= (int)(ok & ng);
             has_pos |= (int)(ok & (ng ^ 1u));
@@ -4315,7 +4371,13 @@
          tile += gridDim.x * 4u) {
         const uint32_t t0 = tile * 256u + lane * 4u;
         const float4 s4 = reinterpret_cast<const float4*>(b.sdf)[t0 >> 2];
-        const int4 w4 = reinterpret_cast<const int4*>(b.wt)[t0 >> 2];
+        int4 w4;
+        if (b.wt_wide) {
+            w4 = reinterpret_cast<const int4*>(b.wt)[t0 >> 2];
+        } else {
+            const uint2 p = reinterpret_cast<const uint2*>(b.wt)[t0 >> 2];
+            w4 = make_int4((int)(p.x & 0xFFFFu), (int)(p.x >> 16), (int)(p.y & 0xFFFFu), (int)(p.y >> 16));
+        }
         const float sv[4] = {s4.x, s4.y, s4.z, s4.w};
         const int wv[4] = {w4.x, w4.y, w4.z, w4.w};
         unsigned sel = 0;
diff --git a/slam-maskrcnn_amd/csrc/semtsdf_wscan.h b/slam-maskrcnn_amd/csrc/semtsdf_wscan.h
--- /dev/null
+++ b/slam-maskrcnn_amd/csrc/semtsdf_wscan.h
@@ -0,0 +1,23 @@
+#pragma once
+#include <stdint.h>
+
+namespace semtsdf {
+
+constexpr int64_t kNarrowWeightMax = 65535;
+
+struct WeightScan {
+    int64_t wmax;
+    bool fits_u16;
+};
+
+inline WeightScan scan_weights(const int32_t* wt, uint64_t n) {
+    WeightScan r{0, true};
+    for (uint64_t i = 0; i < n; ++i) {
+        const int64_t w = wt[i];
+        if (w > r.wmax) r.wmax = w;
+        if (w < 0 || w > kNarrowWeightMax) r.fits_u16 = false;
+    }
+    return r;
+}
+
+}
```

After: 1.737 million Mvoxel-updates/s (median of 6 runs). 1.08x the previous value.
